# real-world-cryprography/APSU

Hardware: AMD Instinct MI355X
Metric: sender query-eval ms (ComputePowers + all BinBundles + gather), 16M-4096 params (lower is better)
Workload: dtype u64; 1 GPU; 16M-4096: n=8192, 4 bundle indices x 7 BinBundles (degrees [1303, 170]), 6 source -> 72 target powers, ps_low_degree=44; db_bytes_rank0=5459379072, binbundles_rank0=28, parallelism=binbundle-shard x1

## Files before the change

### apsu_amd/csrc/c_api.cpp

```cpp
#include "../../include/apsu_he.h"

#include <algorithm>
#include <thread>
#include <atomic>
#include <cstdlib>
#include <cstddef>
#include <cstring>
#include <new>
#include <string>

#include "db_file.h"
#include "engine.h"
#include "multi.h"
#include "wire.h"
#include "seal_codec.h"

using namespace apsu_he;

#include <condition_variable>
#include <mutex>
#include <unordered_set>

struct apsu_he_powers;
struct apsu_he_ctx { std::unique_ptr<Engine> eng; std::unordered_set<apsu_he_powers *> live_powers; int recycling = 0; };
// ... 296 lines not shown

static void wrap_bundles(std::vector<std::unique_ptr<Bundle>> &made, apsu_he_bundle **out)
{
    std::vector<std::unique_ptr<apsu_he_bundle>> hs(made.size());
    for (auto &h : hs) h = std::make_unique<apsu_he_bundle>();
    for (size_t i = 0; i < hs.size(); i++) { hs[i]->b = std::move(made[i]); out[i] = hs[i].release(); }
}

int apsu_he_bundle_split(apsu_he_ctx *c, const apsu_he_bundle *b, uint32_t parts, const uint32_t *cache_idx, apsu_he_bundle **out)
{
    return guarded([&] {
        REQUIRE(c && b && b->b && out, "null argument");
        auto made = c->eng->split_bundle(*b->b, parts, cache_idx);
        wrap_bundles(made, out);
    });
}

int apsu_he_bundle_adopt(apsu_he_ctx *dst, apsu_he_ctx *src, const apsu_he_bundle *b, uint32_t cache_idx, apsu_he_bundle **out)
{
    return guarded([&] {
        REQUIRE(dst && src && b && b->b && out, "null argument");
        std::vector<std::unique_ptr<Bundle>> made;
        made.push_back(dst->eng->adopt_bundle(*src->eng, *b->b, cache_idx));
        wrap_bundles(made, out);
    });
}

int apsu_he_db_rebase(apsu_he_ctx *dst, apsu_he_ctx *src, const apsu_he_bundle *const *bundles, uint32_t n_bundles, apsu_he_bundle **out,
                      uint32_t *origin, uint32_t *cache_idx, uint32_t capacity, uint32_t *n_out)
{
    return guarded([&] {
        REQUIRE(dst && src && n_out && ((out && origin) || !capacity), "null argument");
        const auto v = bundle_ptrs(bundles, n_bundles);
        Engine::RebaseResult r = dst->eng->rebase_from(*src->eng, v.data(), n_bundles);
        *n_out = (uint32_t)r.bundles.size();
        if (r.bundles.size() > capacity)
            throw std::invalid_argument("rebase: " + std::to_string(r.bundles.size()) + " BinBundles come out, the caller has room for " + std::to_string(capacity));
        for (size_t i = 0; i < r.bundles.size(); i++) { origin[i] = r.origin[i]; if (cache_idx) cache_idx[i] = r.bundles[i]->cache_idx; }
        wrap_bundles(r.bundles, out);
    });
}

int apsu_he_db_entries_plan(const apsu_he_ctx *c, const uint64_t *offsets, uint32_t *bundles_per_index, uint32_t *total)
{
    return guarded([&] {
        REQUIRE(c && offsets && total, "null argument");
        const BulkPlan plan = c->eng->entries_plan(offsets);
        REQUIRE(plan.total <= 0xFFFFFFFFull, "more than 2^32 - 1 BinBundles");
        if (bundles_per_index) std::copy(plan.bundles.begin(), plan.bundles.end(), bundles_per_index);
        *total = (uint32_t)plan.total;
    });
}

int apsu_he_db_build_from_entries(apsu_he_ctx *c, const uint8_t *entries, int entries_on_device, const uint64_t *offsets, apsu_he_bundle **out,
                                  uint32_t capacity, uint32_t *n_out)
{
    return guarded([&] {
        REQUIRE(c && offsets && n_out && (out || !capacity), "null argument");
        const BulkPlan plan = c->eng->entries_plan(offsets);
        REQUIRE(plan.total <= 0xFFFFFFFFull, "more than 2^32 - 1 BinBundles");
        *n_out = (uint32_t)plan.total;
        if (plan.total > capacity)
            throw std::invalid_argument("build_from_entries: " + std::to_string(plan.total) + " BinBundles come out, the caller has room for " + std::to_string(capacity));
        REQUIRE(entries || !plan.total, "null argument");
        auto made = c->eng->build_from_entries(entries, entries_on_device != 0, offsets);
        wrap_bundles(made, out);
    });
}

int apsu_he_bundle_bins(apsu_he_ctx *c, const apsu_he_bundle *b, uint64_t *roots, uint32_t *counts, uint32_t stride)
{ return guarded([&] { REQUIRE(c && b && b->b && counts, "null argument"); c->eng->bundle_bins(*b->b, roots, counts, stride); }); }
int apsu_he_debug_bundle_bins_form(apsu_he_ctx *c, const apsu_he_bundle *b, uint64_t *roots, uint32_t *counts, uint32_t stride, int form)
{
    return guarded([&] {
        REQUIRE(c && b && b->b && counts, "null argument");
        REQUIRE(form >= Engine::BINS_FORM_AUTO && form <= Engine::BINS_FORM_COMPOSED, "unknown form");
        c->eng->bundle_bins(*b->b, roots, counts, stride, form);
    });
}
int apsu_he_debug_run_step(apsu_he_ctx *c, const apsu_he_step_args *args)
{
    return guarded([&] {
        REQUIRE(c && args, "null argument");
        static_assert((int)APSU_HE_STEP_LIFT == (int)Engine::STEP_LIFT && (int)APSU_HE_STEP_UNLIFT == (int)Engine::STEP_UNLIFT && (int)APSU_HE_STEP_INTT_TENSOR == (int)Engine::STEP_INTT_TENSOR && (int)APSU_HE_STEP_ROOTS_SPLIT == (int)Engine::STEP_ROOTS_SPLIT && (int)APSU_HE_STEP_SEED_EXPAND == (int)Engine::STEP_SEED_EXPAND && (int)APSU_HE_STEP_FLAG_MONOMIAL == (int)Engine::STEP_FLAG_MONOMIAL && (int)APSU_HE_STEP_MAC_INFO == (int)Engine::STEP_MAC_INFO && (int)APSU_HE_STEP_LIMB0_ROWS == (int)Engine::STEP_LIMB0_ROWS && (int)APSU_HE_STEP_ENTRIES_SCATTER + 1 == (int)Engine::STEP_COUNT && (int)APSU_HE_STEP_KEY == (int)Engine::STEP_KEY &&
                      (int)APSU_HE_STEP_KARA == (int)Engine::STEP_KARA && (int)APSU_HE_STEP_PACKED == (int)Engine::STEP_PACKED && (int)APSU_HE_STEP_LIMB_SLOW == (int)Engine::STEP_LIMB_SLOW &&
                      (int)APSU_HE_STEP_COMPOSED == (int)Engine::STEP_COMPOSED && (int)APSU_HE_STEP_NORED == (int)Engine::STEP_NORED, "step ids of the header and the engine");
        Engine::StepArgs a{};
        a.step = args->step; a.chain_idx = args->chain_idx; a.flags = args->flags;
        a.terms = args->terms; a.polys = args->polys; a.batch = args->batch; a.e0 = args->e0; a.n_ext = args->n_ext;
        for (int i = 0; i < 6; i++) { a.in[i] = args->in[i]; a.in_words[i] = args->in_words[i]; }
        for (int i = 0; i < 2; i++) { a.out[i] = args->out[i]; a.out_words[i] = args->out_words[i]; }
        c->eng->debug_run_step(a);
    });
}
static int read_op_times(apsu_he_ctx *c, Engine::Op op, std::initializer_list<double *> out)
{
    return guarded([&] {
        REQUIRE(c, "null argument");
        double ms[Engine::OP_SPANS];
        c->eng->op_times(op, ms, (int)out.size());
        int i = 0;
        for (double *p : out) { if (p) *p = ms[i]; i++; }
    });
}
int apsu_he_debug_bins_times(apsu_he_ctx *c, double *decode_ms, double *roots_ms, double *mult_ms)
{ return read_op_times(c, Engine::OP_BINS, { decode_ms, roots_ms, mult_ms }); }
int apsu_he_debug_split_times(apsu_he_ctx *c, double *decode_ms, double *roots_ms, double *split_ms, double *build_ms)
{ return read_op_times(c, Engine::OP_SPLIT, { decode_ms, roots_ms, split_ms, build_ms }); }
int apsu_he_debug_merge_times(apsu_he_ctx *c, double *decode_ms, double *kernel_ms, double *encode_ms)
{ return read_op_times(c, Engine::OP_MERGE, { decode_ms, kernel_ms, encode_ms }); }
int apsu_he_debug_build_from_entries_times(apsu_he_ctx *c, double *copy_ms, double *scatter_ms, double *build_ms)
{ return read_op_times(c, Engine::OP_BUILD, { copy_ms, scatter_ms, build_ms }); }
int apsu_he_debug_set_scatter_blocks(apsu_he_ctx *c, uint32_t blocks)
{ return guarded([&] { REQUIRE(c, "null argument"); c->eng->set_scatter_blocks(blocks); }); }
int apsu_he_debug_lookup_times(apsu_he_ctx *c, double *decode_ms, double *kernels_ms)
{ return read_op_times(c, Engine::OP_LOOKUP, { decode_ms, kernels_ms }); }
int apsu_he_algebraize_items(apsu_he_ctx *c, const uint8_t *items, size_t count, int items_on_device, uint64_t *felts, int felts_on_device)
{
    return guarded([&] {
        REQUIRE(c && (!count || (items && felts)), "null argument");
        c->eng->algebraize_items(items, count, items_on_device != 0, felts, felts_on_device != 0);
    });
}
int apsu_he_item_locations(apsu_he_ctx *c, const uint8_t *items, size_t count, int items_on_device, uint32_t *locs, int locs_on_device)
{
    return guarded([&] {
        REQUIRE(c && (!count || (items && locs)), "null argument");
        c->eng->item_locations(items, count, items_on_device != 0, locs, locs_on_device != 0);
    });
}
int apsu_he_items_bucket(apsu_he_ctx *c, const uint8_t *items, size_t count, int items_on_device, uint64_t *offsets, uint32_t *order, uint64_t *total)
{
    return guarded([&] {
        REQUIRE(c && offsets && total && (!count || (items && order)), "null argument");
        c->eng->items_bucket(items, count, items_on_device != 0, offsets, order, total);
    });
}
int apsu_he_cuckoo_table(apsu_he_ctx *c, const uint8_t *items, size_t count, int items_on_device, uint64_t max_rounds, uint32_t *table_idx,
                         uint32_t *item_loc, uint64_t *rounds)
{
    return guarded([&] {
        REQUIRE(c && table_idx && (!count || (items && item_loc)), "null argument");
        c->eng->cuckoo_table(items, count, items_on_device != 0, max_rounds, table_idx, item_loc, rounds);
    });
}
int apsu_he_query_values(apsu_he_ctx *c, const uint8_t *table_items, int on_device, uint64_t *values, int values_on_device)
{
    return guarded([&] {
        REQUIRE(c && table_items && values, "null argument");
        c->eng->query_values(table_items, on_device != 0, values, values_on_device != 0);
    });
}
int apsu_he_debug_item_locations(apsu_he_ctx *c, const uint8_t *items, size_t count, uint32_t hash_func_count, uint32_t table_size, uint32_t *locs)
{
    return guarded([&] {
        REQUIRE(c && (!count || (items && locs)), "null argument");
        c->eng->debug_item_locations(items, count, hash_func_count, table_size, locs);
    });
}
int apsu_he_debug_cuckoo_insert(apsu_he_ctx *c, const uint8_t *items, const uint32_t *locs, size_t count, uint32_t hash_func_count, uint32_t table_size,
                                uint64_t max_rounds, int form, uint32_t *table_idx, uint32_t *item_loc, uint64_t *rounds)
{
    return guarded([&] {
        REQUIRE(c && table_idx && (!count || (items && locs && item_loc)), "null argument");
        c->eng->debug_cuckoo_insert(items, locs, count, hash_func_count, table_size, max_rounds, form, table_idx, item_loc, rounds);
    });
}
// ... 1425 lines not shown
```

### apsu_amd/csrc/dev_consts.cpp

```cpp
#include "dev_consts.h"
#include "eval_plan.h"
#include "mac_core.h"

#include <algorithm>
#include <cstdint>
#include <cstdlib>
#include <cstring>
#include <stdexcept>
#include <string>
#include <utility>

namespace apsu_he {

uint32_t packed_row_bits(u64 q)
{
    const int bits = 64 - __builtin_clzll(q);
    for (u32 c = (u32)std::max(bits, 32); c < 64; c++) {
        u32 g = 2 * c, r = 32;
        while (r) { const u32 t2 = g % r; g = r; r = t2; }
        if ((32 - g) + 2 * c <= 128) return c;
    }
    return 64;
}

// ... 149 lines not shown
            dc.map_ksacc[(size_t)c * (DMAXL + 1) + I] = id;
        }
    }
    dc.map_ext_fin = dc.map_ext;
    for (int c = 0; c < nl; c++) {
        DevLevel &d = dc.levels[c];
        if (!behz_unrolled(d.L, d.nB)) continue;
        for (int e = 0; e < d.E; e++) {
            (e < d.L ? d.fin_q[e] : d.fin_b[e - d.L]) = table_ref<ShoupConst>(dc.fin.size());
            push_twisted(hp, dc.map_ext[(size_t)c * DMAXE + e], e < d.L ? d.t_inv_punct_q[e].w : d.t_bsk[e - d.L].w, dc.fin);
            dc.map_ext_fin[(size_t)c * DMAXE + e] |= NTT_MAP_RAW;
        }
    }
    for (int c = 1; c < nl; c++) {
        DevLevel &d = dc.levels[c];
        for (int j = 0; j + 1 < d.L; j++) {
            d.drop_tw[j] = table_ref<ShoupConst>(dc.drop.size());
            push_twisted(hp, j, d.inv_q_last[j].w, dc.drop);
        }
        d.last_tw = scale_ref(hp, d.L - 1);
    }
    dc.map_ksacc_raw = dc.map_ksacc;
    for (int &v : dc.map_ksacc_raw) v |= NTT_MAP_RAW;
    dc.map_ct.resize(DMAXL + DMAXB + 4);
    for (size_t i = 0; i < dc.map_ct.size(); i++) dc.map_ct[i] = (int)i;
}

static void build_key(const HeParams &hp, DeviceConstants &dc)
{
    DevKey &k = dc.key;
    std::memset(&k, 0, sizeof(k));
    k.K = hp.K;
    for (int j = 0; j < hp.K; j++) k.q[j] = make_mod(hp.key_q[j]);
    if (hp.K > 1) {
        const u64 p = hp.key_q[hp.K - 1];
        k.p_half = p >> 1;
        for (int j = 0; j < hp.K - 1; j++) {
            k.p_half_mod[j] = k.p_half % hp.key_q[j];
            k.inv_p[j] = shoup_const(hp.inv_p_mod_q[j], hp.key_q[j]);
            k.md_tw[j] = table_ref<ShoupConst>(dc.mdtw.size());
            push_twisted(hp, j, hp.inv_p_mod_q[j], dc.mdtw);
        }
        k.p_tw = scale_ref(hp, hp.K - 1);
    }
    if (hp.K - 1 > hp.first_chain_idx && hp.K <= DMAXL) {
        dc.key_level.resize(1);
        DevLevel &d = dc.key_level[0];
        std::memset(&d, 0, sizeof(d));
        d.L = hp.K;
        for (int j = 0; j < hp.K; j++) d.q[j] = k.q[j];
    }
    for (u64 q : hp.key_q) {
        dc.max_multiple.push_back(~(u64)0 - (~(u64)0 % q) - 1);
        dc.row_bits.push_back(packed_row_bits(q));
    }
}

DeviceConstants build_device_constants(const HeParams &hp)
{
    DeviceConstants dc;
    build_transform_tables(hp, dc);
    build_levels(hp, dc);
    build_key(hp, dc);
    dc.data_primes_narrow = true;
    for (u64 q : hp.key_q) dc.data_primes_narrow = dc.data_primes_narrow && ntt_is_narrow(q, hp.logn);
    dc.ext_primes_narrow = dc.data_primes_narrow;
    for (u64 m : hp.aux_primes) dc.ext_primes_narrow = dc.ext_primes_narrow && ntt_is_narrow(m, hp.logn);
    dc.unlift_exact = hp.batching && hp.key_q[0] / 2 >= hp.t && hp.key_q[0] > 2 * hp.t;
    return dc;
}

EngineSwitches read_switches()
{
    EngineSwitches s;
    auto flag = [](const char *name, auto &out) { if (const char *v = std::getenv(name)) out = std::atoi(v) != 0; };
    auto size = [](const char *name, size_t &out) { if (const char *v = std::getenv(name)) out = std::strtoull(v, nullptr, 10); };
    flag("APSU_HE_SPLIT", s.two_stream_default);
    flag("APSU_HE_MAC_KARA", s.mac_kara);
    flag("APSU_HE_EVAL_SIDE", s.eval_side);
    flag("APSU_HE_PACKED_ROWS", s.packed_rows);
    flag("APSU_HE_EVAL_PER_TERM", s.force_per_term);
    flag("APSU_HE_SEED_EXPAND_HOST", s.seed_expand_host);
    flag("APSU_HE_FUSE_TAIL", s.fuse_tail);
    size("APSU_HE_EVAL_WS_BYTES", s.eval_ws_bytes);
    size("APSU_HE_ARENA_BYTES", s.arena_bytes);
    size("APSU_HE_NTT_LATENCY_LIMBS", s.ntt_latency_limbs);
    size("APSU_HE_SEED_REJ_CAP", s.seed_rej_cap);
    return s;
}

}
```

### apsu_amd/csrc/dev_consts.h

```cpp
#pragma once
#include <cstddef>
#include <vector>

#include "modmath.h"
#include "ntt_core.h"
#include "ntt_form.h"
#include "params.h"

namespace apsu_he {

constexpr int EW_T = 256;
constexpr int DMAXL = 8;
constexpr int DMAXB = DMAXL + 2;
constexpr int DMAXE = DMAXL + DMAXB;
constexpr u32 SEED_REJ_CAP = 8192;

struct ShoupConst { u64 w, wq; };

struct DevLevel {
    int L, nB, nBsk, E;
    Mod q[DMAXL];
    Mod bsk[DMAXB];
    Mod ext[DMAXE];
    u64 t;
// ... 23 lines not shown
    u64 msk_half;
    ShoupConst s_q_to_bsk[DMAXB][DMAXL];
    ShoupConst s_prod_q_bsk[DMAXB];
    ShoupConst s_q_to_bsk_mt[DMAXB][DMAXL];
    ShoupConst s_prod_q_bsk_mt[DMAXB];
    ShoupConst s_fl[DMAXB];
    ShoupConst s_B_to_q[DMAXL][DMAXB];
    ShoupConst s_B_to_msk[DMAXB];
    ShoupConst s_prod_B_q[DMAXL], s_neg_prod_B_q[DMAXL];
    const ShoupConst *fin_q[DMAXL];
    const ShoupConst *fin_b[DMAXB];
    const ShoupConst *drop_tw[DMAXL];
    const ShoupConst *last_tw;
};

struct DevKey {
    int K;
    Mod q[DMAXL + 1];
    u64 p_half;
    u64 p_half_mod[DMAXL];
    ShoupConst inv_p[DMAXL];
    const ShoupConst *md_tw[DMAXL];
    const ShoupConst *p_tw;
};

constexpr int NTT_MAP_RAW = 1 << 30, NTT_MAP_MASK = NTT_MAP_RAW - 1;

inline ShoupConst shoup_const(u64 w, u64 q) { return ShoupConst{ w, (u64)(((u128)w << 64) / q) }; }
inline Mod make_mod(u64 q) { ModulusInfo m(q); return Mod{ q, m.ratio[0], m.ratio[1] }; }
uint32_t packed_row_bits(u64 q);

inline NttTable make_ntt_table(u64 q, int logn)
{
    const ModulusInfo m(q);
    NttTable tb{};
    tb.q = q;
    tb.r1 = m.ratio[1];
    tb.r0 = m.ratio[0];
    tb.narrow = ntt_is_narrow(q, logn) ? 1 : 0;
    ntt_fold_params(q, tb.fold_k, tb.fold_c);
    tb.wide_d4 = ntt_wide_d4(q, tb.narrow != 0);
    return tb;
}
inline NttTable make_ntt_table(const NttTablesHost &t, int logn, const TwPair *fwd, const TwPair *dit, const TwPair *scale)
{
    NttTable tb = make_ntt_table(t.mod.value, logn);
    tb.ninv = t.ninv;
    tb.ninv_q = t.ninv_q;
    tb.fwd = fwd;
    tb.dit = dit;
    tb.scale = scale;
    return tb;
}

struct DeviceConstants {
    std::vector<TwPair> tw;
    std::vector<NttTable> tabs;
    std::vector<ShoupConst> fin, drop, mdtw;
    std::vector<DevLevel> levels;
    DevKey key;
    std::vector<int> map_ext, map_ext_fin, map_ks, map_ksacc, map_ksacc_raw, map_ct;
    std::vector<DevLevel> key_level;
    std::vector<u64> max_multiple;
    bool data_primes_narrow = false;
    bool ext_primes_narrow = false;
    bool unlift_exact = false;
    std::vector<u32> row_bits;
    void relocate(const TwPair *tw_base, const ShoupConst *fin_base, const ShoupConst *drop_base, const ShoupConst *mdtw_base);
};
DeviceConstants build_device_constants(const HeParams &hp);

struct EngineSwitches {
    static constexpr size_t ARENA_AUTO = ~(size_t)0;
    int two_stream_default = -1;
    bool eval_side = true;
    bool packed_rows = true;
    size_t eval_ws_bytes = (size_t)6 << 30;
    size_t arena_bytes = ARENA_AUTO;
    bool force_per_term = false;
    int mac_kara = -1;
    bool seed_expand_host = false;
    size_t seed_rej_cap = SEED_REJ_CAP;
    bool fuse_tail = true;
    size_t ntt_latency_limbs = NTT_FORM_AUTO;
};
EngineSwitches read_switches();

}
```

### apsu_amd/csrc/engine.h

```cpp
#pragma once
#include <hip/hip_runtime.h>

#include <functional>
#include <memory>
#include <mutex>
#include <string>
#include <vector>

#include "device.h"
#include "params.h"
#include "db_place.h"
#include "db_compact.h"
#include "bulk_place.h"
#include "powers_dag.h"
#include "powers_sched.h"
#include "bundle_layout.h"

namespace apsu_he {

struct HipError : std::runtime_error { using std::runtime_error::runtime_error; };

class DevBuf {
public:
    DevBuf() = default;
// ... 129 lines not shown
    RebaseResult rebase_from(Engine &src, const Bundle *const *bundles, uint32_t n_bundles);
    void bundles_eval_plain(const Bundle *const *bundles, uint32_t n_bundles, const u64 *x, bool x_on_device, const u64 *masks, bool masks_on_device,
                            u64 *out, bool out_on_device, unsigned char *is_bin);
    SelfTestReport self_test(const Bundle *const *bundles, uint32_t count, const u64 seed[8], const u64 *x_host, const uint32_t *query_indices = nullptr,
                             uint32_t n_query = 0, const uint32_t *mask_positions = nullptr);
    enum { SAVED_STRIPPED = 1, SAVED_NO_CACHE = 2 };
    std::vector<uint8_t> export_saved(const Bundle &b, const u64 ntt_parms_id[4], uint32_t flags, int compr);
    struct CompactResult {
        CompactPlan plan;
        std::vector<std::unique_ptr<Bundle>> merged;
    };
    CompactResult compact(uint32_t bundle_idx, const Bundle *const *bundles, uint32_t n_bundles);
    void algebraize_items(const unsigned char *items, size_t count, bool items_on_device, u64 *out, bool out_on_device);
    void item_locations(const unsigned char *items, size_t count, bool items_on_device, uint32_t *locs, bool locs_on_device);
    void items_bucket(const unsigned char *items, size_t count, bool items_on_device, u64 *offsets, uint32_t *order, u64 *total);
    void cuckoo_table(const unsigned char *items, size_t count, bool items_on_device, u64 max_rounds, uint32_t *table_idx, uint32_t *item_loc, u64 *rounds);
    void query_values(const unsigned char *table_items, bool on_device, u64 *values, bool values_on_device);
    enum { CUCKOO_FORM_AUTO = 0, CUCKOO_FORM_LDS = 1, CUCKOO_FORM_GLOBAL = 2 };
    void debug_item_locations(const unsigned char *items, size_t count, uint32_t H, uint32_t T, uint32_t *locs);
    void debug_cuckoo_insert(const unsigned char *items, const uint32_t *locs, size_t count, uint32_t H, uint32_t T, u64 max_rounds, int form,
                             uint32_t *table_idx, uint32_t *item_loc, u64 *rounds);
    size_t bundle_image_size(const Bundle &b) const;
    size_t save_bundle(const Bundle &b, unsigned char *buf, size_t capacity);
    std::unique_ptr<Bundle> load_bundle(const unsigned char *buf, size_t size);
    void mask_generate(u64 seed, uint32_t count, u64 *masks_dev, u64 *values_host, u64 *blocks_host);
    void mask_generate_blake2xb(const u64 seed[8], u64 first_value, uint32_t count, u64 *masks_dev, u64 *values_host, u64 *blocks_host);
    void decrypt_decode(const u64 *sk_ntt_host, const u64 *cts, bool on_device, uint32_t count, u64 *values_host, u64 *blocks_host,
                        int *budget_bits = nullptr, bool sk_on_device = false, u64 *values_dev = nullptr);
    void keygen(const u64 seed[8], u64 *sk_ntt_host, bool sk_on_device = false);
    void relin_keygen(const u64 *sk_ntt_host, const u64 seed[8], u64 *ksk_host, u64 *seeds_host, std::unique_ptr<RelinKeys> *resident,
                      bool sk_on_device = false);
    void query_create(const u64 *sk_ntt_host, const u64 seed[8], const uint32_t *bundle_indices, int nb, const u64 *values, bool values_on_device,
                      u64 *cts_dev, u64 *seeds_host, bool sk_on_device = false);
    void seed_expand(int chain_idx, int count, const u64 *seeds, u64 *const *dst);
    size_t download_coeff(const Bundle &b, uint32_t d, u64 *out, size_t capacity, int *kind);
    std::unique_ptr<Powers> compute_powers(const uint32_t *bundle_indices, int nb, const u64 *const *src, bool on_device,
                                           const RelinKeys *rk);
    void eval_bundles(const Bundle *const *bundles, int count, const Powers &pw, const RelinKeys *rk,
                      const u64 *const *masks, bool masks_on_device, u64 *out, bool out_on_device, u64 *const *out_rows = nullptr);

    uint32_t power_size(uint32_t power) const;
    uint32_t result_size(const Bundle &b) const;
    uint32_t result_polys() const { return result_polys_; }

    size_t workspace_bytes() const { return arena_.bytes(); }
    enum Counter { C_HOST_SYNC = 0, C_JOB_UPLOAD, C_JOB_HIT, C_ARENA_GROW, C_POWERS_ALLOC, C_STAGE_WRAP, C_JOB_REALLOC, C_PIPELINED, C_COUNT };
    void counters_read(uint64_t *out, int capacity) const { for (int i = 0; i < capacity && i < C_COUNT; i++) out[i] = counters_[i]; }

    enum ProfKind { P_NTT_FWD = 0, P_NTT_INV, P_MAC, P_BEHZ_EXT, P_TENSOR, P_BEHZ_FINISH, P_KEYSWITCH, P_MODSWITCH, P_OTHER, P_NTT_FUSED, P_COUNT };
    struct ProfStats { double ms[P_COUNT]; uint64_t launches[P_COUNT]; uint64_t units[P_COUNT]; };
    void profile_enable(int mode);
    void profile_read(ProfStats *out, bool reset);
    enum Phase { PH_RUN_QUERY = 0, PH_COMPUTE_POWERS, PH_PROCESS_BIN_BUNDLE_CACHE, PH_COUNT };
    struct PhaseSummary { uint64_t count = 0; double sum_ms = 0, min_ms = 0, max_ms = 0; };
    static const char *phase_name(int phase);
    void phase_enable(bool on);
    void phase_read(PhaseSummary *out, bool reset);
    void set_two_stream(int mode) { std::lock_guard<std::mutex> g(mu_); two_stream_mode_ = mode < 0 ? -1 : (mode ? 1 : 0); }
    void set_async_results(bool on) { std::lock_guard<std::mutex> g(mu_); async_results_ = on; }
    void set_query_overlap(int mode)
    {
        std::lock_guard<std::mutex> g(mu_);
        inputs_ready_ = mode != 0;
        pipe_cp_ = mode == 1 || mode == 3;
        force_pipe_ = mode == 3;
    }
    void set_tier1_on_device(bool on) { std::lock_guard<std::mutex> g(mu_); tier1_device_ = on; }
    void wait();
    void drain();
    bool take_bad_source();
    void download_power(const Powers &pw, uint32_t bundle_idx, uint32_t power, u64 *out, size_t capacity_words, int *chain_idx,
                        int *is_ntt);
    int device() const { return device_; }
    enum Step { STEP_LEVEL_INFO = 0, STEP_BEHZ_EXT, STEP_DROP_BEHZ_EXT, STEP_TENSOR, STEP_TENSOR_CONV, STEP_TENSOR_SUM, STEP_BEHZ_FINISH,
                STEP_BEHZ_FINISH_SUM, STEP_KS_INNER, STEP_KS_MODDOWN, STEP_MODSWITCH, STEP_MODSWITCH_JOBS, STEP_I0_FINISH, STEP_EVAL_EPILOGUE,
                STEP_ADD_MANY, STEP_SUM_JOBS, STEP_ADD_PLAIN, STEP_DYADIC_PLAIN, STEP_LIFT,
                STEP_POLYN_WITH_ROOTS, STEP_BINS_UPDATE, STEP_BIN_COUNTS, STEP_POLY_DEGREE, STEP_BINS_LOOKUP, STEP_BINS_MERGE, STEP_BINS_ROWS,
                STEP_BINS_EVAL, STEP_EVAL_COMPARE, STEP_ROOTS, STEP_UNLIFT,
                STEP_NTT_INFO, STEP_NTT, STEP_NTT_GATHER, STEP_INTT_TENSOR,
                STEP_ROOTS_SPLIT,
                STEP_SEED_EXPAND, STEP_DECRYPT_ROUND, STEP_PLAIN_POWERS, STEP_SAMPLE_SMALL, STEP_SMALL_LIFT, STEP_ENC_FINISH, STEP_RLK_FINISH,
                STEP_FLAG_MONOMIAL,
                STEP_MAC_INFO, STEP_MAC, STEP_TERM_PRODUCT, STEP_PACK_ROWS, STEP_UNPACK_ROWS, STEP_LIMB0_ROWS,
                STEP_ENTRIES_SCATTER, STEP_COUNT };
    enum : uint32_t { STEP_RAW = 1, STEP_ACCUMULATE = 2, STEP_STORE = 4, STEP_KEY = 8, STEP_PLAN = 16, STEP_COMPOSED = 32, STEP_INVERSE = 64, STEP_NORED = 128,
                      STEP_KARA = 256, STEP_PACKED = 512, STEP_LIMB_SLOW = 1024 };
    struct StepArgs {
        int step, chain_idx;
        uint32_t flags;
        int terms, polys, batch, e0, n_ext;
        const u64 *in[6];
        size_t in_words[6];
        u64 *out[2];
        size_t out_words[2];
    };
    void debug_run_step(const StepArgs &a);
    void debug_run_db_step(const StepArgs &a);
    void debug_run_ntt_step(const StepArgs &a);
    void debug_run_query_step(const StepArgs &a);
    void debug_run_mac_step(const StepArgs &a);
    std::mutex &wire_mutex() { return wire_mu_; }
    void wire_stage(size_t bytes, u64 **device, u64 **pinned);

private:
    u64 *ws(size_t words);
    template <class T> T *ws_as(size_t count, size_t extra_words = 0);
    void ws_reset(size_t need_bytes_hint = 0);
    template <class T> const T *upload_jobs(const std::vector<T> &v);

    const DevLevel *dlevel(int chain_idx) const { return d_levels_.u() ? reinterpret_cast<const DevLevel *>(d_levels_.p()) + chain_idx : nullptr; }
    const LevelConstants &hlevel(int chain_idx) const { return hp_.level[chain_idx]; }
    const NttTable *tabs() const { return reinterpret_cast<const NttTable *>(d_tabs_.p()); }
    const DevKey *dkey() const { return reinterpret_cast<const DevKey *>(d_key_.p()); }
    const int *map_ct() const { return reinterpret_cast<const int *>(d_map_ct_.p()); }
    const int *map_ext(int chain_idx) const { return reinterpret_cast<const int *>(d_map_ext_.p()) + chain_idx * DMAXE; }
    const int *map_ext_fin(int chain_idx) const { return reinterpret_cast<const int *>(d_map_ext_fin_.p()) + chain_idx * DMAXE; }
    const int *map_ks(int chain_idx) const { return reinterpret_cast<const int *>(d_map_ks_.p()) + chain_idx * (DMAXL + 1) * DMAXL; }
    const int *map_ksacc(int chain_idx) const { return reinterpret_cast<const int *>(d_map_ksacc_.p()) + chain_idx * (DMAXL + 1); }
    const int *map_ksacc_raw(int chain_idx) const { return reinterpret_cast<const int *>(d_map_ksacc_raw_.p()) + chain_idx * (DMAXL + 1); }

    void d_ntt(u64 *data, size_t count, const int *modmap, int period, bool inverse, bool narrow);
    void d_ntt_ct(u64 *data, size_t polys, int chain_idx, bool inverse) { d_ntt(data, polys * (chain_idx + 1), map_ct(), chain_idx + 1, inverse, data_primes_narrow_); }
    bool d_relinearize(u64 *ct3, size_t ct_stride, int batch, const RelinKeys &rk, int chain_idx, u64 *ext_out = nullptr, int n_ext = 0,
                       u64 **defer_moddown = nullptr);
    void check_level(int chain_idx) const;
    void check_tier1_residues(const u64 *ct, size_t polys, int chain_idx, const char *what) const;
    void d_multiply_sized(const u64 *ea, int sa, const u64 *eb, int sb, u64 *out, int chain_idx);
    std::unique_ptr<Powers> compute_powers_nks(const uint32_t *bundle_indices, int nb, const u64 *const *src, bool on_device);
    void eval_bundles_nks(const Bundle *const *bundles, int count, const Powers &pw, const u64 *const *masks, bool masks_on_device,
                          u64 *out, bool out_on_device, u64 *const *out_rows);
    PowerSizes sizes_;
    uint32_t result_polys_ = 2;

    HeParams hp_;
    const EngineSwitches sw_ = read_switches();
    PSUParams psu_;
    bool has_psu_ = false;
    PowersDag dag_;
    int device_ = 0;
    hipStream_t st_ = nullptr;
    std::mutex mu_;

    DevBuf d_tabs_, d_tw_, d_levels_, d_key_, d_map_ct_, d_map_ext_, d_map_ext_fin_, d_map_ks_, d_map_ksacc_, d_map_ksacc_raw_, d_fin_, d_drop_, d_mdtw_;
    DevBuf arena_;
    size_t arena_off_ = 0;
    struct Lane { hipStream_t st = nullptr; DevBuf arena; size_t off = 0, job_seq = 0; };
    Lane lanes_[3];
    int cur_lane_ = 0, overflow_lane_ = 0;
    void switch_lane(int lane);
    hipEvent_t ev_main_ = nullptr;
    hipEvent_t ev_fork_ = nullptr, ev_side_ = nullptr, ev_intt_ = nullptr;
    bool inputs_ready_ = false;
    bool pipe_cp_ = true;
    bool force_pipe_ = false;
    bool data_primes_narrow_ = false;
    bool ext_primes_narrow_ = false;
    bool async_results_ = false;
    std::vector<hipEvent_t> inflight_;
    size_t inflight_head_ = 0, inflight_count_ = 0;
    int max_inflight_ = 2;
    void throttle_inflight();
    void mark_inflight();
    static constexpr int BAD_SLOTS = 16;
    unsigned *bad_source_ = nullptr;
    unsigned bad_reported_[BAD_SLOTS] = {};
    uint32_t query_seq_ = 0;
    void check_sources();
    void check_sources(const Powers &pw);
    bool bad_source_pending(int slot, bool take);
    void *stage_ = nullptr;
    size_t stage_bytes_ = 0, stage_off_ = 0;
    struct JobWay { DevBuf buf; std::vector<unsigned char> host; uint64_t stamp = 0; };
    struct JobSlot { JobWay way[4]; };
    uint64_t job_stamp_ = 0;
    std::vector<JobSlot> job_slots_;
    size_t job_seq_ = 0, job_seq_base_ = 0;
    std::vector<std::unique_ptr<Powers>> powers_pool_;
public:
    void recycle_powers(std::unique_ptr<Powers> p);
private:
    std::vector<DevBuf> retired_;
    uint64_t counters_[C_COUNT] = {};
    std::mutex wire_mu_;
    DevBuf wire_dev_;
    void *wire_pinned_ = nullptr;
    size_t wire_pinned_bytes_ = 0;

    PowersSched sched_, sched_low_, sched_high_;
    void mask_generate_impl(uint32_t count, u64 *masks_dev, u64 *values_host, u64 *blocks_host, const std::function<void(u64 *, size_t)> &fill);
    bool fuse_tensor_ = true;
    bool tier1_device_ = false;
    void tier1_done() { if (!tier1_device_ || prof_on_) sync(); }
    bool packed_rows_ = true;
    BundleLayout layout_of(uint32_t degree) const { return bundle_layout(psu_.query_params.ps_low_degree, degree, hp_.first_chain_idx); }
    std::unique_ptr<Bundle> new_bundle(uint32_t bundle_idx, uint32_t cache_idx, uint32_t degree, BundleLayout *layout = nullptr) const;
    size_t slot_bytes(int chain_idx, bool packed) const;
    void pack_bundle(Bundle &b);
    void unpack_bundle(Bundle &b);
    MacPlan plan_mac(const std::vector<MacStream> &streams, size_t nlimbs, size_t n) const;
    void d_mac(const MacPlan &p, const MacJob *jobs = nullptr);
    bool split_ok_ = false;
    int two_stream_mode_ = -1;
    struct DagRun;
    void dag_sources(DagRun &run, const u64 *const *src, bool on_device);
    void dag_level(DagRun &run, size_t d, const RelinKeys *rk);
    void dag_outputs(DagRun &run, Powers &pw, bool do_low, bool do_high);
    void dag_walk(const PowersSched &s, int nb, const u64 *const *src, bool on_device, const RelinKeys *rk, Powers &pw);
    void powers_header(Powers &pw, const uint32_t *bundle_indices, int nb, int low_level, int high_level);
    template <class F> void with_powers_span(F &&body);
    struct EvalCall;
    void eval_plain(EvalCall &c, const std::vector<int> &pl_ids);
    void eval_patstock(EvalCall &c, const std::vector<int> &ps_ids);
    void ps_cf_streams(const EvalCall &c, const PsBatch &g, std::vector<MacStream> &out);
    void ps_cf_mac(const EvalCall &c, const PsBatch &g);
    void ps_term_product(const EvalCall &c, const PsBatch &g);
    void ps_i0_finish(const EvalCall &c, const EvalPlan &plan, const PsBatch &g, u64 *i0);
    void ps_tables(EvalCall &c, const EvalPlan &plan, PsBatch &g);
    void ps_run(EvalCall &c, const EvalPlan &plan, PsBatch &g);
    void ps_mac(EvalCall &c, const EvalPlan &plan, PsBatch &g);
    void ps_side(EvalCall &c, const EvalPlan &plan, PsBatch &g);
    void ps_drop_ext(EvalCall &c, const EvalPlan &plan, PsBatch &g);
    void ps_products_summed(EvalCall &c, const EvalPlan &plan, PsBatch &g);
    void ps_products_per_term(EvalCall &c, const EvalPlan &plan, PsBatch &g);
    u64 *ps_i0(EvalCall &c, const EvalPlan &plan, PsBatch &g);
    void ps_epilogue(EvalCall &c, PsBatch &g, const u64 *i0);
    void finish_bundle(Bundle &b, const u64 *raw);
    void encode_bundle(Bundle &b, const u64 *poly);
    void decode_bundle(const Bundle &b, u64 *poly, u64 *coeff = nullptr);
    void decode_coeff(const Bundle &b, u64 *raw);
    void export_coeff(const Bundle &b, DevBuf &raw);
    void build_from_roots(Bundle &b, const u64 *droots, const uint32_t *dcounts, uint32_t bins, uint32_t stride);
    enum { NEED_PSU = 1, NEED_BATCHING, NEED_DECODE };
    void lookup_check(const char *what, int need = NEED_DECODE) const;
    u64 *decode_counted(const Bundle &b, uint32_t *dcounts, u64 *coeff = nullptr, EventStamps *evs = nullptr, size_t mid = 0);
    struct OpClock { EventStamps evs; double ms[OP_SPANS] = {}; } clock_[OP_COUNT];
    void lookup_impl(const Bundle *const *bundles, uint32_t n_bundles, const u64 *felts, const uint32_t *start, size_t count, uint32_t *counts,
                     unsigned char *flags);
    void eval_plain_queue(const Bundle *const *bundles, uint32_t n_bundles, const u64 *const *xs, const u64 *const *masks, u64 *out, unsigned char *is_bin,
                          u32 *bad, EventStamps &evs, size_t first);
    static void eval_plain_collect(const EventStamps &evs, size_t first, uint32_t n_bundles, double *ms);
    struct BinsCounted { u64 *poly, *coeff; uint32_t *dcounts; const uint32_t *counts; };
    struct BinsFound { std::vector<uint32_t> occ, found, mult; std::vector<u64> hits; uint32_t hstride = 0; };
    bool bins_prepare(const Bundle &b, int form);
    BinsCounted bins_counted(const Bundle &b, bool want_coeff, uint32_t *counts, EventStamps &evs);
    void bins_search(const BinsCounted &c, bool kernel, const uint32_t *stride, EventStamps &evs, size_t s, BinsFound &f);
    struct BinsDevice { uint32_t *occ, *found, *mult; u64 *hits; };
    BinsDevice bins_search_device(const BinsCounted &c, bool kernel, const uint32_t *stride, EventStamps &evs, size_t s, BinsFound &f);
    void bins_finish(const BinsCounted &c, BinsFound &f, u64 *roots, uint32_t stride);
    void keep_coeff_rows(const Bundle &b, const u64 *coeff, DevBuf &keep);
    void roots_tables();
    u64 roots_g_ = 0;
    DevBuf d_roots_step_, d_roots_pts_;
    uint32_t scatter_blocks_ = 0;
    bool unlift_exact_ = false;
    DevBuf d_slot_map_;
    DevBuf d_cuckoo_tabs_;
    void cuckoo_tables_ready();
    const unsigned char *cuckoo_items(const unsigned char *items, size_t count, bool on_device);
    void cuckoo_insert_run(const unsigned char *ditems, const uint32_t *dlocs, uint32_t count, uint32_t H, uint32_t T, u64 max_rounds, int form,
                           uint32_t *table_idx, uint32_t *item_loc, u64 *rounds);
    bool queue_seed_expand(int L, int count, const u64 *seeds, u64 *const *dst);
    bool seeds_overflowed(int count);
    const DevLevel *seed_level(int L);
    void host_seed_expand(int L, int count, const u64 *seeds, u64 *const *dst);
    void check_key_residues(const u64 *sk_ntt_host, int limbs) const;
    DevBuf d_seed_rej_, d_key_level_;
    std::vector<DevLevel> key_level_;
    std::vector<u64> max_multiple_;

    struct ProfRec { hipEvent_t a, b; int kind; uint64_t units; };
    bool prof_on_ = false, prof_open_ = false, prof_ntt_only_ = false;
    std::vector<ProfRec> prof_recs_;
    std::vector<hipEvent_t> prof_pool_;
    ProfStats prof_{};
    void prof_begin(int kind, uint64_t units);
    void prof_end();
    void prof_collect();

    struct PhaseSpan { hipEvent_t a = nullptr, b = nullptr, b2 = nullptr; int phase = 0; };
    bool phase_on_ = false;
    std::vector<PhaseSpan> phase_spans_;
    std::vector<hipEvent_t> phase_pool_;
    PhaseSummary phase_[PH_COUNT];
    hipEvent_t query_start_ = nullptr, query_end_ = nullptr;
    hipEvent_t phase_event(hipStream_t st);
    void phase_close_query();
    void phase_collect();
    struct Enter;
    friend struct EngineAccess;
    friend struct ProfScope;
};

}
```

### apsu_amd/csrc/engine_eval.cpp

```cpp
#include "engine_impl.h"
#include "eval_plan.h"

namespace apsu_he {

static const u64 *bundle_slot(const Bundle &b, bool lifted, size_t slot, size_t dense_words)
{
    const DevBuf &buf = lifted ? b.lifted : b.ntt;
    if (!b.packed) return buf.u() + slot * dense_words;
    return reinterpret_cast<const u64 *>(static_cast<const char *>(buf.p()) + slot * (lifted ? b.lifted_slot_bytes : b.ntt_slot_bytes));
}
static u32 bundle_stride(const Bundle &b, bool lifted, size_t dense_words)
{
    return b.packed ? (u32)(lifted ? b.lifted_slot_bytes : b.ntt_slot_bytes) : (u32)dense_words;
}

struct Engine::EvalCall {
    const Bundle *const *bundles; const Powers &pw; const RelinKeys *rk;
    const u64 *const *masks; bool masks_on_device; u64 *const *out_rows;
    size_t n; uint32_t l; int high, low; size_t Ll, Lh, Eh; u32 low_term_stride;
    std::vector<int> bslot;
    int c0 = 0;
    u64 *res = nullptr, *mask_d = nullptr;
    const u64 *low_ptr(uint32_t power, int b) const { return pw.low.u() + (((size_t)b * pw.n_low + (power - 1)) * 2) * Ll * n; }
    const u64 *hext_ptr(uint32_t i, int b) const { return pw.hext.u() + (((size_t)b * pw.n_high + (i - 1)) * 2) * Eh * n; }
    u64 *res_ptr(int i) const { return out_rows ? out_rows[c0 + i] : res + (size_t)i * 2 * n; }
    const u64 *mask_ptr(int i) const { return masks_on_device ? masks[c0 + i] : mask_d + (size_t)i * n; }
    const Bundle &bundle(int i) const { return *bundles[c0 + i]; }
    int slot(int i) const { return bslot[c0 + i]; }
};
struct PsBatch {
    std::vector<int> ids;
    std::vector<int> nin, in_off;
    int Bs = 0, NI = 0;
    u64 *inner = nullptr, *ssum = nullptr, *vlast = nullptr, *term = nullptr, *cf = nullptr;
    std::vector<int> imap;
    const int *imap_dev = nullptr;
    size_t n_vlast_side = 0;
    MacPlan mac;
    const MacJob *mac_jobs = nullptr;
    const TermJob *term_jobs = nullptr;
    size_t n_term = 0; bool term_packed = false;
    u64 *ext = nullptr, *result = nullptr, *ks_acc = nullptr, *i0_side = nullptr;
};

void Engine::eval_plain(EvalCall &c, const std::vector<int> &pl_ids)
{
    const int Bp = (int)pl_ids.size();
    const int lvl = c.low;
    const size_t Lv = lvl + 1;
    u64 *acc = ws((size_t)Bp * 2 * Lv * c.n);
    std::vector<MacStream> ms;
    std::vector<EpiJob> ej;
    for (int x = 0; x < Bp; x++) {
        const Bundle &b = c.bundle(pl_ids[x]);
        u64 *o = acc + (size_t)x * 2 * Lv * c.n;
        if (b.degree) ms.push_back(MacStream{ bundle_slot(b, false, 0, Lv * c.n), c.low_ptr(1, c.slot(pl_ids[x])), o, b.degree,
                                              bundle_stride(b, false, Lv * c.n), c.low_term_stride, (u32)(c.Ll * c.n), (u32)(Lv * c.n), 0, (u32)Lv,
                                              (u32)b.packed });
        else HIP_CHECK(hipMemsetAsync(o, 0, 2 * Lv * c.n * sizeof(u64), st_));
        ej.push_back(EpiJob{ o, nullptr, nullptr, b.a0.u(), c.mask_ptr(pl_ids[x]), c.res_ptr(pl_ids[x]) });
    }
    d_mac(plan_mac(ms, Lv, c.n));
    d_ntt_ct(acc, (size_t)Bp * 2, lvl, true);
    { PROFW(P_MODSWITCH, (size_t)Bp * c.n * (2 * Lv + 4)); launch_eval_epilogue(dlevel(0), lvl, upload_jobs(ej), Lv * c.n, hp_.irrelevant_bit_count, c.n, Bp, st_); }
}

void Engine::ps_cf_streams(const EvalCall &c, const PsBatch &g, std::vector<MacStream> &out)
{
    for (int x = 0; x < g.Bs; x++) {
        const Bundle &b = c.bundle(g.ids[x]);
        out.push_back(MacStream{ bundle_slot(b, true, 0, c.Lh * c.n), c.hext_ptr(1, c.slot(g.ids[x])), g.cf + (size_t)x * 2 * c.Lh * c.n, b.H,
                                 bundle_stride(b, true, c.Lh * c.n), (u32)((size_t)2 * c.Eh * c.n), (u32)(c.Eh * c.n), (u32)(c.Lh * c.n), 0, (u32)c.Lh,
                                 (u32)b.packed });
    }
}
void Engine::ps_cf_mac(const EvalCall &c, const PsBatch &g)
{
    std::vector<MacStream> cs;
    ps_cf_streams(c, g, cs);
    d_mac(plan_mac(cs, c.Lh, c.n));
}

void Engine::eval_patstock(EvalCall &c, const std::vector<int> &ps_ids)
{
    if (c.low < c.high) throw std::logic_error("the low powers lie below the high powers");
    PsBatch g;
    g.ids = ps_ids;
    std::stable_sort(g.ids.begin(), g.ids.end(), [&](int a, int b) { return c.slot(a) < c.slot(b); });
    g.Bs = (int)g.ids.size();
    g.nin.resize(g.Bs); g.in_off.resize(g.Bs);
    EvalState s{};
    for (int x = 0; x < g.Bs; x++) {
        const Bundle &b = c.bundle(g.ids[x]);
        g.nin[x] = (int)b.H - (b.r == 0 ? 1 : 0);
        g.in_off[x] = g.NI;
        g.NI += g.nin[x];
        s.max_terms = std::max(s.max_terms, g.nin[x]);
    }
    s.low = c.low; s.high = c.high;
    s.L = hlevel(c.high).L; s.nB = hlevel(c.high).nB;
    s.l = c.l; s.q_last = hlevel(c.low).q[c.Ll - 1];
    for (size_t j = 0; j < c.Lh; j++) s.q_widest = std::max(s.q_widest, hlevel(c.high).q[j]);
    s.Bs = g.Bs;
    s.high_in_flight = c.pw.high_async && c.pw.high_ready;
    s.eval_side = sw_.eval_side; s.prof_on = prof_on_; s.force_per_term = sw_.force_per_term; s.fuse_tensor = fuse_tensor_; s.fuse_tail = sw_.fuse_tail;
    s.lane2 = lanes_[2].st != nullptr; s.on_lane0 = cur_lane_ == 0;
    const EvalPlan plan = plan_eval(s);
    ps_tables(c, plan, g);
    ps_run(c, plan, g);
}

void Engine::ps_tables(EvalCall &c, const EvalPlan &plan, PsBatch &g)
{
    const size_t n = c.n, Ll = c.Ll, Lh = c.Lh;
    const uint32_t l = c.l;
    const int Bs = g.Bs;
    const bool cf_here = plan.cf == CF_WITH_MAC;
    const size_t w_inner = (size_t)g.NI * 2 * Ll * n, w_ssum = plan.i0_fast ? (size_t)Bs * 2 * Lh * n : 0;
    const size_t w_vlast = plan.need_vlast ? (size_t)Bs * l * 2 * n : 0, w_term = plan.i0_fast ? 0 : (size_t)Bs * l * 2 * Ll * n;
    const size_t w_cf = (size_t)Bs * 2 * Lh * n;
    g.inner = ws(w_inner + w_ssum + w_vlast + w_term + (cf_here ? w_cf : 0));
    g.ssum = g.inner + w_inner; g.vlast = g.ssum + w_ssum; g.term = g.vlast + w_vlast;
    g.cf = cf_here ? g.term + w_term : nullptr;
    std::vector<MacStream> ms;
    auto map_push = [&](size_t polys, int first_limb, int limbs) {
        for (size_t p = 0; p < polys; p++) for (int j = 0; j < limbs; j++) g.imap.push_back(first_limb + j);
    };
    for (int x = 0; x < Bs; x++) {
        const Bundle &b = c.bundle(g.ids[x]);
        for (int i = 1; i <= g.nin[x]; i++) {
            const u32 cnt = (u32)i < b.H ? l : b.r;
            ms.push_back(MacStream{ bundle_slot(b, false, (size_t)i * l, Ll * n), c.low_ptr(1, c.slot(g.ids[x])),
                                    g.inner + ((size_t)g.in_off[x] + i - 1) * 2 * Ll * n, cnt,
                                    bundle_stride(b, false, Ll * n), c.low_term_stride, (u32)(Ll * n), (u32)(Ll * n), 0, (u32)Ll,
                                    (u32)b.packed });
        }
    }
    map_push((size_t)g.NI * 2, 0, (int)Ll);
    if (plan.raw_drop) for (int &v : g.imap) v |= NTT_MAP_RAW;
    if (plan.i0_fast) {
        for (int x = 0; x < Bs; x++) {
            const Bundle &b = c.bundle(g.ids[x]);
            ms.push_back(MacStream{ bundle_slot(b, false, 0, Ll * n), c.low_ptr(1, c.slot(g.ids[x])), g.ssum + (size_t)x * 2 * Lh * n, l,
                                    bundle_stride(b, false, Ll * n), c.low_term_stride, (u32)(Ll * n), (u32)(Lh * n), 0, (u32)Lh,
                                    (u32)b.packed });
        }
        map_push((size_t)Bs * 2, 0, (int)Lh);
        if (plan.raw_i0) for (size_t x = g.imap.size() - (size_t)Bs * 2 * Lh; x < g.imap.size(); x++) g.imap[x] |= NTT_MAP_RAW;
    }
    std::vector<TermJob> tj;
    if (plan.need_vlast || !plan.i0_fast) {
        for (int x = 0; x < Bs; x++) {
            const Bundle &b = c.bundle(g.ids[x]);
            const int bs = c.slot(g.ids[x]);
            if (plan.i0_fast) {
                if (x == 0) g.term_packed = b.packed;
                else if (g.term_packed != (bool)b.packed) throw std::logic_error("BinBundles of one evaluation differ in their row format");
            }
            for (u32 j = 1; j <= l; j++) {
                if (plan.i0_fast)
                    tj.push_back(TermJob{ bundle_slot(b, false, j - 1, Ll * n), c.low_ptr(j, bs), g.vlast + ((size_t)x * l + j - 1) * 2 * n });
                else
                    ms.push_back(MacStream{ bundle_slot(b, false, j - 1, Ll * n), c.low_ptr(j, bs),
                                            g.term + ((size_t)x * l + j - 1) * 2 * Ll * n, 1, bundle_stride(b, false, Ll * n), c.low_term_stride,
                                            (u32)(Ll * n), (u32)(Ll * n), 0, (u32)Ll, (u32)b.packed });
            }
        }
        if (plan.i0_fast) {
            map_push((size_t)Bs * l * 2, (int)Ll - 1, 1);
            if (plan.raw_i0) for (size_t x = g.imap.size() - (size_t)Bs * l * 2; x < g.imap.size(); x++) g.imap[x] |= NTT_MAP_RAW;
        } else map_push((size_t)Bs * l * 2, 0, (int)Ll);
    }
    if (plan.side_i0) g.n_vlast_side = (size_t)Bs * l * 2;
    if (cf_here) { ps_cf_streams(c, g, ms); map_push((size_t)Bs * 2, 0, (int)Lh); }
    g.mac = plan_mac(ms, Ll, n);
    g.mac_jobs = upload_jobs(g.mac.jobs);
    if (!tj.empty()) { g.term_jobs = upload_jobs(tj); g.n_term = tj.size(); }
}

void Engine::ps_term_product(const EvalCall &c, const PsBatch &g)
{
    PROF(P_MAC, (uint64_t)g.n_term * (g.term_packed ? packed_row_bits(hp_.key_q[c.Ll - 1]) : 64));
    launch_term_product(dlevel(c.low), g.term_jobs, g.n_term, c.n, (int)c.Ll - 1, (u32)(c.Ll * c.n), (u32)c.n, g.term_packed, st_);
}
void Engine::ps_i0_finish(const EvalCall &c, const EvalPlan &plan, const PsBatch &g, u64 *i0)
{
    std::vector<I0Job> ij;
    for (int x = 0; x < g.Bs; x++)
        ij.push_back(I0Job{ g.ssum + (size_t)x * 2 * c.Lh * c.n, g.vlast + (size_t)x * c.l * 2 * c.n, i0 + (size_t)x * 2 * c.Lh * c.n, (int)c.l, 1 });
    PROFW(P_MODSWITCH, (size_t)g.Bs * c.n * (4 * c.Lh + 2 * c.l));
    launch_i0_finish(dlevel(c.low), upload_jobs(ij), c.n, g.Bs, st_, plan.raw_i0);
}

void Engine::ps_mac(EvalCall &c, const EvalPlan &plan, PsBatch &g)
{
    d_mac(g.mac, g.mac_jobs);
    g.imap_dev = upload_jobs(g.imap);
    if (plan.side_i0) HIP_CHECK(hipEventRecord(ev_fork_, st_));
    else if (g.n_term) ps_term_product(c, g);
    d_ntt(g.inner, g.imap.size() - g.n_vlast_side, g.imap_dev, (int)g.imap.size(), true, false);
    if (plan.side_i0) HIP_CHECK(hipEventRecord(ev_intt_, st_));
}

void Engine::ps_side(EvalCall &c, const EvalPlan &plan, PsBatch &g)
{
    g.cf = ws((size_t)g.Bs * 2 * c.Lh * c.n);
    if (plan.side_i0) g.i0_side = ws((size_t)g.Bs * 2 * c.Lh * c.n);
    else HIP_CHECK(hipEventRecord(ev_fork_, st_));
    switch_lane(2);
    struct Back { Engine *e; ~Back() { e->switch_lane(0); } } back{ this };
    HIP_CHECK(hipStreamWaitEvent(st_, ev_fork_, 0));
    if (plan.side_i0) {
        ps_term_product(c, g);
        d_ntt(g.vlast, g.n_vlast_side, g.imap_dev + (g.imap.size() - g.n_vlast_side), (int)g.n_vlast_side, true, false);
    }
    if (plan.wait_high_ready) HIP_CHECK(hipStreamWaitEvent(st_, c.pw.high_ready, 0));
    ps_cf_mac(c, g);
    d_ntt_ct(g.cf, (size_t)g.Bs * 2, c.high, true);
    if (plan.side_i0) {
        HIP_CHECK(hipStreamWaitEvent(st_, ev_intt_, 0));
        ps_i0_finish(c, plan, g, g.i0_side);
    }
    HIP_CHECK(hipEventRecord(ev_side_, st_));
}

void Engine::ps_drop_ext(EvalCall &c, const EvalPlan &plan, PsBatch &g)
{
    const size_t n = c.n;
    const int NI = g.NI;
    const LevelConstants &h = hlevel(c.high);
    g.ext = ws((size_t)NI * 2 * c.Eh * n);
    if (plan.fused_drop) {
        PROFW(P_BEHZ_EXT, (size_t)NI * 2 * n * (c.Ll + c.Eh));
        if (!launch_drop_behz_ext(dlevel(c.high), h.L, h.nB, g.inner, c.Ll * n, 1, g.ext, n, NI * 2, st_, plan.raw_drop))
            throw std::logic_error("the plan takes the fused drop + extension, the kernel table has none for this level");
    } else {
        u64 *innerh = g.inner;
        for (int lv = c.low; lv > c.high; lv--) {
            u64 *nxt = ws((size_t)NI * 2 * lv * n);
            { PROFW(P_MODSWITCH, (size_t)NI * 2 * n * (2 * lv + 1)); launch_modswitch(dlevel(lv), innerh, (size_t)2 * (lv + 1) * n, 2, nxt, n, NI, st_); }
            innerh = nxt;
        }
        { PROFW(P_BEHZ_EXT, (size_t)NI * 2 * n * (c.Lh + c.Eh)); launch_behz_ext(dlevel(c.high), h.L, h.nB, innerh, c.Lh * n, 1, g.ext, n, NI * 2, st_); }
    }
    d_ntt(g.ext, (size_t)NI * 2 * c.Eh, map_ext(c.high), (int)c.Eh, false, ext_primes_narrow_);
}

void Engine::ps_products_summed(EvalCall &c, const EvalPlan &plan, PsBatch &g)
{
    const size_t n = c.n, Lh = c.Lh, Eh = c.Eh, nBskh = Eh - Lh;
    const int Bs = g.Bs, NI = g.NI;
    const LevelConstants &h = hlevel(c.high);
    const bool late_cf = plan.cf == CF_BEHIND_HIGH_READY;
    g.result = ws((size_t)Bs * 3 * Lh * n);
    u64 *dq = ws((size_t)NI * 3 * Lh * n + (size_t)Bs * 3 * nBskh * n + (late_cf ? (size_t)Bs * 2 * Lh * n : 0));
    u64 *bsum = dq + (size_t)NI * 3 * Lh * n;
    if (late_cf) {
        g.cf = bsum + (size_t)Bs * 3 * nBskh * n;
        ps_cf_mac(c, g);
    }
    std::vector<TensorSumJob> tj;
    std::vector<FinishSumJob> fj;
    std::vector<int> dmap;
    for (int x = 0; x < Bs; x++) {
        if (!g.nin[x]) { HIP_CHECK(hipMemsetAsync(g.result + (size_t)x * 3 * Lh * n, 0, 3 * Lh * n * sizeof(u64), st_)); continue; }
        const size_t job = (size_t)g.in_off[x];
        tj.push_back(TensorSumJob{ g.ext + job * 2 * Eh * n, c.hext_ptr(1, c.slot(g.ids[x])), dq + job * 3 * Lh * n,
                                   bsum + (size_t)x * 3 * nBskh * n, g.nin[x], 0 });
        fj.push_back(FinishSumJob{ dq + job * 3 * Lh * n, bsum + (size_t)x * 3 * nBskh * n, g.result + (size_t)x * 3 * Lh * n, g.nin[x], 0 });
    }
    const int rawf = behz_unrolled(h.L, h.nB) ? NTT_MAP_RAW : 0;
    for (size_t p = 0; p < (size_t)NI * 3; p++) for (size_t j = 0; j < Lh; j++) dmap.push_back((int)j | rawf);
    for (size_t p = 0; p < (size_t)Bs * 3; p++) for (size_t i = 0; i < nBskh; i++) dmap.push_back(hp_.bsk_id(h.nB, (int)i) | rawf);
    if (late_cf) for (size_t p = 0; p < (size_t)Bs * 2; p++) for (size_t j = 0; j < Lh; j++) dmap.push_back((int)j);
    if (plan.fuse_tensor) {
        std::vector<TensorJob> pj;
        for (int x = 0; x < Bs; x++)
            for (int i = 0; i < g.nin[x]; i++) {
                const size_t job = (size_t)g.in_off[x] + i;
                pj.push_back(TensorJob{ g.ext + job * 2 * Eh * n, c.hext_ptr(1 + i, c.slot(g.ids[x])), dq + job * 3 * Lh * n });
            }
        { PROFW(P_TENSOR, ((size_t)NI * 4 + (size_t)Bs * 3) * (Eh - Lh) * n); launch_tensor_sum(dlevel(c.high), (int)Eh, upload_jobs(tj), n, (int)tj.size(), (int)Lh, st_); }
        PROF(P_NTT_FUSED, dmap.size());
        launch_intt_tensor(hp_.logn, upload_jobs(pj), (int)pj.size(), (int)Lh, Eh * n, bsum, dmap.size() - pj.size() * 3 * Lh,
                           tabs(), upload_jobs(dmap), (int)dmap.size(), st_, sw_.ntt_latency_limbs);
    } else {
        { PROFW(P_TENSOR, ((size_t)NI * 4 * Eh + (size_t)NI * 3 * Lh + (size_t)Bs * 3 * (Eh - Lh)) * n); launch_tensor_sum(dlevel(c.high), (int)Eh, upload_jobs(tj), n, (int)tj.size(), 0, st_); }
        d_ntt(dq, dmap.size(), upload_jobs(dmap), (int)dmap.size(), true, false);
    }
    { PROFW(P_BEHZ_FINISH, ((size_t)NI * 3 * Lh + (size_t)Bs * 3 * (Eh - Lh) + (size_t)Bs * 3 * Lh) * n); launch_behz_finish_sum(dlevel(c.high), h.L, h.nB, upload_jobs(fj), n, (int)fj.size(), st_); }
}

void Engine::ps_products_per_term(EvalCall &c, const EvalPlan &plan, PsBatch &g)
{
    const size_t n = c.n, Lh = c.Lh, Eh = c.Eh;
// ... 180 lines not shown
```

### apsu_amd/csrc/engine_mac_steps.cpp

```cpp
#include "engine_impl.h"
#include "mac_plan.h"

#include <string>

namespace apsu_he {

namespace {

[[noreturn]] void refuse(const std::string &why) { throw std::invalid_argument("debug_run_step: " + why); }
void need(bool ok, const char *why) { if (!ok) refuse(why); }

void canonical(const u64 *x, size_t words, u64 m, const char *what)
{
    u64 bad = 0;
    for (size_t k = 0; k < words; k++) bad |= (u64)(x[k] >= m);
    if (bad) refuse(std::string(what) + " holds a word that is not a canonical residue of its limb");
}

void canonical_dense(const u64 *x, size_t slots, int L, size_t n, const DevLevel &lv, const char *what)
{
    for (size_t s = 0; s < slots; s++)
        for (int j = 0; j < L; j++) canonical(x + (s * L + j) * n, n, lv.q[j].q, what);
}

void canonical_packed(const std::vector<u64> &padded, size_t slots, size_t slot_bytes, int L, size_t n, const DevLevel &lv, const char *what)
{
    const char *base = reinterpret_cast<const char *>(padded.data());
    u64 bad = 0;
    for (size_t s = 0; s < slots; s++)
        for (int j = 0; j < L; j++) {
            const u32 *row = reinterpret_cast<const u32 *>(base + s * slot_bytes + lv.mac_row_off[j]);
            for (size_t c = 0; c < n; c++) bad |= (u64)(packed_coeff(row, c, lv.mac_bits[j]) >= lv.q[j].q);
        }
    if (bad) refuse(std::string(what) + " holds a coefficient that is not a canonical residue of its limb");
}

}

void Engine::debug_run_mac_step(const StepArgs &a)
{
    const size_t n = hp_.n;
    need(a.step >= STEP_MAC_INFO && a.step <= STEP_LIMB0_ROWS, "unknown step");
    check_level(a.chain_idx);
    const int L = a.chain_idx + 1;
    const bool kara = a.flags & STEP_KARA, packed = a.flags & STEP_PACKED, limb_slow = a.flags & STEP_LIMB_SLOW;
    const size_t batch = a.batch > 0 ? (size_t)a.batch : 0, terms = a.terms > 0 ? (size_t)a.terms : 0, polys = a.polys > 0 ? (size_t)a.polys : 0;
    auto in_is = [&](int i, size_t words, const char *what) { if (!a.in[i] || a.in_words[i] != words) refuse(std::string(what) + ": wrong size"); };
    auto out_is = [&](int i, size_t words, const char *what) { if (!a.out[i] || a.out_words[i] != words) refuse(std::string(what) + ": wrong size"); };

    sync();
    DevLevel lv;
    HIP_CHECK(hipMemcpy(&lv, dlevel(a.chain_idx), sizeof(DevLevel), hipMemcpyDeviceToHost));
    if (lv.L != L) throw std::logic_error("debug_run_step: the device's level block is not the level's");
    size_t packed_slot = 0;
    bool any_packed = false;
    for (int j = 0; j < L; j++) { packed_slot += n * lv.mac_bits[j] / 8; any_packed |= lv.mac_bits[j] != 64; }
    const size_t dense_slot = (size_t)L * n * sizeof(u64);

    if (a.step == STEP_MAC_INFO) {
        out_is(0, 2 + 7 * (size_t)L, "mac_info: out[0] [2 + 7 L]");
        u64 *o = a.out[0];
        *o++ = (u64)L; *o++ = packed_slot;
        for (int j = 0; j < L; j++) {
            *o++ = lv.mac_shift[j]; *o++ = lv.mac_chunk[j]; *o++ = lv.mac_chunk_k[j]; *o++ = lv.mac_bits[j]; *o++ = lv.mac_row_off[j];
            *o++ = lv.mac_mask_hi[j]; *o++ = mac_kara_usable(lv.q[j].q) ? 1 : 0;
        }
        return;
    }
    need(n % 64 == 0, "the multiply-accumulate steps take rings of a multiple of 64 coefficients (a bit-packed slot is whole 64-bit words)");
    if (packed) need(any_packed, "packed: every row of this context is 64 bits wide (mac_bits), there is no bit-packed form");
    const size_t slot = packed ? packed_slot : dense_slot, slot_words = slot / 8;

    std::vector<MacJob> mj;
    std::vector<TermJob> tj;
    std::vector<u64> padded;
    auto pad_in = [&](int i) { padded.assign(a.in_words[i] + 2, 0); std::memcpy(padded.data(), a.in[i], a.in_words[i] * sizeof(u64)); };
    size_t P = 0, NL = 0, njobs = 0;
    switch (a.step) {
    case STEP_MAC: {
        need(batch >= 1 && batch <= 64, "mac: batch out of range (1 .. 64)");
        need(polys >= 1 && polys <= (size_t)MAC_G, "mac: streams per job (polys) outside 1 .. 4");
        need(terms >= 1, "mac: a chain of no terms (terms 0)");
        need(terms <= 4096, "mac: terms out of range (1 .. 4096)");
        NL = a.n_ext > 0 ? (size_t)a.n_ext : 0;
        need(a.e0 >= 0 && NL >= 1 && (size_t)a.e0 + NL <= (size_t)L, "mac: limbs limb0 .. limb0 + nl - 1 (e0, n_ext) reach beyond the level");
        const size_t pw_job = batch * terms * 2 * n;
        need(a.in[0] && a.in_words[0] % pw_job == 0, "mac: in[0] powers [batch][terms][2][P][n]: wrong size");
        P = a.in_words[0] / pw_job;
        need(P >= (size_t)L, "mac: powers of fewer limbs per polynomial (P) than the level has");
        need(P <= (size_t)DMAXE, "mac: powers of more limbs per polynomial (P) than an extended polynomial has");
        in_is(1, batch * polys * terms * slot_words, "mac: in[1] plaintexts [batch][polys][terms] slots");
        out_is(0, batch * polys * 2 * NL * n, "mac: out[0] [batch][polys][2][n_ext][n]");
        if (a.in[2]) in_is(2, batch * 4, "mac: in[2] job table [batch][4]");
        if (kara) for (int j = 0; j < L; j++) need(mac_kara_usable(lv.q[j].q), "mac: the three-product form on a level with a prime that mac_kara_usable rejects");
        for (size_t r = 0; r < batch * terms * 2; r++)
            for (int j = 0; j < L; j++) canonical(a.in[0] + (r * P + j) * n, n, lv.q[j].q, "mac: in[0] (powers)");
        if (packed) { pad_in(1); canonical_packed(padded, batch * polys * terms, slot, L, n, lv, "mac: in[1] (bit-packed plaintexts)"); }
        else canonical_dense(a.in[1], batch * polys * terms, L, n, lv, "mac: in[1] (plaintexts)");
        for (size_t b = 0; b < batch; b++) {
            const u64 limb0 = a.in[2] ? a.in[2][b * 4] : (u64)a.e0, nl = a.in[2] ? a.in[2][b * 4 + 1] : NL;
            const u64 ng = a.in[2] ? a.in[2][b * 4 + 2] : polys, cnt = a.in[2] ? a.in[2][b * 4 + 3] : terms;
            need(limb0 <= (u64)L && nl >= 1 && nl <= NL && limb0 + nl <= (u64)L, "mac: a job's limbs (limb0, nl) reach beyond the level or beyond n_ext");
            need(ng >= 1 && ng <= polys, "mac: a job's streams (ng) outside 1 .. polys");
            need(cnt >= 1, "mac: a job with a chain of no terms (cnt 0)");
            need(cnt <= terms, "mac: a job's chain (cnt) is longer than terms");
            MacJob j{};
            j.cnt = (u32)cnt; j.ng = (u32)ng; j.limb0 = (u32)limb0; j.nl = (u32)nl; j.packed = packed ? 1 : 0;
            j.pt_stride = (u32)(packed ? slot : slot_words); j.pw_stride = (u32)(2 * P * n); j.pw_poly_stride = (u32)(P * n); j.out_poly_stride = (u32)(NL * n);
            mj.push_back(j);
        }
    } break;
    case STEP_TERM_PRODUCT: {
        need(batch >= 1 && batch <= 64, "term_product: batch out of range (1 .. 64)");
        need(terms >= 1 && batch * terms <= ((size_t)1 << 17), "term_product: jobs (batch * terms) outside 1 .. 2^17");
        need(a.e0 >= 0 && a.e0 < L, "term_product: the limb (e0) is beyond the level");
        need(a.in[0] && a.in_words[0] % (batch * 2 * n) == 0, "term_product: in[0] powers [batch][2][P][n]: wrong size");
        P = a.in_words[0] / (batch * 2 * n);
        need(P >= (size_t)L && P <= (size_t)DMAXE, "term_product: limbs per polynomial of the powers (P) outside L .. the extended base");
        njobs = batch * terms;
        in_is(1, batch * slot_words, "term_product: in[1] plaintexts [batch] slots");
        out_is(0, (njobs + 1) * 2 * n, "term_product: out[0] [batch * terms + 1][2][n]");
        for (size_t r = 0; r < batch * 2; r++) canonical(a.in[0] + (r * P + (size_t)a.e0) * n, n, lv.q[a.e0].q, "term_product: in[0] (powers)");
        if (packed) { pad_in(1); canonical_packed(padded, batch, slot, L, n, lv, "term_product: in[1] (bit-packed plaintexts)"); }
        else canonical_dense(a.in[1], batch, L, n, lv, "term_product: in[1] (plaintexts)");
    } break;
    case STEP_PACK_ROWS:
    case STEP_UNPACK_ROWS: {
        need(batch >= 1, "pack_rows / unpack_rows: no slots (batch)");
        pack_rows_grid_check(batch, L);
        if (a.step == STEP_PACK_ROWS) {
            in_is(0, batch * (size_t)L * n, "pack_rows: in[0] dense [slots][L][n]");
            out_is(0, batch * packed_slot / 8 + 2, "pack_rows: out[0] [slots] bit-packed slots + 16 bytes");
            canonical_dense(a.in[0], batch, L, n, lv, "pack_rows: in[0]");
        } else {
            in_is(0, batch * packed_slot / 8, "unpack_rows: in[0] [slots] bit-packed slots");
            out_is(0, batch * (size_t)L * n, "unpack_rows: out[0] dense [slots][L][n]");
            pad_in(0);
        }
    } break;
    case STEP_LIMB0_ROWS: {
        need(batch >= 1 && batch <= 65535, "limb0_rows: count (batch) outside 1 .. 65535");
        in_is(0, batch * slot_words, "limb0_rows: in[0] [count] slots");
        out_is(0, batch * n, "limb0_rows: out[0] [count][n]");
        if (packed) pad_in(0);
    } break;
    default: refuse("unknown step");
    }

    WITH_ARENA({
        auto up = [&](const u64 *src, size_t words) {
            u64 *d = ws(words);
            HIP_CHECK(hipMemcpyAsync(d, src, words * sizeof(u64), hipMemcpyHostToDevice, st_));
            return d;
        };
        auto up_slots = [&](int i) { return packed || a.step == STEP_UNPACK_ROWS ? up(padded.data(), padded.size()) : up(a.in[i], a.in_words[i]); };
        auto down = [&](const u64 *src) { HIP_CHECK(hipMemcpyAsync(a.out[0], src, a.out_words[0] * sizeof(u64), hipMemcpyDeviceToHost, st_)); };
        auto jobs = [&](const auto &v) {
            using T = typename std::decay_t<decltype(v)>::value_type;
            T *d = ws_as<T>(v.size());
            HIP_CHECK(hipMemcpyAsync(d, v.data(), v.size() * sizeof(T), hipMemcpyHostToDevice, st_));
            return static_cast<const T *>(d);
        };
        u64 *o = up(a.out[0], a.out_words[0]);

        switch (a.step) {
        case STEP_MAC: {
            const u64 *pw = up(a.in[0], a.in_words[0]);
            const char *pt = reinterpret_cast<const char *>(up_slots(1));
            for (size_t b = 0; b < batch; b++) {
                MacJob &j = mj[b];
                j.pw = pw + b * terms * 2 * P * n;
                for (size_t g = 0; g < (size_t)MAC_G; g++) {
                    j.pt[g] = reinterpret_cast<const u64 *>(pt + ((b * polys + (g < j.ng ? g : 0)) * terms) * slot);
                    j.out[g] = o + (b * polys + (g < polys ? g : 0)) * 2 * NL * n;
                }
            }
            launch_mac(dlevel(a.chain_idx), L, jobs(mj), n, (int)batch, st_, kara, packed, MacGrid{ mac_grid(n, batch).gx, limb_slow ? 1 : 0 });
        } break;
        case STEP_TERM_PRODUCT: {
            const u64 *pw = up(a.in[0], a.in_words[0]);
            const char *pt = reinterpret_cast<const char *>(up_slots(1));
            tj.clear();
            for (size_t u = 0; u < njobs; u++) tj.push_back(TermJob{ reinterpret_cast<const u64 *>(pt + (u % batch) * slot), pw + (u % batch) * 2 * P * n, o + u * 2 * n });
            launch_term_product(dlevel(a.chain_idx), jobs(tj), njobs, n, a.e0, (u32)(P * n), (u32)n, packed, st_);
        } break;
        case STEP_PACK_ROWS:
            launch_pack_rows(dlevel(a.chain_idx), L, up(a.in[0], a.in_words[0]), o, packed_slot, n, batch, st_);
            break;
        case STEP_UNPACK_ROWS:
            launch_unpack_rows(dlevel(a.chain_idx), L, up_slots(0), packed_slot, o, n, batch, st_);
            break;
        default:
            launch_limb0_rows(dlevel(a.chain_idx), L, up_slots(0), slot, packed, o, n, batch, st_);
            break;
        }
        down(o);
        sync();
    });
}

}
```

### apsu_amd/csrc/eval_plan.h

```cpp
#pragma once
#include <cstddef>
#include <cstdint>

namespace apsu_he {

constexpr bool behz_unrolled(int L, int nB) { return L == nB && L <= 3; }

struct EvalState {
    int low, high;
    int L, nB;
    uint32_t l;
    uint64_t q_last;
    uint64_t q_widest;
    int Bs, max_terms;
    bool high_in_flight;
    bool eval_side, prof_on, force_per_term, fuse_tensor, fuse_tail;
    bool lane2, on_lane0;
};
enum CfPlace {
    CF_WITH_MAC = 0,
    CF_SIDE_LANE = 1,
    CF_BEHIND_HIGH_READY = 2
};
enum I0Form {
    I0_SIDE = 0,
    I0_SSUM = 1,
    I0_FINISH_MAIN = 2,
    I0_GENERAL = 3
};
struct EvalPlan {
    bool i0_fast, need_vlast, raw_drop, raw_i0, fused_drop, summed, side, side_i0, wait_high_ready, fuse_tensor, fuse_tail;
    int cf;
    int i0;
};

inline EvalPlan plan_eval(const EvalState &s)
{
    EvalPlan p{};
    const int Lh = s.high + 1;
    p.i0_fast = (s.low - s.high <= 1) && ((unsigned __int128)(s.l + 1) * s.q_last < ((unsigned __int128)1 << 64));
    p.need_vlast = p.i0_fast && s.low > s.high;
    p.raw_drop = s.low == s.high + 1 && behz_unrolled(s.L, s.nB);
    p.raw_i0 = p.need_vlast;
    p.fused_drop = p.raw_drop;
    p.wait_high_ready = s.high_in_flight;
    p.side = s.eval_side && s.high_in_flight && !s.prof_on && p.i0_fast && s.low != s.high && s.lane2 && s.on_lane0;
    p.side_i0 = p.side && (size_t)s.Bs * s.l <= 4096;
    p.cf = !s.high_in_flight ? CF_WITH_MAC : p.side ? CF_SIDE_LANE : CF_BEHIND_HIGH_READY;
    p.i0 = p.side_i0 ? I0_SIDE : p.i0_fast && s.low == s.high ? I0_SSUM : p.i0_fast ? I0_FINISH_MAIN : I0_GENERAL;
    p.summed = !s.force_per_term && Lh <= 4 && (unsigned __int128)s.max_terms * s.q_widest < ((unsigned __int128)1 << 63);
    p.fuse_tensor = s.fuse_tensor;
    p.fuse_tail = s.fuse_tail;
    return p;
}

}
```

### apsu_amd/csrc/kernels_behz.hip

```cpp
#include "launch_behz.h"
#include "kernel_launch.h"
#include "eval_plan.h"

namespace apsu_he {

template <int TL, int TNB>
__global__ __launch_bounds__(EW_T) void k_behz_ext(const DevLevel *__restrict__ lv, const u64 *__restrict__ in,
                                                   size_t in_stride, int polys, u64 *__restrict__ out, size_t n)
{
    const size_t k = (size_t)blockIdx.x * EW_T + threadIdx.x;
    if (k >= n) return;
    const int L = TL ? TL : lv->L, nBsk = TL ? TNB + 1 : lv->nBsk, E = L + nBsk;
    constexpr int LMAX = TL ? TL : DMAXL;
    constexpr int BMAX = TL ? TNB + 1 : DMAXB;
    const size_t c = blockIdx.y / polys, p = blockIdx.y % polys;
    const u64 *src = in + c * in_stride + p * (size_t)L * n;
    u64 *dst = out + (size_t)blockIdx.y * E * n;
    u64 xs[LMAX];
    u32 mt_acc = 0;
#pragma unroll
    for (int j = 0; j < LMAX; j++) {
        if (TL || j < L) {
            const u64 x = src[(size_t)j * n + k];
            dst[(size_t)j * n + k] = x;
// ... 536 lines not shown
#pragma unroll
    for (int p = 0; p < 2; p++) {
        u64 tl = 0;
        const u64 *a = nullptr;
        if constexpr (MD) {
            a = job.ks_acc + (size_t)p * (L + 1) * n;
            const Mod pm = key->q[key->K - 1];
            const u64x2 tw = ldg16(reinterpret_cast<const u64 *>(key->p_tw + k));
            tl = barrett64(mul_shoup(a[(size_t)L * n + k], tw[0], tw[1], pm.q) + key->p_half, pm);
        }
#pragma unroll
        for (int j = 0; j < DMAXL; j++)
            if (j < L) {
                const u64 q = lv->q[j].q;
                u64 x = job.ct[p * ct_poly_stride + (size_t)j * n + k];
                if constexpr (MD) {
                    const Mod m = key->q[j];
                    const u64 tk = submod(barrett64(tl, m), key->p_half_mod[j], m.q);
                    const u64x2 tw = ldg16(reinterpret_cast<const u64 *>(key->md_tw[j] + k));
                    const u64 u = mul_shoup_lazy(a[(size_t)j * n + k], tw[0], tw[1], m.q);
                    const u64 w = mul_shoup_lazy(tk, key->inv_p[j].w, key->inv_p[j].wq, m.q);
                    x = addmod(x, csub(csub(u + (m.q << 1) - w, m.q << 1), m.q), m.q);
                }
                if (job.add1) x = addmod(x, job.add1[((size_t)p * L + j) * n + k], q);
                if (job.add2) x = addmod(x, job.add2[((size_t)p * L + j) * n + k], q);
                v[p][j] = x;
            }
    }
    {
        const u64 m0 = job.a0[k], m1 = job.mask[k];
        const u64 f0 = plain_fix(lv, m0), f1 = plain_fix(lv, m1);
#pragma unroll
        for (int j = 0; j < DMAXL; j++)
            if (j < L) {
                const u64 q = lv->q[j].q;
                v[0][j] = addmod(addmod(v[0][j], scaled_plain(lv, m0, f0, j), q), scaled_plain(lv, m1, f1, j), q);
            }
    }
    for (int l = lvl; l > 0; l--) {
        const DevLevel *ll = levels + l;
        const u64 ql = ll->q[l].q;
#pragma unroll
        for (int p = 0; p < 2; p++) {
            u64 last = 0;
#pragma unroll
            for (int j = 0; j < DMAXL; j++) if (j == l) last = v[p][j];
            last = addmod(last, ll->half, ql);
#pragma unroll
            for (int j = 0; j < DMAXL; j++)
                if (j < l) {
                    const Mod m = ll->q[j];
                    const u64 tmp = submod(barrett64(last, m), ll->half_mod[j], m.q);
                    v[p][j] = mul_shoup(submod(v[p][j], tmp, m.q), ll->inv_q_last[j].w, ll->inv_q_last[j].wq, m.q);
                }
        }
    }
    job.out[k] = v[0][0] & clear_mask;
    job.out[n + k] = v[1][0] & clear_mask;
}

void launch_eval_epilogue(const DevLevel *levels, int lvl, const EpiJob *jobs, size_t ct_poly_stride, int clear_bits, size_t n,
                          int njobs, hipStream_t st, const DevKey *key)
{
    if (!njobs) return;
    const u64 mask = clear_bits > 0 ? ~(((u64)1 << clear_bits) - 1) : ~(u64)0;
    if (key) hipLaunchKernelGGL(k_eval_epilogue<true>, ew_grid(n, njobs), dim3(EW_T), 0, st, levels, lvl, jobs, ct_poly_stride, mask, n, key);
    else hipLaunchKernelGGL(k_eval_epilogue<false>, ew_grid(n, njobs), dim3(EW_T), 0, st, levels, lvl, jobs, ct_poly_stride, mask, n, key);
    KERNEL_CHECK();
}

template <bool RAW>
__global__ __launch_bounds__(EW_T) void k_i0_finish(const DevLevel *__restrict__ lv, const I0Job *__restrict__ jobs, size_t n)
{
    const size_t k = (size_t)blockIdx.x * EW_T + threadIdx.x;
    if (k >= n) return;
    const I0Job job = jobs[blockIdx.y >> 1];
    const int p = blockIdx.y & 1;
    const int L = lv->L;
    const u64 ql = lv->q[L - 1].q, half = lv->half;
    u64 R = 0;
    const u64 *v = job.v + (size_t)p * n + k;
    u64 tw0 = 0, tw1 = 0;
    if (RAW) { const u64x2 tw = ldg16(reinterpret_cast<const u64 *>(lv->last_tw + k)); tw0 = tw[0]; tw1 = tw[1]; }
    for (int t = 0; t < job.terms; t++) {
        u64 x = v[(size_t)t * 2 * n];
        if (RAW) x = mul_shoup(x, tw0, tw1, ql);
        R += addmod(x, half, ql);
    }
    for (int m = 0; m + 1 < L; m++) {
        const Mod mq = lv->q[m];
        const u64 th = barrett128(mul128((u64)job.terms, lv->half_mod[m]), mq);
        const u64 corr = submod(th, barrett64(R, mq), mq.q);
        const size_t o = ((size_t)p * (L - 1) + m) * n + k;
        u64 r;
        if (RAW) {
            const u64x2 tw = ldg16(reinterpret_cast<const u64 *>(lv->drop_tw[m] + k));
            const u64 a = mul_shoup_lazy(job.s[o], tw[0], tw[1], mq.q);
            const u64 b = mul_shoup_lazy(corr, lv->inv_q_last[m].w, lv->inv_q_last[m].wq, mq.q);
            r = csub(csub(a + b, mq.q << 1), mq.q);
        } else {
            const u64 val = addmod(job.s[o], corr, mq.q);
            r = mul_shoup(val, lv->inv_q_last[m].w, lv->inv_q_last[m].wq, mq.q);
        }
        job.acc[o] = job.store ? r : addmod(job.acc[o], r, mq.q);
    }
}

void launch_i0_finish(const DevLevel *lv_low, const I0Job *jobs, size_t n, int njobs, hipStream_t st, bool raw)
{
    if (!njobs) return;
    if (raw) hipLaunchKernelGGL(k_i0_finish<true>, ew_grid(n, njobs * 2), dim3(EW_T), 0, st, lv_low, jobs, n);
    else hipLaunchKernelGGL(k_i0_finish<false>, ew_grid(n, njobs * 2), dim3(EW_T), 0, st, lv_low, jobs, n);
    KERNEL_CHECK();
}

}
```

### apsu_amd/csrc/kernels_ntt.hip

```cpp
#include "launch_ntt.h"
#include "kernel_launch.h"
#include "ntt_wg.h"
#include "ntt_form.h"
#include <type_traits>

namespace apsu_he {

template <int LOGN, bool INV, int T, int C = 16, int MINW = 4>
__global__ __launch_bounds__(T, MINW) void k_ntt(u64 *__restrict__ data, const NttTable *__restrict__ tabs,
                                           const int *__restrict__ modmap, int period, int split)
{
    constexpr int N = 1 << LOGN;
    __shared__ __attribute__((aligned(16))) u64 lds[lds_slots(N)];
    const int tid = threadIdx.x;
    const size_t g = blockIdx.x;
    const int mv = modmap[(split ? g >> 1 : g) % (size_t)period];
    const NttTable tab = tabs[split ? (((mv & NTT_MAP_MASK) << 1) | (int)(g & 1)) : (mv & NTT_MAP_MASK)];
    u64 *p = data + g * N;
    using SRC = std::conditional_t<INV, SrcStaged, SrcPlain>;
    if (INV && ((mv & NTT_MAP_RAW) || split)) {
        if (tab.narrow) ntt_body<LOGN, INV, NTT_NARROW, T, 0, INV, SRC, true, false, 0, -1, C>(lds, p, tab, tid, nullptr, SRC());
        else if (tab.wide_d4) ntt_body<LOGN, INV, NTT_WIDE_NEAR, T, 0, INV, SRC, true, false, 0, -1, C>(lds, p, tab, tid, nullptr, SRC());
        else ntt_body<LOGN, INV, NTT_WIDE, T, 0, INV, SRC, true, false, 0, -1, C>(lds, p, tab, tid, nullptr, SRC());
        return;
// ... 32 lines not shown
    const u64 e = ntt_reduce_any(p[k], tab);
    const u64 o = mul_shoup_lazy(p[k + h], tw[0], tw[1], q);
    u64 x0 = e + o, x1 = e + (q << 1) - o;
    if (!(mv & NTT_MAP_RAW)) {
        const u64x2 s0 = ldg16(reinterpret_cast<const u64 *>(tab.scale + k)), s1 = ldg16(reinterpret_cast<const u64 *>(tab.scale + k + h));
        x0 = mul_shoup(x0, s0[0], s0[1], q);
        x1 = mul_shoup(x1, s1[0], s1[1], q);
    }
    p[k] = x0;
    p[k + h] = x1;
}

template <int LOGN, int T, int C = 16, int MINW = 4>
__global__ __launch_bounds__(T, MINW) void k_ntt_gather(const u64 *const *__restrict__ src, u64 *__restrict__ data,
                                                  const NttTable *__restrict__ tabs, const int *__restrict__ modmap, int period, int nored)
{
    constexpr int N = 1 << LOGN;
    __shared__ __attribute__((aligned(16))) u64 lds[lds_slots(N)];
    const int tid = threadIdx.x;
    const size_t g = blockIdx.x;
    const NttTable tab = tabs[modmap[g % (size_t)period]];
    u64 *p = data + g * N;
    if (tab.narrow) {
        if (nored) ntt_body<LOGN, false, NTT_NARROW, T, 2, false, SrcPlain, true, false, 0, -1, C>(lds, p, tab, tid, src[g]);
        else ntt_body<LOGN, false, NTT_NARROW, T, 1, false, SrcPlain, true, false, 0, -1, C>(lds, p, tab, tid, src[g]);
    } else if (tab.wide_d4) ntt_body<LOGN, false, NTT_WIDE_NEAR, T, 1, false, SrcPlain, true, false, 0, -1, C>(lds, p, tab, tid, src[g]);
    else ntt_body<LOGN, false, NTT_WIDE, T, 1, false, SrcPlain, true, false, 0, -1, C>(lds, p, tab, tid, src[g]);
}

template <int LOGN, int T, int C = 16>
__global__ __launch_bounds__(T, 4) void k_intt_tensor(const TensorJob *__restrict__ jobs, int limbs, size_t src_ps, size_t n_tensor,
                                                   u64 *__restrict__ plain, const NttTable *__restrict__ tabs,
                                                   const int *__restrict__ modmap, int period)
{
    constexpr int N = 1 << LOGN;
    __shared__ __attribute__((aligned(16))) u64 lds[lds_slots(N)];
    const int tid = threadIdx.x;
    size_t g = blockIdx.x;
    {
        const size_t pairs = n_tensor / 3, padded = (pairs + 7) / 8 * 24;
        if (g < padded) {
            const size_t blk = g / 24, rem = g - blk * 24, pl = rem >> 3, u = blk * 8 + (rem & 7);
            if (u >= pairs) return;
            const size_t jb = u / (size_t)limbs, e = u - jb * limbs;
            g = jb * 3 * limbs + pl * limbs + e;
        } else {
            g = n_tensor + (g - padded);
        }
    }
    const int mv = modmap[g % (size_t)period];
    const NttTable tab = tabs[mv & NTT_MAP_MASK];
    if (g >= n_tensor) {
        u64 *p = plain + (g - n_tensor) * N;
        if (mv & NTT_MAP_RAW) {
            if (tab.narrow) ntt_body<LOGN, true, NTT_NARROW, T, 0, true, SrcStaged, true, false, 0, -1, C>(lds, p, tab, tid, nullptr, SrcStaged());
            else if (tab.wide_d4) ntt_body<LOGN, true, NTT_WIDE_NEAR, T, 0, true, SrcStaged, true, false, 0, -1, C>(lds, p, tab, tid, nullptr, SrcStaged());
            else ntt_body<LOGN, true, NTT_WIDE, T, 0, true, SrcStaged, true, false, 0, -1, C>(lds, p, tab, tid, nullptr, SrcStaged());
        } else {
            if (tab.narrow) ntt_body<LOGN, true, NTT_NARROW, T, 0, false, SrcStaged, true, false, 0, -1, C>(lds, p, tab, tid, nullptr, SrcStaged());
            else if (tab.wide_d4) ntt_body<LOGN, true, NTT_WIDE_NEAR, T, 0, false, SrcStaged, true, false, 0, -1, C>(lds, p, tab, tid, nullptr, SrcStaged());
            else ntt_body<LOGN, true, NTT_WIDE, T, 0, false, SrcStaged, true, false, 0, -1, C>(lds, p, tab, tid, nullptr, SrcStaged());
        }
        return;
    }
    const size_t per = (size_t)3 * limbs, jb = g / per;
    const int r = (int)(g - jb * per), pl = r / limbs, e = r - pl * limbs;
    const TensorJob job = jobs[jb];
    const u64 *a0 = job.a + (size_t)e * N, *a1 = a0 + src_ps, *b0 = job.b + (size_t)e * N, *b1 = b0 + src_ps;
    const bool lazy = ntt_lazy_input_ok(tab, LOGN);
    SrcTensor ops;
    if (pl == 0) ops = SrcTensor{ a0, b0, nullptr, nullptr, lazy };
    else if (pl == 1) ops = SrcTensor{ a0, b1, a1, b0, lazy };
    else ops = SrcTensor{ a1, b1, nullptr, nullptr, lazy };
    u64 *p = job.d + (size_t)r * N;
    if (mv & NTT_MAP_RAW) {
        if (tab.narrow) ntt_body<LOGN, true, NTT_NARROW, T, 0, true, SrcTensor, true, false, 0, -1, C>(lds, p, tab, tid, nullptr, ops);
        else if (tab.wide_d4) ntt_body<LOGN, true, NTT_WIDE_NEAR, T, 0, true, SrcTensor, true, false, 0, -1, C>(lds, p, tab, tid, nullptr, ops);
        else ntt_body<LOGN, true, NTT_WIDE, T, 0, true, SrcTensor, true, false, 0, -1, C>(lds, p, tab, tid, nullptr, ops);
    } else {
        if (tab.narrow) ntt_body<LOGN, true, NTT_NARROW, T, 0, false, SrcTensor, true, false, 0, -1, C>(lds, p, tab, tid, nullptr, ops);
        else if (tab.wide_d4) ntt_body<LOGN, true, NTT_WIDE_NEAR, T, 0, false, SrcTensor, true, false, 0, -1, C>(lds, p, tab, tid, nullptr, ops);
        else ntt_body<LOGN, true, NTT_WIDE, T, 0, false, SrcTensor, true, false, 0, -1, C>(lds, p, tab, tid, nullptr, ops);
    }
}

template <class K> struct NttFormRow { int logn, threads, coeffs_per_lane, min_waves; K inv, fwd; };
template <class K, size_t R> static K form_kernel(const NttFormRow<K> (&rows)[R], int logn, const NttForm &f, bool inverse)
{
    for (const NttFormRow<K> &r : rows)
        if (r.logn == logn && r.threads == f.threads && r.coeffs_per_lane == f.coeffs_per_lane && r.min_waves == f.min_waves && (inverse ? r.inv : r.fwd))
            return inverse ? r.inv : r.fwd;
    throw_hip(hipErrorInvalidValue, __FILE__, __LINE__);
    return nullptr;
}

using GatherKernel = void (*)(const u64 *const *, u64 *, const NttTable *, const int *, int, int);
#define ROW(LN, T, C, W) { LN, T, C, W, nullptr, k_ntt_gather<LN, T, C, W> },
static const NttFormRow<GatherKernel> k_ntt_gather_forms[] = {
    ROW(13, 1024, 8, 4) ROW(12, 512, 8, 4) ROW(13, 1024, 8, 8)
    ROW(14, 1024, 16, 4) ROW(13, 512, 16, 4) ROW(12, 256, 16, 4) ROW(11, 128, 16, 4) ROW(10, 64, 16, 4) ROW(8, 64, 16, 4) ROW(6, 64, 16, 4)
};
#undef ROW
using TensorKernel = void (*)(const TensorJob *, int, size_t, size_t, u64 *, const NttTable *, const int *, int);
#define ROW(LN, T, C) { LN, T, C, 4, k_intt_tensor<LN, T, C>, nullptr },
static const NttFormRow<TensorKernel> k_intt_tensor_forms[] = {
    ROW(13, 1024, 8) ROW(12, 512, 8)
    ROW(14, 1024, 16) ROW(13, 512, 16) ROW(12, 256, 16) ROW(11, 128, 16) ROW(10, 64, 16) ROW(8, 64, 16) ROW(6, 64, 16)
};
#undef ROW
using NttKernel = void (*)(u64 *, const NttTable *, const int *, int, int);
#define ROW(LN, T, C, W) { LN, T, C, W, k_ntt<LN, true, T, C, W>, k_ntt<LN, false, T, C, W> },
static const NttFormRow<NttKernel> k_ntt_forms[] = {
    ROW(14, 1024, 16, 4)
    { 13, 1024, 8, 8, nullptr, k_ntt<13, false, 1024, 8, 8> },
    ROW(13, 1024, 8, 4) ROW(12, 512, 8, 4)
    ROW(13, 512, 16, 4) ROW(12, 256, 16, 4) ROW(11, 128, 16, 4) ROW(10, 64, 16, 4) ROW(8, 64, 16, 4) ROW(6, 64, 16, 4)
};
#undef ROW

static void launch_ntt_split(bool inverse, const u64 *const *src, u64 *data, size_t count, const NttTable *tabs, const int *modmap, int period,
                             hipStream_t st, const NttForm &f)
{
    const size_t n = (size_t)1 << SPLIT_LOGN;
    const dim3 g((unsigned)((n / 2 + EW_T - 1) / EW_T), (unsigned)count);
    if (!inverse) hipLaunchKernelGGL(k_ntt_first_stage, g, dim3(EW_T), 0, st, src, data, n, tabs, modmap, period);
    hipLaunchKernelGGL(form_kernel(k_ntt_forms, SPLIT_LOGN - 1, f, inverse), dim3((unsigned)(count * 2)), dim3(f.threads), 0, st,
                       data, tabs, modmap, period, 1);
    if (inverse) hipLaunchKernelGGL(k_ntt_last_stage, g, dim3(EW_T), 0, st, data, n, tabs, modmap, period);
}

void launch_ntt(int logn, bool inverse, u64 *data, size_t count, const NttTable *tabs, const int *modmap, int period,
                hipStream_t st, size_t latency_limbs, bool narrow)
{
    if (!count) return;
    const NttForm f = ntt_form(logn, inverse ? NTT_KIND_INVERSE : NTT_KIND_FORWARD, count, latency_limbs, narrow);
    if (f.split) launch_ntt_split(inverse, nullptr, data, count, tabs, modmap, period, st, f);
    else hipLaunchKernelGGL(form_kernel(k_ntt_forms, logn, f, inverse), dim3((unsigned)count), dim3(f.threads), 0, st, data, tabs, modmap, period, 0);
    KERNEL_CHECK();
}

void launch_ntt_gather(int logn, const u64 *const *src, u64 *data, size_t count, const NttTable *tabs, const int *modmap, int period,
                       hipStream_t st, bool nored, size_t latency_limbs, bool narrow)
{
    if (!count) return;
    const NttForm f = ntt_form(logn, NTT_KIND_GATHER, count, latency_limbs, narrow);
    if (f.split) launch_ntt_split(false, src, data, count, tabs, modmap, period, st, f);
    else hipLaunchKernelGGL(form_kernel(k_ntt_gather_forms, logn, f, false), dim3((unsigned)count), dim3(f.threads), 0, st, src, data, tabs, modmap, period, nored ? 1 : 0);
    KERNEL_CHECK();
}

void launch_intt_tensor(int logn, const TensorJob *jobs, int njobs, int limbs, size_t src_ps, u64 *plain, size_t n_plain,
                        const NttTable *tabs, const int *modmap, int period, hipStream_t st, size_t latency_limbs)
{
    const size_t n_tensor = (size_t)njobs * 3 * limbs;
    const size_t count = (n_tensor / 3 + 7) / 8 * 24 + n_plain;
    if (!(n_tensor + n_plain)) return;
    const NttForm f = ntt_form(logn, NTT_KIND_TENSOR, n_tensor + n_plain, latency_limbs, false);
    hipLaunchKernelGGL(form_kernel(k_intt_tensor_forms, logn, f, true), dim3((unsigned)count), dim3(f.threads), 0, st,
                       jobs, limbs, src_ps, n_tensor, plain, tabs, modmap, period);
    KERNEL_CHECK();
}

}
```

### apsu_amd/csrc/launch_behz.h

```cpp
#pragma once
#include <hip/hip_runtime.h>
#include "dev_consts.h"
#include "launch_ntt.h"

namespace apsu_he {

void launch_behz_ext(const DevLevel *lv, int L, int nB, const u64 *in, size_t in_stride, int polys, u64 *out, size_t n, int cts,
                     hipStream_t st);
bool launch_drop_behz_ext(const DevLevel *lv, int L, int nB, const u64 *in, size_t in_stride, int polys, u64 *out, size_t n, int cts,
                          hipStream_t st, bool raw = false);
void launch_tensor(const DevLevel *lv, const TensorJob *jobs, size_t n, int batch, hipStream_t st);
struct TensorConvJob { const u64 *a, *b; u64 *d; int sa, sb; };
void launch_tensor_conv(const DevLevel *lv, const TensorConvJob *jobs, size_t n, int njobs, hipStream_t st);
struct TensorSumJob { const u64 *a, *b; u64 *dq, *bs; int terms; int pad; };
void launch_tensor_sum(const DevLevel *lv, int E, const TensorSumJob *jobs, size_t n, int njobs, int e0, hipStream_t st);
struct FinishSumJob { const u64 *dq, *bs; u64 *out; int terms; int pad; };
void launch_behz_finish_sum(const DevLevel *lv, int L, int nB, const FinishSumJob *jobs, size_t n, int njobs, hipStream_t st);
struct FinishJob { const u64 *d; u64 *out; int terms; int pad; };
void launch_behz_finish(const DevLevel *lv, int L, int nB, const FinishJob *jobs, bool accumulate, size_t n, int njobs, hipStream_t st);
void launch_ks_inner(const DevKey *key, int L, const u64 *tdec, const u64 *rk, u64 *acc, size_t n, int batch,
                     hipStream_t st);
void launch_ks_moddown(const DevKey *key, int L, const u64 *acc, u64 *ct, size_t ct_stride, size_t n, int batch,
                       hipStream_t st, const DevLevel *lv = nullptr, u64 *ext = nullptr, int n_ext = 0, bool raw = false);
struct EpiJob { const u64 *ct; const u64 *add1; const u64 *add2; const u64 *a0; const u64 *mask; u64 *out;
                const u64 *ks_acc = nullptr; };
void launch_eval_epilogue(const DevLevel *levels, int lvl, const EpiJob *jobs, size_t ct_poly_stride, int clear_bits, size_t n,
                          int njobs, hipStream_t st, const DevKey *key = nullptr);
struct I0Job { const u64 *s; const u64 *v; u64 *acc; int terms; int store; };
void launch_i0_finish(const DevLevel *lv_low, const I0Job *jobs, size_t n, int njobs, hipStream_t st, bool raw = false);

}
```

### apsu_amd/csrc/launch_ntt.h

```cpp
#pragma once
#include <hip/hip_runtime.h>
#include "dev_consts.h"

namespace apsu_he {

void launch_ntt(int logn, bool inverse, u64 *data, size_t count, const NttTable *tabs, const int *modmap,
                int period, hipStream_t st, size_t latency_limbs, bool narrow);
void launch_ntt_gather(int logn, const u64 *const *src, u64 *data, size_t count, const NttTable *tabs, const int *modmap, int period,
                       hipStream_t st, bool nored, size_t latency_limbs, bool narrow);
struct TensorJob { const u64 *a, *b; u64 *d; };
void launch_intt_tensor(int logn, const TensorJob *jobs, int njobs, int limbs, size_t src_ps, u64 *plain, size_t n_plain,
                        const NttTable *tabs, const int *modmap, int period, hipStream_t st, size_t latency_limbs = 0);

}
```

### apsu_amd/csrc/mac_core.h

```cpp
#pragma once
#include <stddef.h>
#include "dev_consts.h"

namespace apsu_he {

constexpr int MAC_G = 4;
constexpr int MAC_C = 2;

struct MacJob {
    const u64 *pt[MAC_G];
    u64 *out[MAC_G];
    const u64 *pw;
    u32 cnt, ng;
    u32 pt_stride, pw_stride, pw_poly_stride;
    u32 out_poly_stride;
    u32 limb0, nl;
    u32 packed, pad;
};
struct TermJob { const u64 *pt; const u64 *pw; u64 *out; };

inline int mac_shift_of(u64 q) { return (64 - __builtin_clzll(q) + 1) / 2; }
inline u32 mac_chunk_of(u64 q)
{
    const u64 cap = (u64)1 << (63 - 2 * mac_shift_of(q)), c = cap > 2 ? cap - 1 : 2;
    return (u32)(c < (1u << 20) ? c : 1u << 20);
}
inline u32 mac_chunk_k_of(u64 q)
{
    const int s = mac_shift_of(q);
    const u64 capk = 2 * s + 2 < 64 ? (u64)1 << (62 - 2 * s) : 0, c = capk > 2 ? capk - 1 : 0;
    return (u32)(c < (1u << 20) ? c : 1u << 20);
}
inline u32 mac_mask_hi_of(u32 w, int s) { return w == 64 ? 0xffffffffu : (u32)(((u64)1 << (w - s)) - 1); }
inline bool mac_kara_usable(u64 q) { return mac_chunk_k_of(q) >= 7; }

#if defined(__HIP_DEVICE_COMPILE__)
#define MAC_KEEP(v) asm("" : "+v"(v))
#else
#define MAC_KEEP(v) do { } while (0)
#endif

HD u32 alignbit(u32 hi, u32 lo, u32 sh)
{
#if defined(__HIP_DEVICE_COMPILE__)
    return __builtin_amdgcn_alignbit(hi, lo, sh);
#else
    return (u32)((((u64)hi << 32) | lo) >> (sh & 31));
#endif
}

HD const u32 *packed_window(const void *slot, u32 row_off, size_t k, u32 kb, u32 &psh)
{
    const u32 bitoff = (u32)(k >> 1) * 2 * kb;
    psh = bitoff & 31;
    return reinterpret_cast<const u32 *>(static_cast<const char *>(slot) + row_off) + (bitoff >> 5);
}
HD void packed_shift(u64 w_lo, u64 w_hi, u32 psh, u64 &lo64, u64 &hi64)
{
    const u32 w0 = (u32)w_lo, w1 = (u32)(w_lo >> 32), w2 = (u32)w_hi, w3 = (u32)(w_hi >> 32);
    const u32 n0 = alignbit(w1, w0, psh), n1 = alignbit(w2, w1, psh), n2 = alignbit(w3, w2, psh), n3 = w3 >> psh;
    lo64 = (u64)n0 | ((u64)n1 << 32); hi64 = (u64)n2 | ((u64)n3 << 32);
}
#define PACKED_SECOND(lo64, hi64, kb) ((kb) == 64 ? (hi64) : (((lo64) >> (kb)) | ((hi64) << (64 - (kb)))))
HD void packed_pair(u64 w_lo, u64 w_hi, u32 psh, u32 kb, u64 &a0, u64 &a1)
{
    u64 lo64, hi64;
    packed_shift(w_lo, w_hi, psh, lo64, hi64);
    if (kb == 64) { a0 = lo64; a1 = hi64; }
    else { const u64 mask = ((u64)1 << kb) - 1; a0 = lo64 & mask; a1 = PACKED_SECOND(lo64, hi64, kb) & mask; }
}
HD u64 packed_coeff(const u32 *row, size_t c, u32 w)
{
    const size_t bit0 = c * w, d0 = bit0 >> 5;
    const u32 sh = (u32)(bit0 & 31);
    u64 v = ((u64)row[d0] | ((u64)row[d0 + 1] << 32)) >> sh;
    if (sh && w + sh > 64) v |= (u64)row[d0 + 2] << (64 - sh);
    return w == 64 ? v : (v & (((u64)1 << w) - 1));
}

#if defined(__HIPCC__)
#define MAC_LANE_FN __global__ __launch_bounds__(EW_T, 1) void
#define MAC_LANE_AT
#define MAC_LANE_AT_DEF const unsigned bx = blockIdx.x, by = blockIdx.y, bz = blockIdx.z, tx = threadIdx.x
#else
#define MAC_LANE_FN inline void
#define MAC_LANE_AT , unsigned bx, unsigned by, unsigned bz, unsigned tx
#define MAC_LANE_AT_DEF (void)0
#endif
template <bool KARA, bool PACKED>
MAC_LANE_FN k_mac(const DevLevel *__restrict__ lv, const MacJob *__restrict__ jobs, size_t n, int limb_slow MAC_LANE_AT)
{
    MAC_LANE_AT_DEF;
    constexpr int G = MAC_G, C = MAC_C;
    unsigned b_x = bx, b_limb = by, b_job = bz;
    if (limb_slow) { b_limb = bz; b_job = by; }
    const size_t k = ((size_t)b_x * EW_T + tx) * C;
    if (k >= n) return;
    const MacJob *__restrict__ jp = jobs + b_job;
    struct { const u64 *pw; u32 cnt, ng, pt_stride, pw_stride, pw_poly_stride, out_poly_stride, limb0; } job =
        { jp->pw, jp->cnt, jp->ng, jp->pt_stride, jp->pw_stride, jp->pw_poly_stride, jp->out_poly_stride, jp->limb0 };
    if ((int)job.ng <= 0 || b_limb >= jp->nl) return;
    const int j = b_limb + job.limb0;
    const Mod m = lv->q[j];
    const u32 s = lv->mac_shift[j], chunk = KARA ? lv->mac_chunk_k[j] : lv->mac_chunk[j];
    const u32 lomask = (1u << s) - 1;
    const u64 *p0 = job.pw + (size_t)j * n + k;
    const u64 *p1 = p0 + job.pw_poly_stride;
    const u64 *pt[G];
    const u32 *ptw[G];
    u32 psh = 0, kb = 64, himask = 0xffffffffu;
    if constexpr (PACKED) {
        kb = lv->mac_bits[j];
        himask = lv->mac_mask_hi[j];
#pragma unroll
        for (int g = 0; g < G; g++) ptw[g] = packed_window(jp->pt[g < (int)job.ng ? g : 0], lv->mac_row_off[j], k, kb, psh);
    } else {
#pragma unroll
        for (int g = 0; g < G; g++) pt[g] = jp->pt[g < (int)job.ng ? g : 0] + (size_t)j * n + k;
    }

    u64 s00[G][C][2], sx[G][C][2], s11[G][C][2];
#pragma unroll
    for (int g = 0; g < G; g++)
#pragma unroll
        for (int c = 0; c < C; c++)
#pragma unroll
            for (int p = 0; p < 2; p++) s00[g][c][p] = sx[g][c][p] = s11[g][c][p] = 0;

    struct Term { u64 c[2][C]; u64 a[G][C]; };
    auto load_term = [&](u32 i, Term &t) {
        const u64x2 v0 = ldg16(p0 + (size_t)i * job.pw_stride), v1 = ldg16(p1 + (size_t)i * job.pw_stride);
        t.c[0][0] = v0[0]; t.c[0][1] = v0[1]; t.c[1][0] = v1[0]; t.c[1][1] = v1[1];
#pragma unroll
        for (int g = 0; g < G; g++) {
            if constexpr (PACKED) {
                const u32x4a4 w = ldg16_a4_nt(ptw[g] + (size_t)i * (job.pt_stride >> 2));
                t.a[g][0] = (u64)w[0] | ((u64)w[1] << 32); t.a[g][1] = (u64)w[2] | ((u64)w[3] << 32);
            } else {
                const u64x2 a = ldg16_nt(pt[g] + (size_t)i * job.pt_stride);
                t.a[g][0] = a[0]; t.a[g][1] = a[1];
            }
        }
    };
    auto mac_term = [&](const Term &t) {
        u32 clo[2][C], chi[2][C];
#pragma unroll
        for (int p = 0; p < 2; p++)
#pragma unroll
            for (int c = 0; c < C; c++) { clo[p][c] = (u32)t.c[p][c] & lomask; chi[p][c] = (u32)(t.c[p][c] >> s); }
        u32 csum[2][C];
        if (KARA) {
#pragma unroll
            for (int p = 0; p < 2; p++)
#pragma unroll
                for (int c = 0; c < C; c++) csum[p][c] = clo[p][c] + chi[p][c];
        }
#pragma unroll
        for (int g = 0; g < G; g++) {
            u64 av[C];
            if constexpr (PACKED) {
                u64 hi64;
// ... 119 lines not shown
```

### apsu_amd/csrc/ntt_core.h

```cpp
#pragma once
#include <type_traits>

#include "modmath.h"

struct TwPair { u64 w, wq; };

struct NttTable {
    u64 q;
    u64 ninv, ninv_q;
    u64 r1;
    const TwPair *fwd;
    const TwPair *dit;
    const TwPair *scale;
    int narrow;
    u32 fold_k, fold_c;
    u32 wide_d4;
    u64 r0;
};

HD bool ntt_is_narrow(u64 q, int logn) { return (unsigned __int128)q * (unsigned)(4 * logn + 1) < ((unsigned __int128)1 << 64); }

HD bool ntt_gather_nored_ok(u64 q, u64 max_src, int logn)
{
    return ntt_is_narrow(q, logn) && (unsigned __int128)q * (unsigned)(4 * logn) + max_src <= ((unsigned __int128)1 << 64);
}

HD void ntt_fold_params(u64 q, u32 &k, u32 &c)
{
    int bits = 0;
    while (bits < 64 && (q >> bits)) bits++;
    k = 0; c = 0;
    if (bits < 33 || bits > 62) return;
    const u64 cc = ((u64)1 << bits) - q;
    if (cc >> 32) return;
    if ((unsigned __int128)((((u64)1) << (64 - bits)) + 2) * cc > ((unsigned __int128)1 << bits)) return;
    k = (u32)bits; c = (u32)cc;
}

HD u32 ntt_wide_d4(u64 q, bool narrow)
{
    if (narrow || (q >> 61)) return 0;
    const u64 q4 = q << 2;
    if (q4 >= ((u64)1 << 63)) return 0;
    const u64 d = ((u64)1 << 63) - q4;
    return (d >> 32) ? 0 : (u32)d;
}

HD u64 ntt_reduce_any(u64 x, const NttTable &tab)
{
    if (tab.fold_k) {
        const u32 sh = tab.fold_k - 32;
        const u32 hi = (u32)(x >> 32);
        const u64 low = ((u64)(hi & ((1u << sh) - 1)) << 32) | (u32)x;
        const u64 v = (u64)(hi >> sh) * tab.fold_c + low;
        return v >= tab.q ? v - tab.q : v;
    }
    const u64 v = x - mulhi64(x, tab.r1) * tab.q;
    return v >= tab.q ? v - tab.q : v;
}

HD bool ntt_fold128_ok(u32 fold_k, u32 fold_c) { return fold_k >= 44 && fold_k <= 61 && fold_c < (1u << 24); }
HD u64 ntt_reduce128_fold(u64 hi, u64 lo, const NttTable &tab)
{
    const u32 k = tab.fold_k, c = tab.fold_c, s = k - 32;
    const u64 pl = lo & (((u64)1 << k) - 1);
    const u64 ph = (hi << (64 - k)) | (lo >> k);
    const u64 a = (u64)(u32)ph * c;
    const u64 t = (u64)(u32)(ph >> 32) * c;
    const u64 w = pl + a + (u64)(u32)(t >> s) * c + ((t & (((u64)1 << s) - 1)) << 32);
    return ntt_reduce_any(w, tab);
}

HD u64 ntt_reduce128(u64 hi, u64 lo, const NttTable &tab)
{
    if (ntt_fold128_ok(tab.fold_k, tab.fold_c)) return ntt_reduce128_fold(hi, lo, tab);
    return barrett128(u128p{ lo, hi }, Mod{ tab.q, tab.r0, tab.r1 });
}
HD u64 ntt_lazy_bound_q(const NttTable &tab)
{
    const u64 c = tab.fold_c;
    return 5 + ((((c << 32) + 4 * c * c)) >> (tab.fold_k - 1));
}
constexpr int plan_passes(int logn, int c);
constexpr int plan_k(int logn, int p, int c);
HD bool ntt_lazy_input_ok(const NttTable &tab, int logn)
{
    if (!ntt_fold128_ok(tab.fold_k, tab.fold_c)) return false;
    if (!tab.narrow) return true;
    const int k16 = plan_k(logn, plan_passes(logn, 16) - 1, 16);
    const u64 mult = (ntt_lazy_bound_q(tab) << k16) + (u64)(4 * (logn - k16));
    return (unsigned __int128)tab.q * mult < ((unsigned __int128)1 << 64);
}
HD u64 ntt_reduce128_lazy(u64 hi, u64 lo, const NttTable &tab)
{
    const u32 k = tab.fold_k, c = tab.fold_c, s = k - 32;
    const u64 pl = lo & (((u64)1 << k) - 1);
    const u64 ph = (hi << (64 - k)) | (lo >> k);
    const u64 a = (u64)(u32)ph * c;
    const u64 t = (u64)(u32)(ph >> 32) * c;
    return pl + a + (u64)(u32)(t >> s) * c + ((t & (((u64)1 << s) - 1)) << 32);
}

struct SrcPlain {};
struct SrcStaged {};
struct SrcTensor { const u64 *x0, *y0, *x1, *y1; bool lazy; };
HD u64x2 src_load2(const SrcPlain &, const u64 *glob, int e, const NttTable &) { return *reinterpret_cast<const u64x2 *>(glob + e); }
HD u64 src_load1(const SrcPlain &, const u64 *glob, int e, const NttTable &) { return glob[e]; }
HD u64x2 src_load2(const SrcStaged &, const u64 *glob, int e, const NttTable &) { return *reinterpret_cast<const u64x2 *>(glob + e); }
HD u64 src_load1(const SrcStaged &, const u64 *glob, int e, const NttTable &) { return glob[e]; }
HD u64x2 src_load2(const SrcTensor &s, const u64 *, int e, const NttTable &tab)
{
    const u64x2 x = ldg16(s.x0 + e), y = ldg16(s.y0 + e);
    u128p p0 = mul128(x[0], y[0]), p1 = mul128(x[1], y[1]);
    if (s.x1) {
        const u64x2 u = ldg16(s.x1 + e), v = ldg16(s.y1 + e);
        mac128(p0, u[0], v[0]);
        mac128(p1, u[1], v[1]);
    }
    u64x2 r;
    if (s.lazy) {
        r[0] = ntt_reduce128_lazy(p0.hi, p0.lo, tab);
        r[1] = ntt_reduce128_lazy(p1.hi, p1.lo, tab);
    } else {
        r[0] = ntt_reduce128(p0.hi, p0.lo, tab);
        r[1] = ntt_reduce128(p1.hi, p1.lo, tab);
    }
    return r;
}
HD u64 src_load1(const SrcTensor &s, const u64 *, int e, const NttTable &tab)
{
    u128p p = mul128(s.x0[e], s.y0[e]);
    if (s.x1) mac128(p, s.x1[e], s.y1[e]);
    return s.lazy ? ntt_reduce128_lazy(p.hi, p.lo, tab) : ntt_reduce128(p.hi, p.lo, tab);
}
HD u64 src_in_bound(const SrcPlain &, const NttTable &) { return 1; }
HD u64 src_in_bound(const SrcStaged &, const NttTable &) { return 1; }
HD u64 src_in_bound(const SrcTensor &s, const NttTable &tab) { return s.lazy ? ntt_lazy_bound_q(tab) : 1; }
HD int lds_slot(int e) { return e + ((e >> 4) << 1); }
constexpr int lds_slots(int n) { return n + (n >> 3); }

#if defined(__HIP_DEVICE_COMPILE__)
#define UNIFORM_INT(x) __builtin_amdgcn_readfirstlane(x)
#else
#define UNIFORM_INT(x) (x)
#endif

HD u64 mul_lazy4(u64 x, u64 w, u64 wq, u64 nq)
{
    const u32 x0 = (u32)x, x1 = (u32)(x >> 32), a0 = (u32)wq, a1 = (u32)(wq >> 32);
    const u64 t1 = (u64)x1 * a0, t2 = (u64)x0 * a1;
    const u64 h = (u64)x1 * a1 + (t1 >> 32) + (t2 >> 32);
    const u32 h0 = (u32)h, h1 = (u32)(h >> 32), w0 = (u32)w, w1 = (u32)(w >> 32), n0 = (u32)nq, n1 = (u32)(nq >> 32);
    const u64 lo = (u64)x0 * w0 + (u64)h0 * n0;
    const u64 mid = (u64)x0 * w1 + (u64)x1 * w0 + (u64)h0 * n1 + (u64)h1 * n0;
    return lo + (mid << 32);
}

#if defined(__HIP_DEVICE_COMPILE__)
template <bool SB> __device__ __forceinline__ u64 ntt_mad64(u32 a, u32 b, u64 c)
{
    u64 d;
    unsigned long long carry;
    if constexpr (SB) asm("v_mad_u64_u32 %0, %1, %2, %3, %4" : "=v"(d), "=s"(carry) : "v"(a), "s"(b), "v"(c));
    else asm("v_mad_u64_u32 %0, %1, %2, %3, %4" : "=v"(d), "=s"(carry) : "v"(a), "v"(b), "v"(c));
    return d;
}
#endif
template <bool UNI = false, bool CHAIN = false>
HD void bfly_lazy4(u64 &x, u64 &y, u64 w, u64 wq, u64 nq, u64 q4)
{
    const u32 y0 = (u32)y, y1 = (u32)(y >> 32), a0 = (u32)wq, a1 = (u32)(wq >> 32);
    const u64 t1 = (u64)y1 * a0, t2 = (u64)y0 * a1;
    const u64 h = (u64)y1 * a1 + (t1 >> 32) + (t2 >> 32);
    const u32 h0 = (u32)h, h1 = (u32)(h >> 32), w0 = (u32)w, w1 = (u32)(w >> 32), n0 = (u32)nq, n1 = (u32)(nq >> 32);
    const u64 lo = (u64)h0 * n0 + ((u64)y0 * w0 + x);
    u64 s;
#if defined(__HIP_DEVICE_COMPILE__)
    if constexpr (CHAIN) {
        u64 acc = lo >> 32;
        acc = ntt_mad64<UNI>(y0, w1, acc);
        acc = ntt_mad64<UNI>(y1, w0, acc);
        acc = ntt_mad64<true>(h0, n1, acc);
        acc = ntt_mad64<true>(h1, n0, acc);
        s = (u64)(u32)lo | (acc << 32);
    } else
#endif
    {
        const u32 mid = y0 * w1 + y1 * w0 + h0 * n1 + h1 * n0;
        s = lo + ((u64)mid << 32);
    }
    y = ((x << 1) + q4) - s;
    x = s;
}

HD u64 csub_top(u64 x, u64 n4) { return x + ((u64)((int64_t)x >> 63) & n4); }
HD u64 csub_top_near(u64 x, u32 d4)
{
    const u32 hi = (u32)(x >> 32);
    const u64 low = ((u64)(hi & 0x7fffffffu) << 32) | (u32)x;
    return (u64)(hi >> 31) * d4 + low;
}

enum PassIo { IO_LDS = 0, IO_GLOBAL = 1 };
enum NttMode { NTT_NARROW = 0, NTT_WIDE = 1, NTT_WIDE_NEAR = 2 };
HD int ntt_mode(const NttTable &tab) { return tab.narrow ? NTT_NARROW : (tab.wide_d4 ? NTT_WIDE_NEAR : NTT_WIDE); }

template <int LOGN, int S, int K, bool INV, int C = 16> struct PassShape {
    static constexpr int R = 1 << K, G = C >> K, LOWBITS = LOGN - S - K;
    static constexpr bool COLS = (1 << LOWBITS) >= G;
    static constexpr int CG = COLS ? ((1 << LOWBITS) / G) : 1;
    static constexpr int GM = INV ? (COLS ? G : 1) : (COLS ? 1 : G);
    static constexpr int NT = (R - 1) * GM;
    static constexpr int fwd_slot(int u, int j, int g) { return ((1 << u) - 1) * GM + (j >> (K - u)) * GM + (COLS ? 0 : g); }
    static constexpr int inv_slot(int bit, int j, int gg) { return (bit - 1) * GM + (j & (bit - 1)) * GM + (COLS ? gg : 0); }
};
struct TwInline {};
template <int NT> struct TwRegs { u64x2 t[NT > 0 ? NT : 1]; };
struct NoHook { HD void operator()() const {} };

template <int LOGN, int S, int K, bool INV, int C = 16>
HD void ntt_load_twiddles(TwRegs<PassShape<LOGN, S, K, INV, C>::NT> &tw, int w, const NttTable &tab)
{
    using PS = PassShape<LOGN, S, K, INV, C>;
    constexpr int R = PS::R, G = PS::G, LOWBITS = PS::LOWBITS, CG = PS::CG;
    constexpr bool COLS = PS::COLS;
    constexpr bool UNIFORM_TW = COLS && (CG % 64 == 0);
    int block, c0;
    if (COLS) { block = w / CG; c0 = (w % CG) * G; }
    else { block = w * G; c0 = 0; }
#pragma unroll
    for (int uu = 0; uu < K; uu++) {
        const int u = INV ? K - 1 - uu : uu;
        const int bit = 1 << (K - 1 - u);
        if (INV) {
#pragma unroll
            for (int jl = 0; jl < bit; jl++)
#pragma unroll
                for (int gg = 0; gg < PS::GM; gg++) {
                    const int jj = COLS ? ((jl << LOWBITS) | (c0 + gg)) : jl;
                    const int gap = COLS ? (bit << LOWBITS) : bit;
                    tw.t[PS::inv_slot(bit, jl, gg)] = ldg16(reinterpret_cast<const u64 *>(tab.dit + gap + jj));
                }
        } else {
#pragma unroll
            for (int jh = 0; jh < (1 << u); jh++)
#pragma unroll
                for (int g = 0; g < PS::GM; g++) {
                    int ti = (1 << (S + u)) + ((COLS ? block : block + g) << u) + jh;
                    if (UNIFORM_TW) ti = UNIFORM_INT(ti);
                    tw.t[PS::fwd_slot(u, jh << (K - u), g)] = ldg16(reinterpret_cast<const u64 *>(tab.fwd + ti));
                }
        }
    }
    (void)R;
}

template <int LOGN, int S, int K, bool INV, int MODE, int IN, int OUT, int RED = 0, bool RAW = false, class SRC = SrcPlain,
          class TW = TwInline, class HOOK = NoHook, int C = 16>
HD void ntt_pass16(u64 *lds, u64 *__restrict__ glob, int w, const NttTable &tab, const SRC &src = SRC(), const TW &tw = TW(),
                   const HOOK &hook = HOOK())
{
    using PS = PassShape<LOGN, S, K, INV, C>;
    static_assert((C == 16 || C == 8 || C == 4) && (1 << K) <= C, "radix 2^K on C coefficients per work item");
    constexpr bool PRE = !std::is_same<TW, TwInline>::value;
    constexpr int R = 1 << K;
    constexpr int G = C >> K;
    constexpr int LOWBITS = LOGN - S - K;
    constexpr bool COLS = (1 << LOWBITS) >= G;
    constexpr int CG = COLS ? ((1 << LOWBITS) / G) : 1;
    constexpr bool UNIFORM_TW = COLS && (CG % 64 == 0);
    const TwPair *__restrict__ W = tab.fwd;
    const u64 q = tab.q, nq = (u64)0 - q, q4 = q << 2, n4 = (u64)0 - q4;
    const u32 d4 = tab.wide_d4;
    constexpr bool TRIV_WIDE1 = INV && MODE != NTT_NARROW && LOWBITS == 0 && std::is_same<SRC, SrcTensor>::value;
    const u64 qb0 = ((INV && MODE == NTT_NARROW && LOWBITS == 0) || TRIV_WIDE1) ? q * src_in_bound(src, tab) : 0;

    int block, c0;
    if (COLS) { block = w / CG; c0 = (w % CG) * G; }
    else { block = w * G; c0 = 0; }
    auto idx = [&](int g, int j) -> int {
        return COLS ? ((block << (LOGN - S)) | (j << LOWBITS) | (c0 + g)) : (((block + g) << K) | j);
    };

    constexpr bool PAIR_G = COLS && G >= 2;
    constexpr bool PAIR_J = !PAIR_G && LOWBITS == 0;
    u64 r[G][R];
    if (PAIR_G) {
#pragma unroll
        for (int j = 0; j < R; j++)
#pragma unroll
            for (int g = 0; g < G; g += 2) {
                const int e = idx(g, j);
                const u64x2 v = (IN == IO_GLOBAL) ? src_load2(src, glob, e, tab)
                                                   : *reinterpret_cast<const u64x2 *>(lds + lds_slot(e));
                r[g][j] = v[0]; r[g + 1][j] = v[1];
            }
    } else if (PAIR_J) {
#pragma unroll
        for (int g = 0; g < G; g++)
#pragma unroll
            for (int j = 0; j < R; j += 2) {
                const int e = idx(g, j);
                const u64x2 v = (IN == IO_GLOBAL) ? src_load2(src, glob, e, tab)
                                                   : *reinterpret_cast<const u64x2 *>(lds + lds_slot(e));
                r[g][j] = v[0]; r[g][j + 1] = v[1];
            }
    } else {
#pragma unroll
        for (int g = 0; g < G; g++)
#pragma unroll
            for (int j = 0; j < R; j++) {
                const int e = idx(g, j);
                r[g][j] = (IN == IO_GLOBAL) ? src_load1(src, glob, e, tab) : lds[lds_slot(e)];
            }
    }

    if (RED == 1 && IN == IO_GLOBAL) {
#pragma unroll
        for (int g = 0; g < G; g++)
#pragma unroll
            for (int j = 0; j < R; j++) r[g][j] = ntt_reduce_any(r[g][j], tab);
    }

#pragma unroll
    for (int uu = 0; uu < K; uu++) {
        const int u = INV ? K - 1 - uu : uu;
        const int bit = 1 << (K - 1 - u);
#pragma unroll
        for (int j = 0; j < R; j++) {
            if (j & bit) continue;
#pragma unroll
            for (int g = 0; g < G; g++) {
                if (COLS && g > 0) continue;
                if (INV) {
#pragma unroll
                    for (int gg = 0; gg < G; gg++) {
                        if (!COLS && gg != g) continue;
                        const int jj = COLS ? (((j & (bit - 1)) << LOWBITS) | (c0 + gg)) : (j & (bit - 1));
                        const int gap = COLS ? (bit << LOWBITS) : bit;
                        u64x2 tv;
                        if constexpr (PRE) tv = tw.t[PS::inv_slot(bit, j, gg)];
                        else tv = ldg16(reinterpret_cast<const u64 *>(tab.dit + gap + jj));
                        u64 &x = r[gg][j], &y = r[gg][j | bit];
                        if (((MODE == NTT_NARROW && LOWBITS == 0) || (TRIV_WIDE1 && bit == 1)) && (j & (bit - 1)) == 0) {
                            const u64 M = qb0 * (u64)bit, sum = x + y;
                            y = x + M - y;
                            x = sum;
                            continue;
                        }
                        if (MODE == NTT_WIDE) x = csub_top(x, n4);
                    if (MODE == NTT_WIDE_NEAR) x = csub_top_near(x, d4);
                        bfly_lazy4(x, y, tv[0], tv[1], nq, q4);
                    }
                    continue;
                }
                int ti = (1 << (S + u)) + (((COLS ? block : block + g)) << u) + (j >> (K - u));
                if (UNIFORM_TW) ti = UNIFORM_INT(ti);
                u64x2 tv;
                if constexpr (PRE) tv = tw.t[PS::fwd_slot(u, j, g)];
                else tv = ldg16(reinterpret_cast<const u64 *>(W + ti));
                const TwPair t{ tv[0], tv[1] };
#pragma unroll
                for (int gg = 0; gg < G; gg++) {
                    if (!COLS && gg != g) continue;
                    u64 &x = r[gg][j], &y = r[gg][j | bit];
                    if (MODE == NTT_WIDE) x = csub_top(x, n4);
                    if (MODE == NTT_WIDE_NEAR) x = csub_top_near(x, d4);
                    bfly_lazy4<UNIFORM_TW && !PRE, true>(x, y, t.w, t.wq, nq, q4);
                }
            }
        }
    }

    hook();
    if (OUT == IO_GLOBAL && !(INV && RAW)) {
#pragma unroll
        for (int g = 0; g < G; g++)
#pragma unroll
            for (int j = 0; j < R; j++) {
                u64 v = r[g][j];
                if (INV) {
                    const u64x2 sv = ldg16(reinterpret_cast<const u64 *>(tab.scale + idx(g, j)));
                    v = mul_shoup(v, sv[0], sv[1], q);
                } else v = ntt_reduce_any(v, tab);
                r[g][j] = v;
            }
    }
    if (PAIR_G) {
#pragma unroll
        for (int j = 0; j < R; j++)
#pragma unroll
            for (int g = 0; g < G; g += 2) {
                const int e = idx(g, j);
                u64x2 v; v[0] = r[g][j]; v[1] = r[g + 1][j];
                if (OUT == IO_GLOBAL) *reinterpret_cast<u64x2 *>(glob + e) = v;
                else *reinterpret_cast<u64x2 *>(lds + lds_slot(e)) = v;
            }
    } else if (PAIR_J) {
#pragma unroll
        for (int g = 0; g < G; g++)
#pragma unroll
            for (int j = 0; j < R; j += 2) {
                const int e = idx(g, j);
                u64x2 v; v[0] = r[g][j]; v[1] = r[g][j + 1];
                if (OUT == IO_GLOBAL) *reinterpret_cast<u64x2 *>(glob + e) = v;
                else *reinterpret_cast<u64x2 *>(lds + lds_slot(e)) = v;
            }
    } else {
#pragma unroll
        for (int g = 0; g < G; g++)
#pragma unroll
            for (int j = 0; j < R; j++) {
                const int e = idx(g, j);
                if (OUT == IO_GLOBAL) glob[e] = r[g][j];
                else lds[lds_slot(e)] = r[g][j];
            }
    }
}

template <int MODE>
HD u64 ntt_fwd_finish(u64 v, const NttTable &tab)
{
    return ntt_reduce_any(v, tab);
}

constexpr int plan_passes(int logn, int c = 16)
{
    if (c == 8) return logn == 13 ? 5 : logn == 12 ? 4 : 0;
    return logn == 14 ? 4 : logn == 13 ? 4 : logn == 12 ? 4 : logn == 11 ? 4 : logn == 10 ? 3 : logn == 8 ? 3 : logn == 6 ? 2 : 0;
}
constexpr int plan_k(int logn, int p, int c = 16)
{
    if (c == 8) {
        switch (logn) {
        case 13: return (p == 0 || p == 4) ? 2 : 3;
        case 12: return 3;
        default: return 0;
        }
    }
    switch (logn) {
    case 14: return p >= 2 ? 4 : 3;
    case 13: return p == 3 ? 4 : 3;
    case 12: return 3;
    case 11: return p == 3 ? 2 : 3;
    case 10: return p == 2 ? 4 : 3;
    case 8:  return p == 2 ? 2 : 3;
    case 6:  return 3;
    default: return 0;
    }
}
constexpr int plan_s(int logn, int p, int c = 16)
{
    int s = 0;
    for (int i = 0; i < p; i++) s += plan_k(logn, i, c);
    return s;
}
constexpr bool plan_has_latency_form(int logn) { return plan_passes(logn, 8) > 0; }

template <int LOGN, bool INV, int PASS, int C = 16> struct ExecPass {
    static constexpr int P = plan_passes(LOGN, C), p = INV ? P - 1 - PASS : PASS, K = plan_k(LOGN, p, C), S = plan_s(LOGN, p, C);
    using Shape = PassShape<LOGN, S, K, INV, C>;
    using Tw = TwRegs<Shape::NT>;
};
template <int LOGN, bool INV, int PASS, int C = 16>
HD void ntt_pass_twiddles(typename ExecPass<LOGN, INV, PASS, C>::Tw &tw, int tid, const NttTable &tab)
{
    using E = ExecPass<LOGN, INV, PASS, C>;
    ntt_load_twiddles<LOGN, E::S, E::K, INV, C>(tw, tid, tab);
}

template <int LOGN, bool INV, int MODE, int PASS, int RED = 0, bool RAW = false, class SRC = SrcPlain, bool STAGED = false,
          class TW = TwInline, class HOOK = NoHook, int C = 16>
HD void ntt_pass(u64 *lds, u64 *glob, int tid, int T, const NttTable &tab, const SRC &src = SRC(), const TW &tw = TW(),
                 const HOOK &hook = HOOK())
{
    constexpr int P = plan_passes(LOGN, C);
    constexpr int p = INV ? P - 1 - PASS : PASS;
    constexpr int K = plan_k(LOGN, p, C);
    constexpr int S = plan_s(LOGN, p, C);
    constexpr int IN = (PASS == 0 && !STAGED) ? IO_GLOBAL : IO_LDS;
    constexpr int OUT = (INV && PASS == P - 1) ? IO_GLOBAL : IO_LDS;
    constexpr int LOGC = C == 16 ? 4 : C == 8 ? 3 : 2;
    for (int w = tid; w < (1 << (LOGN - LOGC)); w += T)
        ntt_pass16<LOGN, S, K, INV, MODE, IN, OUT, RED, RAW, SRC, TW, HOOK, C>(lds, glob, w, tab, src, tw, hook);
}
```

### apsu_amd/csrc/ntt_wg.h

```cpp
#pragma once
#include <type_traits>

#include "ntt_core.h"

#if defined(__HIPCC__)

template <int LOGN, int T, int C = 16> constexpr bool ntt_wave_private(int p) { return T == 64 || (LOGN - plan_s(LOGN, p, C) <= (C == 16 ? 10 : C == 8 ? 9 : 8)); }

template <bool WAVE> __device__ __forceinline__ void ntt_sync()
{
    if constexpr (WAVE) {
        __builtin_amdgcn_fence(__ATOMIC_RELEASE, "wavefront");
        __builtin_amdgcn_wave_barrier();
        __builtin_amdgcn_fence(__ATOMIC_ACQUIRE, "wavefront");
    } else __syncthreads();
}

__device__ __forceinline__ void ntt_touch_line(const void *line, unsigned &sink)
{
    asm volatile("global_load_dword %0, %1, off" : "=v"(sink) : "v"(line));
}
__device__ __forceinline__ void ntt_touch_done(unsigned &sink) { asm volatile("s_waitcnt vmcnt(0)" : "+v"(sink)); }

template <int LOGN, bool INV, int MODE, int T, int RED = 0, bool RAW = false, class SRC = SrcPlain, bool WS = true, bool PF = false, int STAGGER = 0,
// ... 17 lines not shown
    if constexpr (NEXTPASS == 0) { if (next) ntt_touch_line(next, sink); }
    if constexpr (STAGGER > 0 && INV) { if (tid & 256) __builtin_amdgcn_s_sleep(STAGGER); }
    if constexpr (PF && P > 1) {
        constexpr bool COMPUTED = !std::is_same<SRC, SrcPlain>::value;
        constexpr bool PF_LAST = !(INV && !RAW);
        constexpr bool ON1 = P > 2 || PF_LAST, ON2 = P > 2 && (P > 3 || PF_LAST), ON3 = P > 3 && PF_LAST;
        std::conditional_t<ON1, typename ExecPass<LOGN, INV, 1>::Tw, TwInline> t1;
        std::conditional_t<ON2, typename ExecPass<LOGN, INV, (P > 2 ? 2 : 1)>::Tw, TwInline> t2;
        std::conditional_t<ON3, typename ExecPass<LOGN, INV, (P > 3 ? 3 : 1)>::Tw, TwInline> t3;
        auto h1 = [&]() { if constexpr (ON1) ntt_pass_twiddles<LOGN, INV, 1>(t1, tid, tab); };
        auto h2 = [&]() { if constexpr (ON2) ntt_pass_twiddles<LOGN, INV, 2>(t2, tid, tab); };
        auto h3 = [&]() { if constexpr (ON3) ntt_pass_twiddles<LOGN, INV, 3>(t3, tid, tab); };
        if constexpr (RED != 0) ntt_pass<LOGN, INV, MODE, 0, RED, false, SrcPlain, false, TwInline, decltype(h1)>(lds, const_cast<u64 *>(src), tid, T, tab, SrcPlain(), TwInline(), h1);
        else if constexpr (COMPUTED) {
            constexpr bool WL = WS && ntt_wave_private<LOGN, T>(fp(0));
            if constexpr (WL) {
#pragma unroll
                for (int i = 0; i < 8; i++) {
                    const int e = wbase + 128 * i + 2 * lane;
                    if (e < N) *reinterpret_cast<u64x2 *>(lds + lds_slot(e)) = src_load2(operands, p, e, tab);
                }
            } else {
                for (int e = 2 * tid; e < N; e += 2 * T) *reinterpret_cast<u64x2 *>(lds + lds_slot(e)) = src_load2(operands, p, e, tab);
            }
            ntt_sync<WL>();
            ntt_pass<LOGN, INV, MODE, 0, 0, false, SRC, true, TwInline, decltype(h1)>(lds, p, tid, T, tab, operands, TwInline(), h1);
        } else ntt_pass<LOGN, INV, MODE, 0, 0, false, SrcPlain, false, TwInline, decltype(h1)>(lds, p, tid, T, tab, SrcPlain(), TwInline(), h1);
        ntt_sync<W1>();
        ntt_pass<LOGN, INV, MODE, 1, 0, RAW, SrcPlain, false, decltype(t1), decltype(h2)>(lds, p, tid, T, tab, SrcPlain(), t1, h2);
        if constexpr (P > 2) { ntt_sync<W2>(); ntt_pass<LOGN, INV, MODE, 2, 0, RAW, SrcPlain, false, decltype(t2), decltype(h3)>(lds, p, tid, T, tab, SrcPlain(), t2, h3); }
        if constexpr (P > 3) { ntt_sync<W3>(); ntt_pass<LOGN, INV, MODE, 3, 0, RAW, SrcPlain, false, decltype(t3)>(lds, p, tid, T, tab, SrcPlain(), t3); }
    } else {
    if constexpr (RED != 0) ntt_pass<LOGN, INV, MODE, 0, RED, false, SrcPlain, false, TwInline, NoHook, C>(lds, const_cast<u64 *>(src), tid, T, tab);
    else if constexpr (!std::is_same<SRC, SrcPlain>::value) {
        constexpr bool WL = WS && ntt_wave_private<LOGN, T, C>(fp(0));
        if constexpr (WL) {
#pragma unroll
            for (int i = 0; i < WCO; i++) {
                const int e = wbase + 128 * i + 2 * lane;
                if (e < N) *reinterpret_cast<u64x2 *>(lds + lds_slot(e)) = src_load2(operands, p, e, tab);
            }
        } else {
            for (int e = 2 * tid; e < N; e += 2 * T) *reinterpret_cast<u64x2 *>(lds + lds_slot(e)) = src_load2(operands, p, e, tab);
        }
        ntt_sync<WL>();
        ntt_pass<LOGN, INV, MODE, 0, 0, false, SRC, true, TwInline, NoHook, C>(lds, p, tid, T, tab, operands);
    } else ntt_pass<LOGN, INV, MODE, 0, 0, false, SrcPlain, false, TwInline, NoHook, C>(lds, p, tid, T, tab);
    if constexpr (P > 1) {
        ntt_sync<W1>();
        if constexpr (STAGGER > 0 && !INV) { if (tid & 256) __builtin_amdgcn_s_sleep(STAGGER); }
        if constexpr (NEXTPASS == 1) { if (next) ntt_touch_line(next, sink); }
        ntt_pass<LOGN, INV, MODE, 1, 0, RAW, SrcPlain, false, TwInline, NoHook, C>(lds, p, tid, T, tab);
    }
    if constexpr (P > 2) { ntt_sync<W2>(); if constexpr (NEXTPASS == 2) { if (next) ntt_touch_line(next, sink); } ntt_pass<LOGN, INV, MODE, 2, 0, RAW, SrcPlain, false, TwInline, NoHook, C>(lds, p, tid, T, tab); }
    if constexpr (P > 3) { ntt_sync<W3>(); if constexpr (NEXTPASS == 3) { if (next) ntt_touch_line(next, sink); } ntt_pass<LOGN, INV, MODE, 3, 0, RAW, SrcPlain, false, TwInline, NoHook, C>(lds, p, tid, T, tab); }
    if constexpr (P > 4) { ntt_sync<W4>(); ntt_pass<LOGN, INV, MODE, 4, 0, RAW, SrcPlain, false, TwInline, NoHook, C>(lds, p, tid, T, tab); }
    }
    if constexpr (!INV) {
        constexpr bool WF = WS && ntt_wave_private<LOGN, T, C>(P - 1);
        ntt_sync<WF>();
        if constexpr (WF) {
#pragma unroll
            for (int i = 0; i < WCO; i++) {
                const int e = wbase + 128 * i + 2 * lane;
                if (e < N) {
                    u64x2 v = *reinterpret_cast<const u64x2 *>(lds + lds_slot(e));
                    v[0] = ntt_fwd_finish<MODE>(v[0], tab);
                    v[1] = ntt_fwd_finish<MODE>(v[1], tab);
                    *reinterpret_cast<u64x2 *>(p + e) = v;
                }
            }
        } else {
            for (int e = 2 * tid; e < N; e += 2 * T) {
                u64x2 v = *reinterpret_cast<const u64x2 *>(lds + lds_slot(e));
                v[0] = ntt_fwd_finish<MODE>(v[0], tab);
                v[1] = ntt_fwd_finish<MODE>(v[1], tab);
                *reinterpret_cast<u64x2 *>(p + e) = v;
            }
        }
    }
    if constexpr (NEXTPASS >= 0) { if (next) ntt_touch_done(sink); }
}

#endif
```

### apsu_amd/engine.py

```python
import collections
import ctypes as C
import json
import os

import numpy as np

_HERE = os.path.dirname(os.path.abspath(__file__))
_LIB = None
u64p = C.POINTER(C.c_uint64)


class ApsuHeError(RuntimeError):
    pass


class _Info(C.Structure):
    _fields_ = [
        ("poly_modulus_degree", C.c_uint64), ("plain_modulus", C.c_uint64),
        ("coeff_modulus_size", C.c_int32), ("first_chain_idx", C.c_int32),
        ("using_keyswitching", C.c_int32), ("irrelevant_bit_count", C.c_int32),
        ("coeff_modulus", C.c_uint64 * 8),
        ("ps_low_degree", C.c_uint32), ("max_items_per_bin", C.c_uint32),
        ("bundle_idx_count", C.c_uint32), ("items_per_bundle", C.c_uint32),
        ("source_power_count", C.c_uint32), ("target_power_count", C.c_uint32),
# ... 50 lines not shown
def _p(a):
    assert isinstance(a, np.ndarray) and a.dtype == np.uint64 and a.flags["C_CONTIGUOUS"], "need contiguous uint64"
    return a.ctypes.data_as(u64p)


def _ptr_array(items):
    arr = (C.c_void_p * len(items))()
    for i, it in enumerate(items):
        arr[i] = it.ctypes.data if isinstance(it, np.ndarray) else int(it)
    return arr


def _update_lists(inserts, removes):
    nb = max(len(inserts or []), len(removes or []))
    args, keep = [], []
    for lists in (inserts, removes):
        if lists is None:
            args += [None, None, 0]
            continue
        stride = max([len(b) for b in lists] + [1])
        roots = np.zeros((max(nb, 1), stride), dtype=np.uint64)
        counts = np.zeros(max(nb, 1), dtype=np.uint32)
        for i, b in enumerate(lists):
            counts[i] = len(b)
            roots[i, :len(b)] = b
        keep += [roots, counts]
        args += [_p(roots), C.c_void_p(counts.ctypes.data), stride]
    return args, keep, nb


def _entries(entries, felts_per_item):
    if isinstance(entries, tuple) and len(entries) == 2 and isinstance(entries[0], np.ndarray) and entries[0].ndim == 2:
        felts, start = entries
    else:
        entries = list(entries if entries is not None else [])
        felts = [[int(v) for v in f] for _, f in entries]
        start = [int(s) for s, _ in entries]
    felts = np.ascontiguousarray(felts, dtype=np.uint64).reshape(-1, felts_per_item)
    start = np.ascontiguousarray(start, dtype=np.uint32).reshape(-1)
    if len(felts) != len(start):
        raise ValueError("entries: felts and start bins differ in length")
    return felts, start


NOT_A_BIN = 0xFFFFFFFF


def _bins_stride(counts):
    held = counts[counts != NOT_A_BIN]
    return max(int(held.max()) if held.size else 0, 1)


def _bins_list(roots, counts):
    return [None if c == NOT_A_BIN else roots[s, :int(c)].copy() for s, c in enumerate(counts)]
ENTRY_INSERTED, ENTRY_DUPLICATE, ENTRY_REMOVED, ENTRY_NOT_FOUND = 0, 1, 2, 3
BUNDLE_UNCHANGED, BUNDLE_REPLACED, BUNDLE_EMPTY = 0, 1, 2
ApplyResult = collections.namedtuple("ApplyResult", "state bundles appended ins_status ins_target rem_status rem_target")
CompactResult = collections.namedtuple("CompactResult", "group merged")
BundleInfo = collections.namedtuple("BundleInfo", "slot bundle_idx cache_idx degree")
MultiApplyResult = collections.namedtuple("MultiApplyResult", "new_id n_appended ins_status ins_target rem_status rem_target")


class _SelfTestReport(C.Structure):
    _fields_ = [("bundles", C.c_uint32), ("reserved", C.c_uint32), ("slots", C.c_uint64), ("mismatches", C.c_uint64),
                ("first_bundle", C.c_int32), ("first_slot", C.c_uint32), ("first_got", C.c_uint64), ("first_expected", C.c_uint64),
                ("min_budget_bits", C.c_int32), ("min_budget_bundle", C.c_int32), ("he_ms", C.c_double), ("plain_ms", C.c_double)]


SelfTestReport = collections.namedtuple("SelfTestReport", "bundles slots mismatches first_mismatch min_budget min_budget_bundle he_ms plain_ms")


class _StepArgs(C.Structure):
    _fields_ = [("step", C.c_int32), ("chain_idx", C.c_int32), ("flags", C.c_uint32), ("terms", C.c_int32), ("polys", C.c_int32),
                ("batch", C.c_int32), ("e0", C.c_int32), ("n_ext", C.c_int32), ("inp", u64p * 6), ("in_words", C.c_size_t * 6),
                ("out", u64p * 2), ("out_words", C.c_size_t * 2)]


STEPS = {name: i for i, name in enumerate((
    "level_info", "behz_ext", "drop_behz_ext", "tensor", "tensor_conv", "tensor_sum", "behz_finish", "behz_finish_sum", "ks_inner",
    "ks_moddown", "modswitch", "modswitch_jobs", "i0_finish", "eval_epilogue", "add_many", "sum_jobs", "add_plain", "dyadic_plain", "lift",
    "polyn_with_roots", "bins_update", "bin_counts", "poly_degree", "bins_lookup", "bins_merge", "bins_rows", "bins_eval", "eval_compare", "roots",
    "unlift", "ntt_info", "ntt", "ntt_gather", "intt_tensor", "roots_split",
    "seed_expand", "decrypt_round", "plain_powers", "sample_small", "small_lift", "enc_finish", "rlk_finish", "flag_monomial",
    "mac_info", "mac", "term_product", "pack_rows", "unpack_rows", "limb0_rows", "entries_scatter"))}
STEP_RAW, STEP_ACCUMULATE, STEP_STORE, STEP_KEY, STEP_PLAN, STEP_COMPOSED, STEP_INVERSE, STEP_NORED = 1, 2, 4, 8, 16, 32, 64, 128
STEP_KARA, STEP_PACKED, STEP_LIMB_SLOW = 256, 512, 1024
STEP_MAP_RAW = 1 << 30


def _self_test_report(r):
    first = None if r.first_bundle < 0 else (int(r.first_bundle), int(r.first_slot), int(r.first_got), int(r.first_expected))
    return SelfTestReport(int(r.bundles), int(r.slots), int(r.mismatches), first, int(r.min_budget_bits),
                          None if r.min_budget_bundle < 0 else int(r.min_budget_bundle), float(r.he_ms), float(r.plain_ms))


class RelinKeys:
    def __init__(self, ctx, handle):
        self._ctx, self.h = ctx, handle

    def __del__(self):
        try:
            if self.h:
                load_library().apsu_he_relin_free(self.h)
        except Exception:
            pass


class Bundle:

    def __init__(self, ctx, handle, bundle_idx, cache_idx, degree):
        self._ctx, self.h = ctx, handle
        self.bundle_idx, self.cache_idx, self.degree = bundle_idx, cache_idx, degree

    @property
    def db_bytes(self):
        v = C.c_uint64()
        _check(load_library().apsu_he_bundle_bytes(self.h, C.byref(v)))
        return v.value

    def __del__(self):
        try:
            if self.h:
                load_library().apsu_he_bundle_free(self.h)
        except Exception:
            pass


class Powers:

    def __init__(self, ctx, handle, bundle_indices):
        self._ctx, self.h, self.bundle_indices = ctx, handle, list(bundle_indices)

    def download(self, bundle_idx, power):
        ctx = self._ctx
        sz = ctx.power_size(power)
        buf = np.empty(sz * (ctx.first_chain_idx + 1) * ctx.n, dtype=np.uint64)
        ci, ntt = C.c_int(), C.c_int()
        _check(load_library().apsu_he_powers_download(ctx.h, self.h, bundle_idx, power, _p(buf), C.c_size_t(buf.size),
                                                     C.byref(ci), C.byref(ntt)))
        L = ci.value + 1
        return buf[: sz * L * ctx.n].reshape(sz, L, ctx.n).copy(), ci.value, bool(ntt.value)

    def __del__(self):
        try:
            if self.h:
                load_library().apsu_he_powers_free(self.h)
        except Exception:
            pass


class HeContext:

    def __init__(self, psu_params_json=None, device=0, n=None, coeff_modulus=None, plain_modulus=None):
        L = load_library()
        h = C.c_void_p()
        if psu_params_json is not None:
            if os.path.exists(psu_params_json):
                with open(psu_params_json) as f:
                    psu_params_json = f.read()
            _check(L.apsu_he_create(psu_params_json.encode(), device, C.byref(h)))
            js = json.loads(psu_params_json)
            self.felts_per_item = int(js["item_params"]["felts_per_item"])
            self.table_size = int(js["table_params"]["table_size"])
            self.hash_func_count = int(js["table_params"]["hash_func_count"])
        else:
            self.felts_per_item = self.table_size = self.hash_func_count = 0
            q = np.array(coeff_modulus, dtype=np.uint64)
# ... 966 lines not shown
```

### include/apsu_he.h

```cpp
#ifndef APSU_HE_H
#define APSU_HE_H

#include <stddef.h>
#include <stdint.h>

#ifdef __cplusplus
extern "C" {
#endif

typedef enum {
    APSU_HE_OK = 0,
    APSU_HE_INVALID_ARGUMENT = -1,
    APSU_HE_LOGIC_ERROR = -2,
    APSU_HE_RUNTIME_ERROR = -3,
    APSU_HE_NO_DEVICE = -4,
    APSU_HE_OUT_OF_MEMORY = -5
} apsu_he_status;

typedef struct apsu_he_ctx apsu_he_ctx;
typedef struct apsu_he_relin apsu_he_relin;
typedef struct apsu_he_bundle apsu_he_bundle;
typedef struct apsu_he_powers apsu_he_powers;

typedef struct {
// ... 2 lines not shown
    int32_t coeff_modulus_size;
    int32_t first_chain_idx;
    int32_t using_keyswitching;
    int32_t irrelevant_bit_count;
    uint64_t coeff_modulus[8];
    uint32_t ps_low_degree, max_items_per_bin, bundle_idx_count, items_per_bundle;
    uint32_t source_power_count, target_power_count, powers_dag_depth;
    uint32_t result_polys;
} apsu_he_info;

typedef struct { uint32_t power, depth, parent1, parent2; } apsu_he_dag_node;

const char *apsu_he_last_error(void);
#define APSU_HE_ABI_VERSION 7
int apsu_he_abi_version(void);

int apsu_he_create(const char *psu_params_json, int device, apsu_he_ctx **out);
int apsu_he_create_raw(uint64_t poly_modulus_degree, const uint64_t *coeff_modulus, int coeff_modulus_size,
                       uint64_t plain_modulus, int device, apsu_he_ctx **out);
int apsu_he_destroy(apsu_he_ctx *ctx);
int apsu_he_get_info(const apsu_he_ctx *ctx, apsu_he_info *out);
int apsu_he_get_powers_dag(const apsu_he_ctx *ctx, apsu_he_dag_node *nodes, int capacity, int *n_nodes);

int apsu_he_transform_to_ntt(apsu_he_ctx *ctx, uint64_t *ct, int polys, int chain_idx);
int apsu_he_transform_from_ntt(apsu_he_ctx *ctx, uint64_t *ct, int polys, int chain_idx);
int apsu_he_transform_plain_to_ntt(apsu_he_ctx *ctx, const uint64_t *pt_mod_t, size_t pt_coeff_count, uint64_t *out,
                                   int chain_idx);
int apsu_he_multiply_plain_ntt(apsu_he_ctx *ctx, const uint64_t *ct, const uint64_t *pt_ntt, uint64_t *out, int polys,
                               int chain_idx);
int apsu_he_multiply_plain(apsu_he_ctx *ctx, const uint64_t *ct, const uint64_t *pt_mod_t, size_t pt_coeff_count,
                           uint64_t *out, int polys, int chain_idx);
int apsu_he_add(apsu_he_ctx *ctx, uint64_t *acc, const uint64_t *x, int polys, int chain_idx);
int apsu_he_add_plain(apsu_he_ctx *ctx, uint64_t *ct, const uint64_t *pt_mod_t, size_t pt_coeff_count, int chain_idx);
int apsu_he_multiply(apsu_he_ctx *ctx, const uint64_t *a, const uint64_t *b, uint64_t *out3, int chain_idx);
int apsu_he_square(apsu_he_ctx *ctx, const uint64_t *a, uint64_t *out3, int chain_idx);
int apsu_he_multiply_sized(apsu_he_ctx *ctx, const uint64_t *a, int size_a, const uint64_t *b, int size_b, uint64_t *out, int chain_idx);
int apsu_he_relinearize(apsu_he_ctx *ctx, uint64_t *ct3, const apsu_he_relin *rk, int chain_idx);
int apsu_he_mod_switch_to_next(apsu_he_ctx *ctx, uint64_t *ct, int polys, int chain_idx);
int apsu_he_clear_irrelevant_bits(apsu_he_ctx *ctx, uint64_t *ct_last_level, int polys);

int apsu_he_relin_upload(apsu_he_ctx *ctx, const uint64_t *ksk, apsu_he_relin **out);
int apsu_he_relin_free(apsu_he_relin *rk);
int apsu_he_db_upload_bundle(apsu_he_ctx *ctx, uint32_t bundle_idx, uint32_t cache_idx, uint32_t n_coeffs,
                             const uint64_t *const *coeff_ptrs, const uint8_t *is_ntt, apsu_he_bundle **out);
int apsu_he_db_random_bundle(apsu_he_ctx *ctx, uint32_t bundle_idx, uint32_t cache_idx, uint32_t degree, uint64_t seed,
                             apsu_he_bundle **out);
int apsu_he_db_build_bundle(apsu_he_ctx *ctx, uint32_t bundle_idx, uint32_t cache_idx, const uint64_t *roots,
                            const uint32_t *counts, uint32_t bins, uint32_t stride, apsu_he_bundle **out);
int apsu_he_bundle_update(apsu_he_ctx *ctx, const apsu_he_bundle *old, const uint64_t *ins_roots, const uint32_t *ins_counts,
                          uint32_t ins_stride, const uint64_t *rem_roots, const uint32_t *rem_counts, uint32_t rem_stride,
                          uint32_t bins, apsu_he_bundle **out);
#define APSU_HE_NOT_A_BIN 0xFFFFFFFFu
enum { APSU_HE_ENTRY_INSERTED = 0, APSU_HE_ENTRY_DUPLICATE = 1, APSU_HE_ENTRY_REMOVED = 2, APSU_HE_ENTRY_NOT_FOUND = 3 };
enum { APSU_HE_BUNDLE_UNCHANGED = 0, APSU_HE_BUNDLE_REPLACED = 1, APSU_HE_BUNDLE_EMPTY = 2 };
int apsu_he_bundle_bin_counts(apsu_he_ctx *ctx, const apsu_he_bundle *bundle, uint32_t *counts);
int apsu_he_bundles_lookup(apsu_he_ctx *ctx, const apsu_he_bundle *const *bundles, uint32_t n_bundles, const uint64_t *felts,
                           const uint32_t *start_bins, size_t count, uint8_t *present, uint32_t *room);
int apsu_he_db_apply_entries(apsu_he_ctx *ctx, uint32_t bundle_idx, const apsu_he_bundle *const *bundles, uint32_t n_bundles,
                             const uint64_t *ins_felts, const uint32_t *ins_start, size_t n_ins, const uint64_t *rem_felts,
                             const uint32_t *rem_start, size_t n_rem, uint32_t *bundle_state, apsu_he_bundle **replaced,
                             apsu_he_bundle **appended, uint32_t *n_appended, uint32_t *ins_status, uint32_t *ins_target,
                             uint32_t *rem_status, uint32_t *rem_target);
int apsu_he_debug_lookup_times(apsu_he_ctx *ctx, double *decode_ms, double *kernels_ms);
int apsu_he_db_entries_plan(const apsu_he_ctx *ctx, const uint64_t *offsets, uint32_t *bundles_per_index, uint32_t *total);
int apsu_he_db_build_from_entries(apsu_he_ctx *ctx, const uint8_t *entries, int entries_on_device, const uint64_t *offsets,
                                  apsu_he_bundle **out, uint32_t capacity, uint32_t *n_out);
int apsu_he_debug_build_from_entries_times(apsu_he_ctx *ctx, double *copy_ms, double *scatter_ms, double *build_ms);
int apsu_he_debug_set_scatter_blocks(apsu_he_ctx *ctx, uint32_t blocks);
int apsu_he_bundle_bins(apsu_he_ctx *ctx, const apsu_he_bundle *bundle, uint64_t *roots, uint32_t *counts, uint32_t stride);
int apsu_he_debug_bundle_bins_form(apsu_he_ctx *ctx, const apsu_he_bundle *bundle, uint64_t *roots, uint32_t *counts, uint32_t stride, int form);
int apsu_he_debug_bins_times(apsu_he_ctx *ctx, double *decode_ms, double *roots_ms, double *mult_ms);
enum { APSU_HE_STEP_LEVEL_INFO = 0, APSU_HE_STEP_BEHZ_EXT, APSU_HE_STEP_DROP_BEHZ_EXT, APSU_HE_STEP_TENSOR, APSU_HE_STEP_TENSOR_CONV,
       APSU_HE_STEP_TENSOR_SUM, APSU_HE_STEP_BEHZ_FINISH, APSU_HE_STEP_BEHZ_FINISH_SUM, APSU_HE_STEP_KS_INNER, APSU_HE_STEP_KS_MODDOWN,
       APSU_HE_STEP_MODSWITCH, APSU_HE_STEP_MODSWITCH_JOBS, APSU_HE_STEP_I0_FINISH, APSU_HE_STEP_EVAL_EPILOGUE, APSU_HE_STEP_ADD_MANY,
       APSU_HE_STEP_SUM_JOBS, APSU_HE_STEP_ADD_PLAIN, APSU_HE_STEP_DYADIC_PLAIN, APSU_HE_STEP_LIFT,
       APSU_HE_STEP_POLYN_WITH_ROOTS, APSU_HE_STEP_BINS_UPDATE, APSU_HE_STEP_BIN_COUNTS, APSU_HE_STEP_POLY_DEGREE, APSU_HE_STEP_BINS_LOOKUP,
       APSU_HE_STEP_BINS_MERGE, APSU_HE_STEP_BINS_ROWS, APSU_HE_STEP_BINS_EVAL, APSU_HE_STEP_EVAL_COMPARE, APSU_HE_STEP_ROOTS, APSU_HE_STEP_UNLIFT,
       APSU_HE_STEP_NTT_INFO, APSU_HE_STEP_NTT, APSU_HE_STEP_NTT_GATHER, APSU_HE_STEP_INTT_TENSOR,
       APSU_HE_STEP_ROOTS_SPLIT,
       APSU_HE_STEP_SEED_EXPAND, APSU_HE_STEP_DECRYPT_ROUND, APSU_HE_STEP_PLAIN_POWERS, APSU_HE_STEP_SAMPLE_SMALL, APSU_HE_STEP_SMALL_LIFT,
       APSU_HE_STEP_ENC_FINISH, APSU_HE_STEP_RLK_FINISH, APSU_HE_STEP_FLAG_MONOMIAL,
       APSU_HE_STEP_MAC_INFO, APSU_HE_STEP_MAC, APSU_HE_STEP_TERM_PRODUCT, APSU_HE_STEP_PACK_ROWS, APSU_HE_STEP_UNPACK_ROWS,
       APSU_HE_STEP_LIMB0_ROWS,
       APSU_HE_STEP_ENTRIES_SCATTER };
enum { APSU_HE_STEP_RAW = 1, APSU_HE_STEP_ACCUMULATE = 2, APSU_HE_STEP_STORE = 4, APSU_HE_STEP_KEY = 8, APSU_HE_STEP_PLAN = 16,
       APSU_HE_STEP_COMPOSED = 32, APSU_HE_STEP_INVERSE = 64, APSU_HE_STEP_NORED = 128, APSU_HE_STEP_KARA = 256, APSU_HE_STEP_PACKED = 512,
       APSU_HE_STEP_LIMB_SLOW = 1024 };
#define APSU_HE_STEP_MAP_RAW ((uint64_t)1 << 30)
typedef struct {
    int32_t step, chain_idx;
    uint32_t flags;
    int32_t terms, polys, batch, e0, n_ext;
    const uint64_t *in[6];
    size_t in_words[6];
    uint64_t *out[2];
    size_t out_words[2];
} apsu_he_step_args;
int apsu_he_debug_run_step(apsu_he_ctx *ctx, const apsu_he_step_args *args);
int apsu_he_bundles_merge(apsu_he_ctx *ctx, const apsu_he_bundle *const *bundles, uint32_t n_bundles, uint32_t cache_idx,
                          apsu_he_bundle **out);
int apsu_he_db_compact(apsu_he_ctx *ctx, uint32_t bundle_idx, const apsu_he_bundle *const *bundles, uint32_t n_bundles, uint32_t *group,
                       apsu_he_bundle **merged, uint32_t *n_merged);
int apsu_he_bundle_split(apsu_he_ctx *ctx, const apsu_he_bundle *b, uint32_t parts, const uint32_t *cache_idx, apsu_he_bundle **out);
int apsu_he_bundle_adopt(apsu_he_ctx *dst, apsu_he_ctx *src, const apsu_he_bundle *b, uint32_t cache_idx, apsu_he_bundle **out);
int apsu_he_db_rebase(apsu_he_ctx *dst, apsu_he_ctx *src, const apsu_he_bundle *const *bundles, uint32_t n_bundles, apsu_he_bundle **out,
                      uint32_t *origin, uint32_t *cache_idx, uint32_t capacity, uint32_t *n_out);
int apsu_he_debug_split_times(apsu_he_ctx *ctx, double *decode_ms, double *roots_ms, double *split_ms, double *build_ms);
int apsu_he_debug_merge_times(apsu_he_ctx *ctx, double *decode_ms, double *kernel_ms, double *encode_ms);
int apsu_he_bundle_image_size(apsu_he_ctx *ctx, const apsu_he_bundle *b, uint64_t *bytes);
int apsu_he_bundle_save(apsu_he_ctx *ctx, const apsu_he_bundle *b, uint8_t *buf, uint64_t capacity, uint64_t *written);
int apsu_he_bundle_load(apsu_he_ctx *ctx, const uint8_t *buf, uint64_t size, apsu_he_bundle **out);
int apsu_he_mask_generate(apsu_he_ctx *ctx, uint64_t seed, uint32_t count, uint64_t *masks_dev, uint64_t *values, uint64_t *blocks);
int apsu_he_mask_generate_blake2xb(apsu_he_ctx *ctx, const uint64_t seed[8], uint64_t first_value, uint32_t count, uint64_t *masks_dev,
                                   uint64_t *values, uint64_t *blocks);
int apsu_he_decrypt_decode(apsu_he_ctx *ctx, const uint64_t *sk_ntt, const uint64_t *cts, int cts_on_device, uint32_t count,
                           uint64_t *values, uint64_t *blocks);
int apsu_he_keygen(apsu_he_ctx *ctx, const uint64_t seed[8], uint64_t *sk_ntt);
int apsu_he_relin_keygen(apsu_he_ctx *ctx, const uint64_t *sk_ntt, const uint64_t seed[8], uint64_t *ksk, uint64_t *key_seeds, apsu_he_relin **out);
int apsu_he_query_create(apsu_he_ctx *ctx, const uint64_t *sk_ntt, const uint64_t seed[8], const uint32_t *bundle_indices, int n_bundle_idx,
                         const uint64_t *values, int values_on_device, uint64_t *cts_dev, uint64_t *ct_seeds);
int apsu_he_decrypt_decode_budget(apsu_he_ctx *ctx, const uint64_t *sk_ntt, const uint64_t *cts, int cts_on_device, uint32_t count,
                                  uint64_t *values, uint64_t *blocks, int32_t *budget_bits);
int apsu_he_algebraize_items(apsu_he_ctx *ctx, const uint8_t *items, size_t count, int items_on_device, uint64_t *felts, int felts_on_device);
int apsu_he_item_locations(apsu_he_ctx *ctx, const uint8_t *items, size_t count, int items_on_device, uint32_t *locs, int locs_on_device);
int apsu_he_items_bucket(apsu_he_ctx *ctx, const uint8_t *items, size_t count, int items_on_device, uint64_t *offsets, uint32_t *order,
                         uint64_t *total);
int apsu_he_cuckoo_table(apsu_he_ctx *ctx, const uint8_t *items, size_t count, int items_on_device, uint64_t max_rounds, uint32_t *table_idx,
                         uint32_t *item_loc, uint64_t *rounds);
int apsu_he_query_values(apsu_he_ctx *ctx, const uint8_t *table_items, int table_items_on_device, uint64_t *values, int values_on_device);
int apsu_he_debug_item_locations(apsu_he_ctx *ctx, const uint8_t *items, size_t count, uint32_t hash_func_count, uint32_t table_size,
                                 uint32_t *locs);
int apsu_he_debug_cuckoo_insert(apsu_he_ctx *ctx, const uint8_t *items, const uint32_t *locs, size_t count, uint32_t hash_func_count,
                                uint32_t table_size, uint64_t max_rounds, int form, uint32_t *table_idx, uint32_t *item_loc, uint64_t *rounds);
typedef struct {
    uint32_t bundles, reserved;
    uint64_t slots, mismatches;
    int32_t first_bundle;
    uint32_t first_slot;
    uint64_t first_got, first_expected;
    int32_t min_budget_bits, min_budget_bundle;
    double he_ms, plain_ms;
} apsu_he_self_test_report;
int apsu_he_bundles_eval_plain(apsu_he_ctx *ctx, const apsu_he_bundle *const *bundles, uint32_t n_bundles, const uint64_t *x, int x_on_device,
                               const uint64_t *masks, int masks_on_device, uint64_t *out, int out_on_device, uint8_t *is_bin);
int apsu_he_debug_eval_plain_times(apsu_he_ctx *ctx, double *decode_ms, double *counts_ms, double *kernel_ms);
int apsu_he_db_self_test(apsu_he_ctx *ctx, const apsu_he_bundle *const *bundles, uint32_t count, const uint64_t seed[8], const uint64_t *x,
                         apsu_he_self_test_report *report);
int apsu_he_debug_self_test_times(apsu_he_ctx *ctx, double *ms5);
typedef struct apsu_he_db_file apsu_he_db_file;
int apsu_he_db_file_save(apsu_he_ctx *ctx, const char *path, const apsu_he_bundle *const *bundles, int count);
int apsu_he_db_file_open(const char *path, apsu_he_db_file **out);
int apsu_he_db_file_close(apsu_he_db_file *f);
int apsu_he_db_file_count(const apsu_he_db_file *f, int *count, uint64_t *file_bytes);
int apsu_he_db_file_entry(const apsu_he_db_file *f, int i, uint32_t *bundle_idx, uint32_t *cache_idx, uint32_t *degree, uint64_t *image_bytes);
int apsu_he_db_file_load(apsu_he_ctx *ctx, const apsu_he_db_file *f, int i, apsu_he_bundle **out);
int apsu_he_bundle_degree(const apsu_he_bundle *b, uint32_t *degree);
int apsu_he_bundle_download(apsu_he_ctx *ctx, const apsu_he_bundle *b, uint32_t degree, uint64_t *out, size_t capacity_words,
                            size_t *words, int *kind);
int apsu_he_power_size(const apsu_he_ctx *ctx, uint32_t power, uint32_t *polys);
int apsu_he_bundle_result_size(const apsu_he_ctx *ctx, const apsu_he_bundle *b, uint32_t *polys);
int apsu_he_bundle_free(apsu_he_bundle *b);
int apsu_he_bundle_bytes(const apsu_he_bundle *b, uint64_t *db_bytes);
int apsu_he_compute_powers(apsu_he_ctx *ctx, const uint32_t *bundle_indices, int n_bundle_idx,
                           const uint64_t *const *src_cts, int src_on_device, const apsu_he_relin *rk,
                           apsu_he_powers **out);
int apsu_he_powers_free(apsu_he_powers *p);
int apsu_he_powers_download(apsu_he_ctx *ctx, const apsu_he_powers *p, uint32_t bundle_idx, uint32_t power,
// ... 188 lines not shown
```

Before: 3.180 ms.

## Fuse last-limb term products with inverse NTT and summed rounding for i0

Adds a k_intt_terms path that, for each bundle, loops over a group of terms. For each term it loads the last-limb row times the low power as the NTT source, runs the inverse NTT passes in LDS, and accumulates the rounded result in a sink. It emits one partial sum per group, so the per-term vlast buffer and the separate term-product plus batched INTT launches are no longer needed. i0_finish then consumes these group partials instead of l per-term polys. This cuts workspace traffic and launches. In exchange, each workgroup runs sequential INTTs per term, which may limit parallelism, and the path is enabled by default behind new switches.

Result: no change. 3.162 ms (median of 6 runs) (-0.6%).

```diff
diff --git a/apsu_amd/csrc/c_api.cpp b/apsu_amd/csrc/c_api.cpp
--- a/apsu_amd/csrc/c_api.cpp
+++ b/apsu_amd/csrc/c_api.cpp
@@ -402,7 +402,7 @@
 {
     return guarded([&] {
         REQUIRE(c && args, "null argument");
-        static_assert((int)APSU_HE_STEP_LIFT == (int)Engine::STEP_LIFT && (int)APSU_HE_STEP_UNLIFT == (int)Engine::STEP_UNLIFT && (int)APSU_HE_STEP_INTT_TENSOR == (int)Engine::STEP_INTT_TENSOR && (int)APSU_HE_STEP_ROOTS_SPLIT == (int)Engine::STEP_ROOTS_SPLIT && (int)APSU_HE_STEP_SEED_EXPAND == (int)Engine::STEP_SEED_EXPAND && (int)APSU_HE_STEP_FLAG_MONOMIAL == (int)Engine::STEP_FLAG_MONOMIAL && (int)APSU_HE_STEP_MAC_INFO == (int)Engine::STEP_MAC_INFO && (int)APSU_HE_STEP_LIMB0_ROWS == (int)Engine::STEP_LIMB0_ROWS && (int)APSU_HE_STEP_ENTRIES_SCATTER + 1 == (int)Engine::STEP_COUNT && (int)APSU_HE_STEP_KEY == (int)Engine::STEP_KEY &&
+        static_assert((int)APSU_HE_STEP_LIFT == (int)Engine::STEP_LIFT && (int)APSU_HE_STEP_UNLIFT == (int)Engine::STEP_UNLIFT && (int)APSU_HE_STEP_INTT_TENSOR == (int)Engine::STEP_INTT_TENSOR && (int)APSU_HE_STEP_ROOTS_SPLIT == (int)Engine::STEP_ROOTS_SPLIT && (int)APSU_HE_STEP_SEED_EXPAND == (int)Engine::STEP_SEED_EXPAND && (int)APSU_HE_STEP_FLAG_MONOMIAL == (int)Engine::STEP_FLAG_MONOMIAL && (int)APSU_HE_STEP_MAC_INFO == (int)Engine::STEP_MAC_INFO && (int)APSU_HE_STEP_LIMB0_ROWS == (int)Engine::STEP_LIMB0_ROWS && (int)APSU_HE_STEP_ENTRIES_SCATTER == (int)Engine::STEP_ENTRIES_SCATTER && (int)APSU_HE_STEP_INTT_TERMS + 1 == (int)Engine::STEP_COUNT && (int)APSU_HE_STEP_KEY == (int)Engine::STEP_KEY &&
                       (int)APSU_HE_STEP_KARA == (int)Engine::STEP_KARA && (int)APSU_HE_STEP_PACKED == (int)Engine::STEP_PACKED && (int)APSU_HE_STEP_LIMB_SLOW == (int)Engine::STEP_LIMB_SLOW &&
                       (int)APSU_HE_STEP_COMPOSED == (int)Engine::STEP_COMPOSED && (int)APSU_HE_STEP_NORED == (int)Engine::STEP_NORED, "step ids of the header and the engine");
         Engine::StepArgs a{};
diff --git a/apsu_amd/csrc/dev_consts.cpp b/apsu_amd/csrc/dev_consts.cpp
--- a/apsu_amd/csrc/dev_consts.cpp
+++ b/apsu_amd/csrc/dev_consts.cpp
@@ -255,10 +255,12 @@
     flag("APSU_HE_EVAL_PER_TERM", s.force_per_term);
     flag("APSU_HE_SEED_EXPAND_HOST", s.seed_expand_host);
     flag("APSU_HE_FUSE_TAIL", s.fuse_tail);
+    flag("APSU_HE_I0_FUSED", s.i0_fused);
     size("APSU_HE_EVAL_WS_BYTES", s.eval_ws_bytes);
     size("APSU_HE_ARENA_BYTES", s.arena_bytes);
     size("APSU_HE_NTT_LATENCY_LIMBS", s.ntt_latency_limbs);
     size("APSU_HE_SEED_REJ_CAP", s.seed_rej_cap);
+    size("APSU_HE_I0_GROUP", s.i0_group);
     return s;
 }
 
diff --git a/apsu_amd/csrc/dev_consts.h b/apsu_amd/csrc/dev_consts.h
--- a/apsu_amd/csrc/dev_consts.h
+++ b/apsu_amd/csrc/dev_consts.h
@@ -129,6 +129,8 @@
     bool seed_expand_host = false;
     size_t seed_rej_cap = SEED_REJ_CAP;
     bool fuse_tail = true;
+    bool i0_fused = true;
+    size_t i0_group = 0;
     size_t ntt_latency_limbs = NTT_FORM_AUTO;
 };
 EngineSwitches read_switches();
diff --git a/apsu_amd/csrc/emu_i0/i0.cpp b/apsu_amd/csrc/emu_i0/i0.cpp
--- /dev/null
+++ b/apsu_amd/csrc/emu_i0/i0.cpp
@@ -0,0 +1,86 @@
+#include <stdexcept>
+#include <vector>
+
+#include "../emu/emu_common.h"
+#include "../emu/ntt_driver.h"
+#include "eval_plan.h"
+#include "dev_consts.h"
+
+using namespace apsu_he;
+
+namespace apsu_he {
+
+template <int LOGN, int MODE, int C, int PASS = 0>
+void emu_terms_passes(u64 *lds, const NttTable &tab, int T, const SrcTerm &ops, u64 *acc)
+{
+    constexpr int P = plan_passes(LOGN, C);
+    if constexpr (PASS < P) {
+        if constexpr (PASS == 0) {
+            for (int tid = 0; tid < T; tid++)
+                for (int e = 2 * tid; e < (1 << LOGN); e += 2 * T) *reinterpret_cast<u64x2 *>(lds + lds_slot(e)) = src_load2(ops, nullptr, e, tab);
+            for (int tid = 0; tid < T; tid++) ntt_pass<LOGN, true, MODE, 0, 0, false, SrcTerm, true, TwInline, NoHook, C>(lds, nullptr, tid, T, tab, ops);
+        } else if constexpr (PASS == P - 1) {
+            for (int tid = 0; tid < T; tid++)
+                ntt_pass<LOGN, true, MODE, PASS, 0, false, SrcPlain, false, TwInline, NoHook, C, SinkRoundSum>(lds, nullptr, tid, T, tab, SrcPlain(), TwInline(), NoHook(),
+                                                                                                          SinkRoundSum{ acc + (size_t)tid * C, tab.q >> 1, tab.q });
+        } else
+            for (int tid = 0; tid < T; tid++) ntt_pass<LOGN, true, MODE, PASS, 0, false, SrcPlain, false, TwInline, NoHook, C>(lds, nullptr, tid, T, tab);
+        emu_terms_passes<LOGN, MODE, C, PASS + 1>(lds, tab, T, ops, acc);
+    }
+}
+template <int LOGN, int MODE, int C, class NEXT>
+void emu_ntt_terms(const NttTable &tab, int terms, const NEXT &next, u64 *out)
+{
+    constexpr int N = 1 << LOGN, T = N / C;
+    std::vector<u64> lds(lds_slots(N)), acc((size_t)N, 0);
+    for (int j = 0; j < terms; j++) emu_terms_passes<LOGN, MODE, C>(lds.data(), tab, T, next(j), acc.data());
+    for (int tid = 0; tid < T; tid++)
+        for (int i = 0; i < C; i++) out[ntt_sink_elem<LOGN, C>(tid, i)] = acc[(size_t)tid * C + i];
+}
+
+}
+
+extern "C" {
+
+const char *emu_i0_last_error() { return g_err.c_str(); }
+
+int emu_intt_terms(int logn, uint64_t q, const void *rows, size_t row_stride, uint32_t kb, const uint64_t *c, size_t c_stride, int terms, int lazy,
+                   uint64_t *out)
+{
+    return guarded([&]() -> int {
+        if (logn != 12 && logn != 13) throw std::invalid_argument("k_intt_terms exists for logn 12 and 13");
+        if (terms < 1 || (unsigned __int128)((u64)terms + 1) * q >= ((unsigned __int128)1 << 64)) throw std::invalid_argument("terms out of range ((terms + 1) q < 2^64)");
+        const EmuTables et(logn, q);
+        const NttTable &tab = et.tab;
+        if (lazy && !ntt_fold128_ok(tab.fold_k, tab.fold_c)) return -2;
+        if (lazy && !ntt_lazy_input_ok(tab, logn)) return -3;
+        auto next = [&](int j) { return SrcTerm{ static_cast<const char *>(rows) + (size_t)j * row_stride, c + (size_t)j * c_stride, kb, lazy != 0 }; };
+        emu_with_mode(tab, [&](auto mode) {
+            constexpr int MODE = decltype(mode)::value;
+            if (logn == 13) emu_ntt_terms<13, MODE, 8>(tab, terms, next, out);
+            else emu_ntt_terms<12, MODE, 8>(tab, terms, next, out);
+        });
+        return 0;
+    });
+}
+
+int emu_plan_eval_i0(unsigned bits, int low, int high, int L, int nB, uint32_t l, uint64_t q_last, uint64_t q_widest, int Bs, int max_terms, int logn)
+{
+    EvalState s{};
+    s.low = low; s.high = high; s.L = L; s.nB = nB; s.l = l; s.q_last = q_last; s.q_widest = q_widest; s.Bs = Bs; s.max_terms = max_terms;
+    s.high_in_flight = bits & 1; s.eval_side = bits & 2; s.prof_on = bits & 4; s.force_per_term = bits & 8; s.fuse_tensor = bits & 16;
+    s.fuse_tail = bits & 32; s.lane2 = bits & 64; s.on_lane0 = bits & 128; s.i0_fused = bits & 256; s.logn = logn;
+    const EvalPlan p = plan_eval(s);
+    return (int)p.i0_fast | p.need_vlast << 1 | p.raw_drop << 2 | p.raw_i0 << 3 | p.fused_drop << 4 | p.summed << 5 | p.side << 6 | p.side_i0 << 7 |
+           p.wait_high_ready << 8 | p.fuse_tensor << 9 | p.fuse_tail << 10 | p.cf << 11 | p.i0 << 13 | p.i0_grouped << 16 | (int)p.i0_g << 17;
+}
+void emu_i0_switches(int64_t *out)
+{
+    const EngineSwitches s = read_switches();
+    out[0] = s.i0_fused; out[1] = (int64_t)s.i0_group;
+}
+int emu_i0_grouped_ring(int logn) { return i0_grouped_ring(logn); }
+int emu_i0_group_terms(uint32_t terms, uint32_t jobs) { return (int)i0_group_terms(terms, jobs); }
+int emu_i0_groups(uint32_t terms, uint32_t g) { return (int)i0_groups(terms, g); }
+
+}
diff --git a/apsu_amd/csrc/engine.h b/apsu_amd/csrc/engine.h
--- a/apsu_amd/csrc/engine.h
+++ b/apsu_amd/csrc/engine.h
@@ -235,7 +235,8 @@
                 STEP_SEED_EXPAND, STEP_DECRYPT_ROUND, STEP_PLAIN_POWERS, STEP_SAMPLE_SMALL, STEP_SMALL_LIFT, STEP_ENC_FINISH, STEP_RLK_FINISH,
                 STEP_FLAG_MONOMIAL,
                 STEP_MAC_INFO, STEP_MAC, STEP_TERM_PRODUCT, STEP_PACK_ROWS, STEP_UNPACK_ROWS, STEP_LIMB0_ROWS,
-                STEP_ENTRIES_SCATTER, STEP_COUNT };
+                STEP_ENTRIES_SCATTER,
+                STEP_INTT_TERMS, STEP_COUNT };
     enum : uint32_t { STEP_RAW = 1, STEP_ACCUMULATE = 2, STEP_STORE = 4, STEP_KEY = 8, STEP_PLAN = 16, STEP_COMPOSED = 32, STEP_INVERSE = 64, STEP_NORED = 128,
                       STEP_KARA = 256, STEP_PACKED = 512, STEP_LIMB_SLOW = 1024 };
     struct StepArgs {
@@ -367,6 +368,7 @@
     void ps_cf_streams(const EvalCall &c, const PsBatch &g, std::vector<MacStream> &out);
     void ps_cf_mac(const EvalCall &c, const PsBatch &g);
     void ps_term_product(const EvalCall &c, const PsBatch &g);
+    void ps_intt_terms(const EvalCall &c, const PsBatch &g);
     void ps_i0_finish(const EvalCall &c, const EvalPlan &plan, const PsBatch &g, u64 *i0);
     void ps_tables(EvalCall &c, const EvalPlan &plan, PsBatch &g);
     void ps_run(EvalCall &c, const EvalPlan &plan, PsBatch &g);
diff --git a/apsu_amd/csrc/engine_eval.cpp b/apsu_amd/csrc/engine_eval.cpp
--- a/apsu_amd/csrc/engine_eval.cpp
+++ b/apsu_amd/csrc/engine_eval.cpp
@@ -40,6 +40,9 @@
     const MacJob *mac_jobs = nullptr;
     const TermJob *term_jobs = nullptr;
     size_t n_term = 0; bool term_packed = false;
+    const TermsJob *terms_jobs = nullptr;
+    size_t n_terms_jobs = 0, term_row_stride = 0;
+    u32 groups = 0, term_kb = 64;
     u64 *ext = nullptr, *result = nullptr, *ks_acc = nullptr, *i0_side = nullptr;
 };
 
@@ -105,6 +108,7 @@
     s.high_in_flight = c.pw.high_async && c.pw.high_ready;
     s.eval_side = sw_.eval_side; s.prof_on = prof_on_; s.force_per_term = sw_.force_per_term; s.fuse_tensor = fuse_tensor_; s.fuse_tail = sw_.fuse_tail;
     s.lane2 = lanes_[2].st != nullptr; s.on_lane0 = cur_lane_ == 0;
+    s.logn = hp_.logn; s.i0_fused = sw_.i0_fused; s.i0_group = (uint32_t)std::min<size_t>(sw_.i0_group, 4096);
     const EvalPlan plan = plan_eval(s);
     ps_tables(c, plan, g);
     ps_run(c, plan, g);
@@ -117,11 +121,17 @@
     const int Bs = g.Bs;
     const bool cf_here = plan.cf == CF_WITH_MAC;
     const size_t w_inner = (size_t)g.NI * 2 * Ll * n, w_ssum = plan.i0_fast ? (size_t)Bs * 2 * Lh * n : 0;
-    const size_t w_vlast = plan.need_vlast ? (size_t)Bs * l * 2 * n : 0, w_term = plan.i0_fast ? 0 : (size_t)Bs * l * 2 * Ll * n;
+    if (plan.i0_grouped) g.groups = i0_groups(l, plan.i0_g);
+    const size_t w_vlast = plan.i0_grouped ? (size_t)Bs * 2 * g.groups * n : plan.need_vlast ? (size_t)Bs * l * 2 * n : 0, w_term = plan.i0_fast ? 0 : (size_t)Bs * l * 2 * Ll * n;
     const size_t w_cf = (size_t)Bs * 2 * Lh * n;
     g.inner = ws(w_inner + w_ssum + w_vlast + w_term + (cf_here ? w_cf : 0));
     g.ssum = g.inner + w_inner; g.vlast = g.ssum + w_ssum; g.term = g.vlast + w_vlast;
     g.cf = cf_here ? g.term + w_term : nullptr;
+    if (plan.i0_grouped) {
+        g.term = g.ssum + w_ssum;
+        g.cf = cf_here ? g.term + w_term : nullptr;
+        g.vlast = g.term + w_term + (cf_here ? w_cf : 0);
+    }
     std::vector<MacStream> ms;
     auto map_push = [&](size_t polys, int first_limb, int limbs) {
         for (size_t p = 0; p < polys; p++) for (int j = 0; j < limbs; j++) g.imap.push_back(first_limb + j);
@@ -149,7 +159,25 @@
         if (plan.raw_i0) for (size_t x = g.imap.size() - (size_t)Bs * 2 * Lh; x < g.imap.size(); x++) g.imap[x] |= NTT_MAP_RAW;
     }
     std::vector<TermJob> tj;
-    if (plan.need_vlast || !plan.i0_fast) {
+    std::vector<TermsJob> gj;
+    if (plan.i0_grouped) {
+        const int limb = (int)Ll - 1;
+        for (int x = 0; x < Bs; x++) {
+            const Bundle &b = c.bundle(g.ids[x]);
+            const int bs = c.slot(g.ids[x]);
+            size_t row_off = (size_t)limb * n * sizeof(u64);
+            if (b.packed) { row_off = 0; for (int j = 0; j < limb; j++) row_off += n * packed_row_bits(hp_.key_q[j]) / 8; }
+            const size_t stride = b.packed ? b.ntt_slot_bytes : Ll * n * sizeof(u64);
+            if (x == 0) { g.term_packed = b.packed; g.term_row_stride = stride; g.term_kb = b.packed ? packed_row_bits(hp_.key_q[limb]) : 64; }
+            else if (g.term_packed != (bool)b.packed || g.term_row_stride != stride) throw std::logic_error("BinBundles of one evaluation differ in their row format");
+            for (u32 grp = 0; grp < g.groups; grp++) {
+                const u32 j0 = grp * plan.i0_g, cnt = std::min(plan.i0_g, l - j0);
+                for (int p = 0; p < 2; p++)
+                    gj.push_back(TermsJob{ reinterpret_cast<const char *>(bundle_slot(b, false, j0, Ll * n)) + row_off,
+                                           c.low_ptr(j0 + 1, bs) + ((size_t)p * Ll + limb) * n, g.vlast + (((size_t)x * g.groups + grp) * 2 + p) * n, cnt, 0 });
+            }
+        }
+    } else if (plan.need_vlast || !plan.i0_fast) {
         for (int x = 0; x < Bs; x++) {
             const Bundle &b = c.bundle(g.ids[x]);
             const int bs = c.slot(g.ids[x]);
@@ -171,11 +199,12 @@
             if (plan.raw_i0) for (size_t x = g.imap.size() - (size_t)Bs * l * 2; x < g.imap.size(); x++) g.imap[x] |= NTT_MAP_RAW;
         } else map_push((size_t)Bs * l * 2, 0, (int)Ll);
     }
-    if (plan.side_i0) g.n_vlast_side = (size_t)Bs * l * 2;
+    if (plan.side_i0 && !plan.i0_grouped) g.n_vlast_side = (size_t)Bs * l * 2;
     if (cf_here) { ps_cf_streams(c, g, ms); map_push((size_t)Bs * 2, 0, (int)Lh); }
     g.mac = plan_mac(ms, Ll, n);
     g.mac_jobs = upload_jobs(g.mac.jobs);
     if (!tj.empty()) { g.term_jobs = upload_jobs(tj); g.n_term = tj.size(); }
+    if (!gj.empty()) { g.terms_jobs = upload_jobs(gj); g.n_terms_jobs = gj.size(); }
 }
 
 void Engine::ps_term_product(const EvalCall &c, const PsBatch &g)
@@ -183,12 +212,20 @@
     PROF(P_MAC, (uint64_t)g.n_term * (g.term_packed ? packed_row_bits(hp_.key_q[c.Ll - 1]) : 64));
     launch_term_product(dlevel(c.low), g.term_jobs, g.n_term, c.n, (int)c.Ll - 1, (u32)(c.Ll * c.n), (u32)c.n, g.term_packed, st_);
 }
+void Engine::ps_intt_terms(const EvalCall &c, const PsBatch &g)
+{
+    PROF(P_NTT_FUSED, (uint64_t)g.Bs * c.l * 2);
+    launch_intt_terms(hp_.logn, g.terms_jobs, g.n_terms_jobs, g.term_row_stride, c.low_term_stride, g.term_kb, tabs(), (int)c.Ll - 1, st_);
+}
 void Engine::ps_i0_finish(const EvalCall &c, const EvalPlan &plan, const PsBatch &g, u64 *i0)
 {
     std::vector<I0Job> ij;
     for (int x = 0; x < g.Bs; x++)
-        ij.push_back(I0Job{ g.ssum + (size_t)x * 2 * c.Lh * c.n, g.vlast + (size_t)x * c.l * 2 * c.n, i0 + (size_t)x * 2 * c.Lh * c.n, (int)c.l, 1 });
-    PROFW(P_MODSWITCH, (size_t)g.Bs * c.n * (4 * c.Lh + 2 * c.l));
+        if (plan.i0_grouped)
+            ij.push_back(I0Job{ g.ssum + (size_t)x * 2 * c.Lh * c.n, nullptr, i0 + (size_t)x * 2 * c.Lh * c.n, (int)c.l, 1, g.vlast + (size_t)x * g.groups * 2 * c.n, (int)g.groups });
+        else
+            ij.push_back(I0Job{ g.ssum + (size_t)x * 2 * c.Lh * c.n, g.vlast + (size_t)x * c.l * 2 * c.n, i0 + (size_t)x * 2 * c.Lh * c.n, (int)c.l, 1 });
+    PROFW(P_MODSWITCH, (size_t)g.Bs * c.n * (4 * c.Lh + 2 * (plan.i0_grouped ? g.groups : c.l)));
     launch_i0_finish(dlevel(c.low), upload_jobs(ij), c.n, g.Bs, st_, plan.raw_i0);
 }
 
@@ -197,6 +234,7 @@
     d_mac(g.mac, g.mac_jobs);
     g.imap_dev = upload_jobs(g.imap);
     if (plan.side_i0) HIP_CHECK(hipEventRecord(ev_fork_, st_));
+    else if (plan.i0_grouped) ps_intt_terms(c, g);
     else if (g.n_term) ps_term_product(c, g);
     d_ntt(g.inner, g.imap.size() - g.n_vlast_side, g.imap_dev, (int)g.imap.size(), true, false);
     if (plan.side_i0) HIP_CHECK(hipEventRecord(ev_intt_, st_));
@@ -210,7 +248,8 @@
     switch_lane(2);
     struct Back { Engine *e; ~Back() { e->switch_lane(0); } } back{ this };
     HIP_CHECK(hipStreamWaitEvent(st_, ev_fork_, 0));
-    if (plan.side_i0) {
+    if (plan.side_i0 && plan.i0_grouped) ps_intt_terms(c, g);
+    else if (plan.side_i0) {
         ps_term_product(c, g);
         d_ntt(g.vlast, g.n_vlast_side, g.imap_dev + (g.imap.size() - g.n_vlast_side), (int)g.n_vlast_side, true, false);
     }
diff --git a/apsu_amd/csrc/engine_mac_steps.cpp b/apsu_amd/csrc/engine_mac_steps.cpp
--- a/apsu_amd/csrc/engine_mac_steps.cpp
+++ b/apsu_amd/csrc/engine_mac_steps.cpp
@@ -1,5 +1,6 @@
 #include "engine_impl.h"
 #include "mac_plan.h"
+#include "eval_plan.h"
 
 #include <string>
 
@@ -40,7 +41,7 @@
 void Engine::debug_run_mac_step(const StepArgs &a)
 {
     const size_t n = hp_.n;
-    need(a.step >= STEP_MAC_INFO && a.step <= STEP_LIMB0_ROWS, "unknown step");
+    need((a.step >= STEP_MAC_INFO && a.step <= STEP_LIMB0_ROWS) || a.step == STEP_INTT_TERMS, "unknown step");
     check_level(a.chain_idx);
     const int L = a.chain_idx + 1;
     const bool kara = a.flags & STEP_KARA, packed = a.flags & STEP_PACKED, limb_slow = a.flags & STEP_LIMB_SLOW;
@@ -73,6 +74,8 @@
 
     std::vector<MacJob> mj;
     std::vector<TermJob> tj;
+    std::vector<TermsJob> gj;
+    size_t groups = 0;
     std::vector<u64> padded;
     auto pad_in = [&](int i) { padded.assign(a.in_words[i] + 2, 0); std::memcpy(padded.data(), a.in[i], a.in_words[i] * sizeof(u64)); };
     size_t P = 0, NL = 0, njobs = 0;
@@ -144,6 +147,20 @@
         out_is(0, batch * n, "limb0_rows: out[0] [count][n]");
         if (packed) pad_in(0);
     } break;
+    case STEP_INTT_TERMS: {
+        need(i0_grouped_ring(hp_.logn), "intt_terms: launch_intt_terms exists for ring sizes 4096 and 8192 only");
+        need(batch >= 1 && batch <= 64, "intt_terms: batch out of range (1 .. 64)");
+        need(terms >= 1 && terms <= 4096, "intt_terms: terms out of range (1 .. 4096)");
+        need(polys >= 1, "intt_terms: a group of no terms (polys 0)");
+        need((unsigned __int128)(terms + 1) * lv.q[L - 1].q < ((unsigned __int128)1 << 64), "intt_terms: (terms + 1) * q_last reaches 2^64 (eval_plan.h, p.i0_fast)");
+        groups = i0_groups((uint32_t)terms, (uint32_t)polys);
+        in_is(0, batch * terms * 2 * L * n, "intt_terms: in[0] powers [batch][terms][2][L][n]");
+        in_is(1, batch * terms * slot_words, "intt_terms: in[1] plaintexts [batch][terms] slots");
+        out_is(0, batch * groups * 2 * n, "intt_terms: out[0] [batch][groups][2][n]");
+        for (size_t r = 0; r < batch * terms * 2; r++) canonical(a.in[0] + (r * L + (size_t)L - 1) * n, n, lv.q[L - 1].q, "intt_terms: in[0] (powers)");
+        if (packed) { pad_in(1); canonical_packed(padded, batch * terms, slot, L, n, lv, "intt_terms: in[1] (bit-packed plaintexts)"); }
+        else canonical_dense(a.in[1], batch * terms, L, n, lv, "intt_terms: in[1] (plaintexts)");
+    } break;
     default: refuse("unknown step");
     }
 
@@ -184,6 +201,20 @@
             for (size_t u = 0; u < njobs; u++) tj.push_back(TermJob{ reinterpret_cast<const u64 *>(pt + (u % batch) * slot), pw + (u % batch) * 2 * P * n, o + u * 2 * n });
             launch_term_product(dlevel(a.chain_idx), jobs(tj), njobs, n, a.e0, (u32)(P * n), (u32)n, packed, st_);
         } break;
+        case STEP_INTT_TERMS: {
+            const u64 *pw = up(a.in[0], a.in_words[0]);
+            const char *pt = reinterpret_cast<const char *>(up_slots(1));
+            const size_t row_off = packed ? lv.mac_row_off[L - 1] : (size_t)(L - 1) * n * sizeof(u64);
+            gj.clear();
+            for (size_t b = 0; b < batch; b++)
+                for (size_t grp = 0; grp < groups; grp++)
+                    for (size_t p = 0; p < 2; p++) {
+                        const size_t j0 = grp * polys, cnt = std::min(polys, terms - j0);
+                        gj.push_back(TermsJob{ pt + (b * terms + j0) * slot + row_off, pw + (((b * terms + j0) * 2 + p) * L + (size_t)L - 1) * n,
+                                               o + ((b * groups + grp) * 2 + p) * n, (u32)cnt, 0 });
+                    }
+            launch_intt_terms(hp_.logn, jobs(gj), gj.size(), slot, 2 * (size_t)L * n, packed ? lv.mac_bits[L - 1] : 64, tabs(), L - 1, st_);
+        } break;
         case STEP_PACK_ROWS:
             launch_pack_rows(dlevel(a.chain_idx), L, up(a.in[0], a.in_words[0]), o, packed_slot, n, batch, st_);
             break;
diff --git a/apsu_amd/csrc/eval_plan.h b/apsu_amd/csrc/eval_plan.h
--- a/apsu_amd/csrc/eval_plan.h
+++ b/apsu_amd/csrc/eval_plan.h
@@ -16,6 +16,9 @@
     bool high_in_flight;
     bool eval_side, prof_on, force_per_term, fuse_tensor, fuse_tail;
     bool lane2, on_lane0;
+    int logn;
+    bool i0_fused;
+    uint32_t i0_group;
 };
 enum CfPlace {
     CF_WITH_MAC = 0,
@@ -32,7 +35,21 @@
     bool i0_fast, need_vlast, raw_drop, raw_i0, fused_drop, summed, side, side_i0, wait_high_ready, fuse_tensor, fuse_tail;
     int cf;
     int i0;
+    bool i0_grouped;
+    uint32_t i0_g;
 };
+
+constexpr bool i0_grouped_ring(int logn) { return logn == 12 || logn == 13; }
+constexpr uint32_t I0_GROUP_WGS = 512, I0_GROUP_MIN = 2, I0_GROUP_MAX = 11;
+constexpr uint32_t i0_group_terms(uint32_t terms, uint32_t jobs)
+{
+    if (terms <= I0_GROUP_MIN || !jobs) return terms ? terms : 1;
+    const uint32_t per_job = (I0_GROUP_WGS + jobs - 1) / jobs;
+    uint32_t g = terms / per_job;
+    g = g < I0_GROUP_MIN ? I0_GROUP_MIN : g > I0_GROUP_MAX ? I0_GROUP_MAX : g;
+    return g < terms ? g : terms;
+}
+constexpr uint32_t i0_groups(uint32_t terms, uint32_t g) { return (terms + g - 1) / g; }
 
 inline EvalPlan plan_eval(const EvalState &s)
 {
@@ -51,6 +68,8 @@
     p.summed = !s.force_per_term && Lh <= 4 && (unsigned __int128)s.max_terms * s.q_widest < ((unsigned __int128)1 << 63);
     p.fuse_tensor = s.fuse_tensor;
     p.fuse_tail = s.fuse_tail;
+    p.i0_grouped = s.i0_fused && p.i0_fast && p.need_vlast && s.low == s.high + 1 && i0_grouped_ring(s.logn);
+    p.i0_g = !p.i0_grouped ? 0 : s.i0_group ? (s.i0_group < s.l ? s.i0_group : s.l) : i0_group_terms(s.l, 2 * (uint32_t)s.Bs);
     return p;
 }
 
diff --git a/apsu_amd/csrc/kernels_behz.hip b/apsu_amd/csrc/kernels_behz.hip
--- a/apsu_amd/csrc/kernels_behz.hip
+++ b/apsu_amd/csrc/kernels_behz.hip
@@ -642,6 +642,10 @@
     const u64 *v = job.v + (size_t)p * n + k;
     u64 tw0 = 0, tw1 = 0;
     if (RAW) { const u64x2 tw = ldg16(reinterpret_cast<const u64 *>(lv->last_tw + k)); tw0 = tw[0]; tw1 = tw[1]; }
+    if (job.groups) {
+        const u64 *gs = job.gsum + (size_t)p * n + k;
+        for (int t = 0; t < job.groups; t++) R += gs[(size_t)t * 2 * n];
+    } else
     for (int t = 0; t < job.terms; t++) {
         u64 x = v[(size_t)t * 2 * n];
         if (RAW) x = mul_shoup(x, tw0, tw1, ql);
diff --git a/apsu_amd/csrc/kernels_ntt.hip b/apsu_amd/csrc/kernels_ntt.hip
--- a/apsu_amd/csrc/kernels_ntt.hip
+++ b/apsu_amd/csrc/kernels_ntt.hip
@@ -138,6 +138,29 @@
         else if (tab.wide_d4) ntt_body<LOGN, true, NTT_WIDE_NEAR, T, 0, false, SrcTensor, true, false, 0, -1, C>(lds, p, tab, tid, nullptr, ops);
         else ntt_body<LOGN, true, NTT_WIDE, T, 0, false, SrcTensor, true, false, 0, -1, C>(lds, p, tab, tid, nullptr, ops);
     }
+}
+
+template <int LOGN, int T, int C, bool PACKED>
+__global__ __launch_bounds__(T, 4) void k_intt_terms(const TermsJob *__restrict__ jobs, size_t row_stride, size_t c_stride, u32 kb,
+                                                  const NttTable *__restrict__ tabs, int mod)
+{
+    constexpr int N = 1 << LOGN;
+    __shared__ __attribute__((aligned(16))) u64 lds[lds_slots(N)];
+    const int tid = threadIdx.x;
+    const TermsJob job = jobs[blockIdx.x];
+    const NttTable tab = tabs[mod];
+    const bool lazy = ntt_lazy_input_ok(tab, LOGN);
+    u64 acc[C];
+#pragma unroll
+    for (int i = 0; i < C; i++) acc[i] = 0;
+    auto sink = [&](const NttTable &t) { return SinkRoundSum{ acc, t.q >> 1, t.q }; };
+    if constexpr (PACKED) __builtin_assume(kb != 0);
+    auto next = [&](int j) { return SrcTerm{ static_cast<const char *>(job.row) + (size_t)j * row_stride, job.c + (size_t)j * c_stride, PACKED ? kb : 0, lazy }; };
+    if (tab.narrow) ntt_terms_body<LOGN, NTT_NARROW, T, C, SrcTerm>(lds, tab, tid, (int)job.terms, next, sink);
+    else if (tab.wide_d4) ntt_terms_body<LOGN, NTT_WIDE_NEAR, T, C, SrcTerm>(lds, tab, tid, (int)job.terms, next, sink);
+    else ntt_terms_body<LOGN, NTT_WIDE, T, C, SrcTerm>(lds, tab, tid, (int)job.terms, next, sink);
+#pragma unroll
+    for (int i = 0; i < C; i++) job.out[ntt_sink_elem<LOGN, C>(tid, i)] = acc[i];
 }
 
 template <class K> struct NttFormRow { int logn, threads, coeffs_per_lane, min_waves; K inv, fwd; };
@@ -217,4 +240,17 @@
     KERNEL_CHECK();
 }
 
-}
+void launch_intt_terms(int logn, const TermsJob *jobs, size_t njobs, size_t row_stride, size_t c_stride, u32 kb, const NttTable *tabs, int mod,
+                       hipStream_t st)
+{
+    if (!njobs) return;
+    const bool packed = kb != 64;
+    if (logn == 13 && packed) hipLaunchKernelGGL((k_intt_terms<13, 1024, 8, true>), dim3((unsigned)njobs), dim3(1024), 0, st, jobs, row_stride, c_stride, kb, tabs, mod);
+    else if (logn == 13) hipLaunchKernelGGL((k_intt_terms<13, 1024, 8, false>), dim3((unsigned)njobs), dim3(1024), 0, st, jobs, row_stride, c_stride, kb, tabs, mod);
+    else if (logn == 12 && packed) hipLaunchKernelGGL((k_intt_terms<12, 512, 8, true>), dim3((unsigned)njobs), dim3(512), 0, st, jobs, row_stride, c_stride, kb, tabs, mod);
+    else if (logn == 12) hipLaunchKernelGGL((k_intt_terms<12, 512, 8, false>), dim3((unsigned)njobs), dim3(512), 0, st, jobs, row_stride, c_stride, kb, tabs, mod);
+    else throw_hip(hipErrorInvalidValue, __FILE__, __LINE__);
+    KERNEL_CHECK();
+}
+
+}
diff --git a/apsu_amd/csrc/launch_behz.h b/apsu_amd/csrc/launch_behz.h
--- a/apsu_amd/csrc/launch_behz.h
+++ b/apsu_amd/csrc/launch_behz.h
@@ -26,7 +26,7 @@
                 const u64 *ks_acc = nullptr; };
 void launch_eval_epilogue(const DevLevel *levels, int lvl, const EpiJob *jobs, size_t ct_poly_stride, int clear_bits, size_t n,
                           int njobs, hipStream_t st, const DevKey *key = nullptr);
-struct I0Job { const u64 *s; const u64 *v; u64 *acc; int terms; int store; };
+struct I0Job { const u64 *s; const u64 *v; u64 *acc; int terms; int store; const u64 *gsum = nullptr; int groups = 0; };
 void launch_i0_finish(const DevLevel *lv_low, const I0Job *jobs, size_t n, int njobs, hipStream_t st, bool raw = false);
 
 }
diff --git a/apsu_amd/csrc/launch_ntt.h b/apsu_amd/csrc/launch_ntt.h
--- a/apsu_amd/csrc/launch_ntt.h
+++ b/apsu_amd/csrc/launch_ntt.h
@@ -11,5 +11,8 @@
 struct TensorJob { const u64 *a, *b; u64 *d; };
 void launch_intt_tensor(int logn, const TensorJob *jobs, int njobs, int limbs, size_t src_ps, u64 *plain, size_t n_plain,
                         const NttTable *tabs, const int *modmap, int period, hipStream_t st, size_t latency_limbs = 0);
+struct TermsJob { const void *row; const u64 *c; u64 *out; u32 terms, pad; };
+void launch_intt_terms(int logn, const TermsJob *jobs, size_t njobs, size_t row_stride, size_t c_stride, u32 kb, const NttTable *tabs, int mod,
+                       hipStream_t st);
 
 }
diff --git a/apsu_amd/csrc/mac_core.h b/apsu_amd/csrc/mac_core.h
--- a/apsu_amd/csrc/mac_core.h
+++ b/apsu_amd/csrc/mac_core.h
@@ -1,6 +1,7 @@
 #pragma once
 #include <stddef.h>
 #include "dev_consts.h"
+#include "packed_rows.h"
 
 namespace apsu_he {
 
@@ -39,44 +40,6 @@
 #else
 #define MAC_KEEP(v) do { } while (0)
 #endif
-
-HD u32 alignbit(u32 hi, u32 lo, u32 sh)
-{
-#if defined(__HIP_DEVICE_COMPILE__)
-    return __builtin_amdgcn_alignbit(hi, lo, sh);
-#else
-    return (u32)((((u64)hi << 32) | lo) >> (sh & 31));
-#endif
-}
-
-HD const u32 *packed_window(const void *slot, u32 row_off, size_t k, u32 kb, u32 &psh)
-{
-    const u32 bitoff = (u32)(k >> 1) * 2 * kb;
-    psh = bitoff & 31;
-    return reinterpret_cast<const u32 *>(static_cast<const char *>(slot) + row_off) + (bitoff >> 5);
-}
-HD void packed_shift(u64 w_lo, u64 w_hi, u32 psh, u64 &lo64, u64 &hi64)
-{
-    const u32 w0 = (u32)w_lo, w1 = (u32)(w_lo >> 32), w2 = (u32)w_hi, w3 = (u32)(w_hi >> 32);
-    const u32 n0 = alignbit(w1, w0, psh), n1 = alignbit(w2, w1, psh), n2 = alignbit(w3, w2, psh), n3 = w3 >> psh;
-    lo64 = (u64)n0 | ((u64)n1 << 32); hi64 = (u64)n2 | ((u64)n3 << 32);
-}
-#define PACKED_SECOND(lo64, hi64, kb) ((kb) == 64 ? (hi64) : (((lo64) >> (kb)) | ((hi64) << (64 - (kb)))))
-HD void packed_pair(u64 w_lo, u64 w_hi, u32 psh, u32 kb, u64 &a0, u64 &a1)
-{
-    u64 lo64, hi64;
-    packed_shift(w_lo, w_hi, psh, lo64, hi64);
-    if (kb == 64) { a0 = lo64; a1 = hi64; }
-    else { const u64 mask = ((u64)1 << kb) - 1; a0 = lo64 & mask; a1 = PACKED_SECOND(lo64, hi64, kb) & mask; }
-}
-HD u64 packed_coeff(const u32 *row, size_t c, u32 w)
-{
-    const size_t bit0 = c * w, d0 = bit0 >> 5;
-    const u32 sh = (u32)(bit0 & 31);
-    u64 v = ((u64)row[d0] | ((u64)row[d0 + 1] << 32)) >> sh;
-    if (sh && w + sh > 64) v |= (u64)row[d0 + 2] << (64 - sh);
-    return w == 64 ? v : (v & (((u64)1 << w) - 1));
-}
 
 #if defined(__HIPCC__)
 #define MAC_LANE_FN __global__ __launch_bounds__(EW_T, 1) void
diff --git a/apsu_amd/csrc/ntt_core.h b/apsu_amd/csrc/ntt_core.h
--- a/apsu_amd/csrc/ntt_core.h
+++ b/apsu_amd/csrc/ntt_core.h
@@ -2,6 +2,7 @@
 #include <type_traits>
 
 #include "modmath.h"
+#include "packed_rows.h"
 
 struct TwPair { u64 w, wq; };
 
@@ -104,6 +105,7 @@
 struct SrcPlain {};
 struct SrcStaged {};
 struct SrcTensor { const u64 *x0, *y0, *x1, *y1; bool lazy; };
+struct SrcTerm { const void *row; const u64 *c; u32 kb; bool lazy; };
 HD u64x2 src_load2(const SrcPlain &, const u64 *glob, int e, const NttTable &) { return *reinterpret_cast<const u64x2 *>(glob + e); }
 HD u64 src_load1(const SrcPlain &, const u64 *glob, int e, const NttTable &) { return glob[e]; }
 HD u64x2 src_load2(const SrcStaged &, const u64 *glob, int e, const NttTable &) { return *reinterpret_cast<const u64x2 *>(glob + e); }
@@ -133,9 +135,34 @@
     if (s.x1) mac128(p, s.x1[e], s.y1[e]);
     return s.lazy ? ntt_reduce128_lazy(p.hi, p.lo, tab) : ntt_reduce128(p.hi, p.lo, tab);
 }
+HD u64x2 src_load2(const SrcTerm &s, const u64 *, int e, const NttTable &tab)
+{
+    u64 a0, a1;
+    if (s.kb) {
+        u32 psh;
+        const u32x4a4 w = ldg16_a4_nt(apsu_he::packed_window(s.row, 0, (size_t)e, s.kb, psh));
+        apsu_he::packed_pair((u64)w[0] | ((u64)w[1] << 32), (u64)w[2] | ((u64)w[3] << 32), psh, s.kb, a0, a1);
+    } else {
+        const u64x2 a = ldg16_nt(static_cast<const u64 *>(s.row) + e);
+        a0 = a[0]; a1 = a[1];
+    }
+    const u64x2 c = ldg16(s.c + e);
+    const u128p p0 = mul128(a0, c[0]), p1 = mul128(a1, c[1]);
+    u64x2 r;
+    if (s.lazy) {
+        r[0] = ntt_reduce128_lazy(p0.hi, p0.lo, tab);
+        r[1] = ntt_reduce128_lazy(p1.hi, p1.lo, tab);
+    } else {
+        r[0] = ntt_reduce128(p0.hi, p0.lo, tab);
+        r[1] = ntt_reduce128(p1.hi, p1.lo, tab);
+    }
+    return r;
+}
+HD u64 src_load1(const SrcTerm &s, const u64 *glob, int e, const NttTable &tab) { return src_load2(s, glob, e & ~1, tab)[e & 1]; }
 HD u64 src_in_bound(const SrcPlain &, const NttTable &) { return 1; }
 HD u64 src_in_bound(const SrcStaged &, const NttTable &) { return 1; }
 HD u64 src_in_bound(const SrcTensor &s, const NttTable &tab) { return s.lazy ? ntt_lazy_bound_q(tab) : 1; }
+HD u64 src_in_bound(const SrcTerm &s, const NttTable &tab) { return s.lazy ? ntt_lazy_bound_q(tab) : 1; }
 HD int lds_slot(int e) { return e + ((e >> 4) << 1); }
 constexpr int lds_slots(int n) { return n + (n >> 3); }
 
@@ -217,6 +244,11 @@
 struct TwInline {};
 template <int NT> struct TwRegs { u64x2 t[NT > 0 ? NT : 1]; };
 struct NoHook { HD void operator()() const {} };
+struct NoSink {};
+struct SinkRoundSum {
+    u64 *acc; u64 half, q;
+    HD void operator()(int slot, u64 v) const { acc[slot] += addmod(v, half, q); }
+};
 
 template <int LOGN, int S, int K, bool INV, int C = 16>
 HD void ntt_load_twiddles(TwRegs<PassShape<LOGN, S, K, INV, C>::NT> &tw, int w, const NttTable &tab)
@@ -256,9 +288,9 @@
 }
 
 template <int LOGN, int S, int K, bool INV, int MODE, int IN, int OUT, int RED = 0, bool RAW = false, class SRC = SrcPlain,
-          class TW = TwInline, class HOOK = NoHook, int C = 16>
+          class TW = TwInline, class HOOK = NoHook, int C = 16, class SINK = NoSink>
 HD void ntt_pass16(u64 *lds, u64 *__restrict__ glob, int w, const NttTable &tab, const SRC &src = SRC(), const TW &tw = TW(),
-                   const HOOK &hook = HOOK())
+                   const HOOK &hook = HOOK(), const SINK &sink = SINK())
 {
     using PS = PassShape<LOGN, S, K, INV, C>;
     static_assert((C == 16 || C == 8 || C == 4) && (1 << K) <= C, "radix 2^K on C coefficients per work item");
@@ -386,6 +418,14 @@
                 r[g][j] = v;
             }
     }
+    if constexpr (!std::is_same<SINK, NoSink>::value) {
+        static_assert(OUT == IO_GLOBAL && INV && !RAW, "a sink takes the canonical results of the pass that leaves an inverse transform");
+#pragma unroll
+        for (int g = 0; g < G; g++)
+#pragma unroll
+            for (int j = 0; j < R; j++) sink(g * R + j, r[g][j]);
+        return;
+    }
     if (PAIR_G) {
 #pragma unroll
         for (int j = 0; j < R; j++)
@@ -470,9 +510,9 @@
 }
 
 template <int LOGN, bool INV, int MODE, int PASS, int RED = 0, bool RAW = false, class SRC = SrcPlain, bool STAGED = false,
-          class TW = TwInline, class HOOK = NoHook, int C = 16>
+          class TW = TwInline, class HOOK = NoHook, int C = 16, class SINK = NoSink>
 HD void ntt_pass(u64 *lds, u64 *glob, int tid, int T, const NttTable &tab, const SRC &src = SRC(), const TW &tw = TW(),
-                 const HOOK &hook = HOOK())
+                 const HOOK &hook = HOOK(), const SINK &sink = SINK())
 {
     constexpr int P = plan_passes(LOGN, C);
     constexpr int p = INV ? P - 1 - PASS : PASS;
@@ -482,5 +522,10 @@
     constexpr int OUT = (INV && PASS == P - 1) ? IO_GLOBAL : IO_LDS;
     constexpr int LOGC = C == 16 ? 4 : C == 8 ? 3 : 2;
     for (int w = tid; w < (1 << (LOGN - LOGC)); w += T)
-        ntt_pass16<LOGN, S, K, INV, MODE, IN, OUT, RED, RAW, SRC, TW, HOOK, C>(lds, glob, w, tab, src, tw, hook);
-}
+        ntt_pass16<LOGN, S, K, INV, MODE, IN, OUT, RED, RAW, SRC, TW, HOOK, C, SINK>(lds, glob, w, tab, src, tw, hook, sink);
+}
+template <int LOGN, int C> HD int ntt_sink_elem(int w, int slot)
+{
+    constexpr int K = plan_k(LOGN, 0, C), R = 1 << K, G = C >> K;
+    return ((slot % R) << (LOGN - K)) | (w * G + slot / R);
+}
diff --git a/apsu_amd/csrc/ntt_wg.h b/apsu_amd/csrc/ntt_wg.h
--- a/apsu_amd/csrc/ntt_wg.h
+++ b/apsu_amd/csrc/ntt_wg.h
@@ -123,4 +123,59 @@
     if constexpr (NEXTPASS >= 0) { if (next) ntt_touch_done(sink); }
 }
 
+template <int LOGN, int MODE, int T, int C, class SRC, class NEXT, class MAKE_SINK>
+__device__ __forceinline__ void ntt_terms_body(u64 *lds, const NttTable &tab0, int tid, int terms, const NEXT &next, const MAKE_SINK &make_sink)
+{
+    NttTable tab = tab0;
+    constexpr int N = 1 << LOGN;
+    constexpr int P = plan_passes(LOGN, C);
+    static_assert(T % 64 == 0 && T * C == N, "one work item per thread: a sink slot is one coefficient for the whole call");
+    static_assert(P >= 2 && P <= 5, "no pass schedule for this ring size and coefficients per lane");
+    constexpr int WCO = 64 * C / 128;
+    auto fp = [](int k) constexpr { return P - 1 - k; };
+    constexpr bool WL = ntt_wave_private<LOGN, T, C>(fp(0));
+    constexpr bool W1 = ntt_wave_private<LOGN, T, C>(fp(1));
+    constexpr bool W2 = P > 2 && ntt_wave_private<LOGN, T, C>(fp(P > 2 ? 2 : 1));
+    constexpr bool W3 = P > 3 && ntt_wave_private<LOGN, T, C>(fp(P > 3 ? 3 : 1));
+    constexpr bool W4 = P > 4 && ntt_wave_private<LOGN, T, C>(fp(P > 4 ? 4 : 1));
+    for (int j = 0; j < terms; j++) {
+        const SRC operands = next(j);
+        asm volatile("" : "+s"(tab.dit), "+s"(tab.scale), "+v"(tid));
+        asm volatile("" : "+s"(tab.q), "+s"(tab.r1), "+s"(tab.r0), "+s"(tab.fold_k), "+s"(tab.fold_c), "+s"(tab.wide_d4));
+        __builtin_assume(tid >= 0 && tid < T);
+        const auto sink = make_sink(tab);
+        using SINK = std::remove_const_t<decltype(sink)>;
+        const int wbase = (tid & ~63) * C, lane = tid & 63;
+        if (j) __syncthreads();
+        if constexpr (WL) {
+#pragma unroll
+            for (int i = 0; i < WCO; i++) {
+                const int e = wbase + 128 * i + 2 * lane;
+                if (e < N) *reinterpret_cast<u64x2 *>(lds + lds_slot(e)) = src_load2(operands, nullptr, e, tab);
+            }
+        } else {
+            for (int e = 2 * tid; e < N; e += 2 * T) *reinterpret_cast<u64x2 *>(lds + lds_slot(e)) = src_load2(operands, nullptr, e, tab);
+        }
+        ntt_sync<WL>();
+        ntt_pass<LOGN, true, MODE, 0, 0, false, SRC, true, TwInline, NoHook, C>(lds, nullptr, tid, T, tab, operands);
+        ntt_sync<W1>();
+        if constexpr (P == 2) ntt_pass<LOGN, true, MODE, 1, 0, false, SrcPlain, false, TwInline, NoHook, C, SINK>(lds, nullptr, tid, T, tab, SrcPlain(), TwInline(), NoHook(), sink);
+        else ntt_pass<LOGN, true, MODE, 1, 0, false, SrcPlain, false, TwInline, NoHook, C>(lds, nullptr, tid, T, tab);
+        if constexpr (P > 2) {
+            ntt_sync<W2>();
+            if constexpr (P == 3) ntt_pass<LOGN, true, MODE, 2, 0, false, SrcPlain, false, TwInline, NoHook, C, SINK>(lds, nullptr, tid, T, tab, SrcPlain(), TwInline(), NoHook(), sink);
+            else ntt_pass<LOGN, true, MODE, 2, 0, false, SrcPlain, false, TwInline, NoHook, C>(lds, nullptr, tid, T, tab);
+        }
+        if constexpr (P > 3) {
+            ntt_sync<W3>();
+            if constexpr (P == 4) ntt_pass<LOGN, true, MODE, 3, 0, false, SrcPlain, false, TwInline, NoHook, C, SINK>(lds, nullptr, tid, T, tab, SrcPlain(), TwInline(), NoHook(), sink);
+            else ntt_pass<LOGN, true, MODE, 3, 0, false, SrcPlain, false, TwInline, NoHook, C>(lds, nullptr, tid, T, tab);
+        }
+        if constexpr (P > 4) {
+            ntt_sync<W4>();
+            ntt_pass<LOGN, true, MODE, 4, 0, false, SrcPlain, false, TwInline, NoHook, C, SINK>(lds, nullptr, tid, T, tab, SrcPlain(), TwInline(), NoHook(), sink);
+        }
+    }
+}
+
 #endif
diff --git a/apsu_amd/csrc/packed_rows.h b/apsu_amd/csrc/packed_rows.h
--- /dev/null
+++ b/apsu_amd/csrc/packed_rows.h
@@ -0,0 +1,45 @@
+#pragma once
+#include <stddef.h>
+#include "modmath.h"
+
+namespace apsu_he {
+
+HD u32 alignbit(u32 hi, u32 lo, u32 sh)
+{
+#if defined(__HIP_DEVICE_COMPILE__)
+    return __builtin_amdgcn_alignbit(hi, lo, sh);
+#else
+    return (u32)((((u64)hi << 32) | lo) >> (sh & 31));
+#endif
+}
+
+HD const u32 *packed_window(const void *slot, u32 row_off, size_t k, u32 kb, u32 &psh)
+{
+    const u32 bitoff = (u32)(k >> 1) * 2 * kb;
+    psh = bitoff & 31;
+    return reinterpret_cast<const u32 *>(static_cast<const char *>(slot) + row_off) + (bitoff >> 5);
+}
+HD void packed_shift(u64 w_lo, u64 w_hi, u32 psh, u64 &lo64, u64 &hi64)
+{
+    const u32 w0 = (u32)w_lo, w1 = (u32)(w_lo >> 32), w2 = (u32)w_hi, w3 = (u32)(w_hi >> 32);
+    const u32 n0 = alignbit(w1, w0, psh), n1 = alignbit(w2, w1, psh), n2 = alignbit(w3, w2, psh), n3 = w3 >> psh;
+    lo64 = (u64)n0 | ((u64)n1 << 32); hi64 = (u64)n2 | ((u64)n3 << 32);
+}
+#define PACKED_SECOND(lo64, hi64, kb) ((kb) == 64 ? (hi64) : (((lo64) >> (kb)) | ((hi64) << (64 - (kb)))))
+HD void packed_pair(u64 w_lo, u64 w_hi, u32 psh, u32 kb, u64 &a0, u64 &a1)
+{
+    u64 lo64, hi64;
+    packed_shift(w_lo, w_hi, psh, lo64, hi64);
+    if (kb == 64) { a0 = lo64; a1 = hi64; }
+    else { const u64 mask = ((u64)1 << kb) - 1; a0 = lo64 & mask; a1 = PACKED_SECOND(lo64, hi64, kb) & mask; }
+}
+HD u64 packed_coeff(const u32 *row, size_t c, u32 w)
+{
+    const size_t bit0 = c * w, d0 = bit0 >> 5;
+    const u32 sh = (u32)(bit0 & 31);
+    u64 v = ((u64)row[d0] | ((u64)row[d0 + 1] << 32)) >> sh;
+    if (sh && w + sh > 64) v |= (u64)row[d0 + 2] << (64 - sh);
+    return w == 64 ? v : (v & (((u64)1 << w) - 1));
+}
+
+}
diff --git a/apsu_amd/engine.py b/apsu_amd/engine.py
--- a/apsu_amd/engine.py
+++ b/apsu_amd/engine.py
@@ -156,7 +156,7 @@
     "polyn_with_roots", "bins_update", "bin_counts", "poly_degree", "bins_lookup", "bins_merge", "bins_rows", "bins_eval", "eval_compare", "roots",
     "unlift", "ntt_info", "ntt", "ntt_gather", "intt_tensor", "roots_split",
     "seed_expand", "decrypt_round", "plain_powers", "sample_small", "small_lift", "enc_finish", "rlk_finish", "flag_monomial",
-    "mac_info", "mac", "term_product", "pack_rows", "unpack_rows", "limb0_rows", "entries_scatter"))}
+    "mac_info", "mac", "term_product", "pack_rows", "unpack_rows", "limb0_rows", "entries_scatter", "intt_terms"))}
 STEP_RAW, STEP_ACCUMULATE, STEP_STORE, STEP_KEY, STEP_PLAN, STEP_COMPOSED, STEP_INVERSE, STEP_NORED = 1, 2, 4, 8, 16, 32, 64, 128
 STEP_KARA, STEP_PACKED, STEP_LIMB_SLOW = 256, 512, 1024
 STEP_MAP_RAW = 1 << 30
diff --git a/include/apsu_he.h b/include/apsu_he.h
--- a/include/apsu_he.h
+++ b/include/apsu_he.h
@@ -108,7 +108,8 @@
        APSU_HE_STEP_ENC_FINISH, APSU_HE_STEP_RLK_FINISH, APSU_HE_STEP_FLAG_MONOMIAL,
        APSU_HE_STEP_MAC_INFO, APSU_HE_STEP_MAC, APSU_HE_STEP_TERM_PRODUCT, APSU_HE_STEP_PACK_ROWS, APSU_HE_STEP_UNPACK_ROWS,
        APSU_HE_STEP_LIMB0_ROWS,
-       APSU_HE_STEP_ENTRIES_SCATTER };
+       APSU_HE_STEP_ENTRIES_SCATTER,
+       APSU_HE_STEP_INTT_TERMS };
 enum { APSU_HE_STEP_RAW = 1, APSU_HE_STEP_ACCUMULATE = 2, APSU_HE_STEP_STORE = 4, APSU_HE_STEP_KEY = 8, APSU_HE_STEP_PLAN = 16,
        APSU_HE_STEP_COMPOSED = 32, APSU_HE_STEP_INVERSE = 64, APSU_HE_STEP_NORED = 128, APSU_HE_STEP_KARA = 256, APSU_HE_STEP_PACKED = 512,
        APSU_HE_STEP_LIMB_SLOW = 1024 };
```
